# Aatrick/LightDiffusion

Hardware: AMD Instinct MI355X
Metric: UNet denoise steps/sec at 512x512 (higher is better)
Workload: dtype f16 (fp32 accumulate); 1 GPU; SD1.5 512x512 UNet CFG step, euler_ancestral / normal-30, batch 8/GPU (UNet batch 16), latent 64x64; global_batch=8, parallelism=dp1 (replicas, RCCL cond broadcast), hip_graph=True, setup_before_warmup=hipGraph capture + one untimed schedule pass per workload

## Files before the change

### include/ld_mi355x.h

```cpp
#ifndef LD_MI355X_H
#define LD_MI355X_H

#include <stddef.h>
#include <stdint.h>

#ifdef __cplusplus
extern "C" {
#endif

#define LD_OK 0
#define LD_ERR_ARG 1
#define LD_ERR_SHAPE 2
#define LD_ERR_HIP 3
#define LD_ERR_STATE 4

#define LD_F16 0
#define LD_F32 1

const char* ld_version(void);
const char* ld_status_string(int status);

typedef struct {
    int in_channels, out_channels, model_channels;
    int num_levels;
    int channel_mult[8];
    int num_res_blocks[8];
    int transformer_depth[16];
    int transformer_depth_output[24];
    int transformer_depth_middle;
    int context_dim, num_heads;
} ld_unet_config;

typedef struct ld_unet ld_unet;

int ld_unet_create(const ld_unet_config* cfg, ld_unet** out);
void ld_unet_destroy(ld_unet* u);
int ld_unet_param_count(const ld_unet* u);
int ld_unet_param_info(const ld_unet* u, int index, const char** name, int* ndim, int64_t shape[4]);
int ld_unet_load_param(ld_unet* u, const char* name, const void* dev_src, int dtype, void* stream);
int ld_unet_reserve(ld_unet* u, int max_n, int max_h, int max_w, int max_ctx_tokens);
size_t ld_unet_workspace_bytes(const ld_unet* u);
size_t ld_unet_weight_bytes(const ld_unet* u);
int ld_unet_set_context(ld_unet* u, const void* ctx, int dtype, int n, int tokens, void* stream);
int ld_unet_forward(ld_unet* u, const float* x, const float* sigma, float* out, int n, int h, int w, int eps_only, void* stream);
int ld_unet_forward_pair(ld_unet* u, const float* x, const float* sigma, float* out, int nb, int h, int w, void* stream);
int ld_unet_profile(ld_unet* u, const float* x, const float* sigma, float* out, int n, int h, int w, void* stream, double ms[6],
                    double flops[6], int launches[6]);
int ld_unet_profile_pair(ld_unet* u, const float* x, const float* sigma, float* out, int nb, int h, int w, void* stream, double ms[6],
                         double flops[6], int launches[6]);
int ld_unet_profile_kernels(const ld_unet* u, char* buf, size_t buf_bytes);
int ld_unet_profile_launches(const ld_unet* u, char* buf, size_t buf_bytes);
int ld_unet_last_launches(const ld_unet* u);
double ld_unet_last_flops(const ld_unet* u);

typedef struct {
    int z_channels, ch, num_levels;
    int ch_mult[8];
    int num_res_blocks, out_ch;
    int with_encoder;
} ld_vae_config;

typedef struct ld_vae ld_vae;

int ld_vae_create(const ld_vae_config* cfg, ld_vae** out);
void ld_vae_destroy(ld_vae* v);
int ld_vae_param_count(const ld_vae* v);
int ld_vae_param_info(const ld_vae* v, int index, const char** name, int* ndim, int64_t shape[4]);
int ld_vae_load_param(ld_vae* v, const char* name, const void* dev_src, int dtype, void* stream);
int ld_vae_reserve(ld_vae* v, int max_b, int max_h, int max_w);
size_t ld_vae_workspace_bytes(const ld_vae* v);
size_t ld_vae_plan_bytes(ld_vae* v, int b, int h, int w);
int ld_vae_decode(ld_vae* v, const float* z, float* out, int b, int h, int w, void* stream);
int ld_vae_encode(ld_vae* v, const float* pixels_nchw, float* moments, int b, int h, int w, void* stream);
int ld_vae_profile(ld_vae* v, const float* z, float* out, int b, int h, int w, void* stream);
int ld_vae_profile_launches(const ld_vae* v, char* buf, size_t buf_bytes);
int ld_vae_last_launches(const ld_vae* v);
double ld_vae_last_flops(const ld_vae* v);

int ld_op_linear(const void* x, const void* w, const void* bias, const void* residual, void* y, int M, int N, int K,
                 float alpha, int act, void* ws, size_t ws_bytes, void* stream);
int ld_op_conv(const void* x1, int c1, const void* x2, int c2, int n, int h, int w, int hv, int wv, int stride, int ksize,
               const void* wt, const void* bias, const void* rowvec, const void* residual, void* y, int cout,
               void* ws, size_t ws_bytes, void* stream);
size_t ld_op_groupnorm_conv_ws_bytes(int c1, int c2, int n, int h, int w, int cout);
int ld_op_groupnorm_conv(const void* x1, int c1, const void* x2, int c2, int n, int h, int w, const void* gamma, const void* beta, float eps,
                         const void* wt, const void* bias, const void* rowvec, const void* residual, void* y, int cout, void* ws,
                         size_t ws_bytes, void* stream);
int ld_op_repack_conv(const void* src_oihw, int dtype, int cout, int cin, void* dst, void* stream);
size_t ld_op_conv_skip_ws_bytes(int c, int sc1, int sc2, int cout);
int ld_op_conv_skip(const void* x, int c, int n, int h, int w, const void* wt, const void* bias, const void* s1, int sc1, const void* s2, int sc2,
                    const void* wskip, const void* bskip, const void* rowvec, void* y, int cout, void* ws, size_t ws_bytes, void* stream);
size_t ld_op_conv_gn_partials_floats(int n, int hw);
int ld_op_conv_gn_partials(const void* x, int c, int n, int h, int w, int hv, int wv, const void* wt, const void* bias,
                           const void* residual, void* y, int cout, float* part, int* chunks, void* ws, size_t ws_bytes, void* stream);
size_t ld_op_groupnorm_ws_bytes(int n, int hw);
int ld_op_groupnorm(const void* x1, int c1, const void* x2, int c2, int n, int hw, const void* gamma, const void* beta,
                    float eps, int silu, void* y, void* ws, void* stream);
int ld_op_layernorm(const void* x, const void* gamma, const void* beta, void* y, int rows, int c, float eps, void* stream);
int ld_op_attention(const void* q, int ldq, const void* k, int ldk, const void* vt, int ldvt, void* o, int ldo, int b,
                    int heads, int lq, int lk, int d, float scale, int causal, void* stream);
int ld_op_attention_rowv(const void* q, int ldq, const void* k, int ldk, const void* v, int ldv, void* o, int ldo, int b,
                         int heads, int lq, int lk, int d, float scale, int causal, void* stream);
int ld_op_softmax_rows(void* s, int rows, int cols, void* stream);
int ld_op_timestep_embed(const float* sigma, const float* log_sigmas, int n_sigmas, int n, int dim, void* out_f16, float* t_out,
                         void* stream);
int ld_op_cfg_combine(const float* den2, float* out, float cfg, size_t n_half, void* stream);
int ld_op_axpby(float* x, float a, const float* y, float b, const float* z, float c, size_t n, void* stream);
int ld_op_hook_check(const void* a, const void* b, size_t words_ab, const void* x, size_t half_words_x, const void* sigma, int half_sigma,
                     int* flags, int epoch, void* stream);

int ld_op_linear_ln(const void* x, const void* w_prod, const void* b_prod, const void* gamma, const void* beta, const void* w,
                    const void* bias, void* t_out, void* y, int M, int C, int N, float eps, void* ws, size_t ws_bytes, void* stream);
int ld_op_linear_ln_geglu(const void* x, const void* w_prod, const void* b_prod, const void* gamma, const void* beta, const void* w,
                          const void* bias, void* t_out, void* y, int M, int C, int N, float eps, void* ws, size_t ws_bytes, void* stream);
int ld_op_bislerp(const float* x, float* tmp, float* y, int n, int c, int h, int w, int h_new, int w_new, void* stream);
const char* ld_op_last_kernel(void);

#ifdef __cplusplus
}
#endif
#endif
```

### lightdiffusion_amd/_lib.py

```python
from __future__ import annotations

import ctypes as C
import os

_HERE = os.path.dirname(os.path.abspath(__file__))
LIB_PATH = os.environ.get("LD_MI355X_LIB") or os.path.join(_HERE, "libld_mi355x.so")

OK, ERR_ARG, ERR_SHAPE, ERR_HIP, ERR_STATE = 0, 1, 2, 3, 4
F16, F32 = 0, 1


class UNetConfig(C.Structure):
    _fields_ = [("in_channels", C.c_int), ("out_channels", C.c_int), ("model_channels", C.c_int), ("num_levels", C.c_int),
                ("channel_mult", C.c_int * 8), ("num_res_blocks", C.c_int * 8), ("transformer_depth", C.c_int * 16),
                ("transformer_depth_output", C.c_int * 24), ("transformer_depth_middle", C.c_int),
                ("context_dim", C.c_int), ("num_heads", C.c_int)]


class VAEConfig(C.Structure):
    _fields_ = [("z_channels", C.c_int), ("ch", C.c_int), ("num_levels", C.c_int), ("ch_mult", C.c_int * 8),
                ("num_res_blocks", C.c_int), ("out_ch", C.c_int), ("with_encoder", C.c_int)]


class LDError(RuntimeError):
    def __init__(self, status: int, where: str):
        self.status = status
        msg = lib().ld_status_string(status).decode() if _lib is not None else str(status)
        super().__init__(f"{where}: {msg} (status {status})")


_lib = None
_P, _I, _F, _Z = C.c_void_p, C.c_int, C.c_float, C.c_size_t

SIGNATURES = {
    "ld_version": (C.c_char_p, []),
    "ld_status_string": (C.c_char_p, [_I]),
    "ld_unet_create": (_I, [C.POINTER(UNetConfig), C.POINTER(_P)]),
    "ld_unet_destroy": (None, [_P]),
    "ld_unet_param_count": (_I, [_P]),
    "ld_unet_param_info": (_I, [_P, _I, C.POINTER(C.c_char_p), C.POINTER(_I), C.POINTER(C.c_int64)]),
    "ld_unet_load_param": (_I, [_P, C.c_char_p, _P, _I, _P]),
    "ld_unet_reserve": (_I, [_P, _I, _I, _I, _I]),
    "ld_unet_workspace_bytes": (_Z, [_P]),
    "ld_unet_weight_bytes": (_Z, [_P]),
    "ld_unet_set_context": (_I, [_P, _P, _I, _I, _I, _P]),
    "ld_unet_forward": (_I, [_P, _P, _P, _P, _I, _I, _I, _I, _P]),
    "ld_unet_forward_pair": (_I, [_P, _P, _P, _P, _I, _I, _I, _P]),
    "ld_unet_profile_pair": (_I, [_P, _P, _P, _P, _I, _I, _I, _P, C.POINTER(C.c_double), C.POINTER(C.c_double), C.POINTER(_I)]),
    "ld_unet_profile": (_I, [_P, _P, _P, _P, _I, _I, _I, _P, C.POINTER(C.c_double), C.POINTER(C.c_double), C.POINTER(_I)]),
    "ld_unet_profile_kernels": (_I, [_P, C.c_char_p, _Z]),
    "ld_unet_profile_launches": (_I, [_P, C.c_char_p, _Z]),
    "ld_unet_last_launches": (_I, [_P]),
    "ld_unet_last_flops": (C.c_double, [_P]),
    "ld_vae_create": (_I, [C.POINTER(VAEConfig), C.POINTER(_P)]),
    "ld_vae_destroy": (None, [_P]),
    "ld_vae_param_count": (_I, [_P]),
    "ld_vae_param_info": (_I, [_P, _I, C.POINTER(C.c_char_p), C.POINTER(_I), C.POINTER(C.c_int64)]),
    "ld_vae_load_param": (_I, [_P, C.c_char_p, _P, _I, _P]),
    "ld_vae_reserve": (_I, [_P, _I, _I, _I]),
    "ld_vae_workspace_bytes": (_Z, [_P]),
    "ld_vae_plan_bytes": (_Z, [_P, _I, _I, _I]),
    "ld_vae_decode": (_I, [_P, _P, _P, _I, _I, _I, _P]),
    "ld_vae_encode": (_I, [_P, _P, _P, _I, _I, _I, _P]),
    "ld_vae_profile": (_I, [_P, _P, _P, _I, _I, _I, _P]),
    "ld_vae_profile_launches": (_I, [_P, C.c_char_p, _Z]),
    "ld_vae_last_launches": (_I, [_P]),
    "ld_vae_last_flops": (C.c_double, [_P]),
    "ld_op_linear": (_I, [_P, _P, _P, _P, _P, _I, _I, _I, _F, _I, _P, _Z, _P]),
    "ld_op_conv": (_I, [_P, _I, _P, _I, _I, _I, _I, _I, _I, _I, _I, _P, _P, _P, _P, _P, _I, _P, _Z, _P]),
    "ld_op_groupnorm_conv_ws_bytes": (_Z, [_I, _I, _I, _I, _I, _I]),
    "ld_op_groupnorm_conv": (_I, [_P, _I, _P, _I, _I, _I, _I, _P, _P, _F, _P, _P, _P, _P, _P, _I, _P, _Z, _P]),
    "ld_op_repack_conv": (_I, [_P, _I, _I, _I, _P, _P]),
    "ld_op_conv_skip_ws_bytes": (_Z, [_I, _I, _I, _I]),
    "ld_op_conv_skip": (_I, [_P, _I, _I, _I, _I, _P, _P, _P, _I, _P, _I, _P, _P, _P, _P, _I, _P, _Z, _P]),
    "ld_op_groupnorm_ws_bytes": (_Z, [_I, _I]),
    "ld_op_groupnorm": (_I, [_P, _I, _P, _I, _I, _I, _P, _P, _F, _I, _P, _P, _P]),
    "ld_op_layernorm": (_I, [_P, _P, _P, _P, _I, _I, _F, _P]),
    "ld_op_attention": (_I, [_P, _I, _P, _I, _P, _I, _P, _I, _I, _I, _I, _I, _I, _F, _I, _P]),
    "ld_op_conv_gn_partials_floats": (_Z, [_I, _I]),
    "ld_op_conv_gn_partials": (_I, [_P, _I, _I, _I, _I, _I, _I, _P, _P, _P, _P, _I, _P, _P, _P, _Z, _P]),
    "ld_op_attention_rowv": (_I, [_P, _I, _P, _I, _P, _I, _P, _I, _I, _I, _I, _I, _I, _F, _I, _P]),
    "ld_op_softmax_rows": (_I, [_P, _I, _I, _P]),
    "ld_op_timestep_embed": (_I, [_P, _P, _I, _I, _I, _P, _P, _P]),
    "ld_op_cfg_combine": (_I, [_P, _P, _F, _Z, _P]),
    "ld_op_axpby": (_I, [_P, _F, _P, _F, _P, _F, _Z, _P]),
    "ld_op_hook_check": (_I, [_P, _P, _Z, _P, _Z, _P, _I, _P, _I, _P]),
    "ld_op_linear_ln": (_I, [_P, _P, _P, _P, _P, _P, _P, _P, _P, _I, _I, _I, _F, _P, _Z, _P]),
    "ld_op_linear_ln_geglu": (_I, [_P, _P, _P, _P, _P, _P, _P, _P, _P, _I, _I, _I, _F, _P, _Z, _P]),
    "ld_op_bislerp": (_I, [_P, _P, _P, _I, _I, _I, _I, _I, _I, _P]),
    "ld_op_last_kernel": (C.c_char_p, []),
}


def lib() -> C.CDLL:
    global _lib
    if _lib is None:
        if not os.path.exists(LIB_PATH):
            raise ImportError(f"{LIB_PATH} not found — build it with `python -c 'import __graft_entry__ as g; g.build()'` "
                              f"or `make -C lightdiffusion_amd/csrc`.  There is no CPU / PyTorch fallback for the hot path.")
        try:
            import torch
        except ImportError:
            pass
        l = C.CDLL(LIB_PATH)
        missing = []
        for name, (res, args) in SIGNATURES.items():
            if not hasattr(l, name):
                if not os.environ.get("LD_MI355X_LIB"):
                    raise AttributeError(f"{LIB_PATH} does not export {name}: header and library out of sync — rebuild it")
                missing.append(name)
                setattr(l, name, _missing_symbol(name))
                continue
            fn = getattr(l, name)
            fn.restype = res
            fn.argtypes = args
        l._ld_missing = tuple(missing)
        _lib = l
    return _lib


def _missing_symbol(name: str):
    def fail(*_a, **_k):
        raise RuntimeError(f"{LIB_PATH} (LD_MI355X_LIB) does not export {name}: it was built from a commit without this entry point")
    return fail


def check(status: int, where: str) -> None:
    if status != OK:
        raise LDError(status, where)
```

### lightdiffusion_amd/csrc/capi.hip

```cpp
#include <string>

#include "kernels.h"
#include "../../include/ld_mi355x.h"

namespace {
inline size_t align256(size_t v) { return (v + 255) / 256 * 256; }

thread_local std::string t_op_kernels;
inline void op_begin() { t_op_kernels.clear(); }
inline int noted(int st, const char* name) {
    if (name != nullptr && *name != '\0') {
        if (!t_op_kernels.empty()) t_op_kernels += ';';
        t_op_kernels += name;
    }
    return st;
}
inline int gemm_op(const GemmParams& p, hipStream_t s) { return noted(gemm_launch(p, s), gemm_last_kernel_name()); }
inline int gemm_op(const GemmParams& p, const GemmPlan& plan, hipStream_t s) { return noted(gemm_run(p, plan, s), gemm_last_kernel_name()); }

constexpr size_t kSyncBytes = LD_SYNC_INTS * sizeof(int);
inline size_t conv8_scratch_head(int cout, int cin) { return kSyncBytes + (conv8_weight_eligible(cout, cin) ? align256(conv8_weight_bytes(cout, cin)) : 0); }
inline void conv8_scratch(GemmParams& p, void* ws, size_t partial_bytes) {
    const int cin = p.C1 + p.C2;
    p.sync = (int*)ws;
    p.W8 = conv8_weight_eligible(p.N, cin) ? (const half_t*)((char*)ws + kSyncBytes) : nullptr;
    p.partial = (float*)((char*)ws + conv8_scratch_head(p.N, cin));
    p.partial_bytes = partial_bytes;
}
inline int conv8_scratch_op(const GemmParams& p, const GemmPlan& plan, const void* wt, hipStream_t stream) {
    if (plan.route == GR_CONV8) {
        if (hipMemsetAsync(p.sync, 0, kSyncBytes, stream) != hipSuccess) return LD_ERR_HIP;
        const int st = conv8_repack_launch((const half_t*)wt, p.N, p.C1 + p.C2, const_cast<half_t*>(p.W8), stream);
        if (st != LD_OK) return st;
    }
    return gemm_op(p, plan, stream);
}
inline int attn_op(const AttnParams& a, hipStream_t s) { return noted(attention_launch(a, s), attention_last_kernel_name()); }
}

extern "C" {

const char* ld_version(void) { return "ld_mi355x 0.1 (gfx950)"; }

const char* ld_op_last_kernel(void) { return t_op_kernels.c_str(); }

const char* ld_status_string(int s) {
    switch (s) {
        case LD_OK: return "ok";
        case LD_ERR_ARG: return "invalid argument";
        case LD_ERR_SHAPE: return "unsupported shape or alignment";
        case LD_ERR_HIP: return "HIP runtime error";
        case LD_ERR_STATE: return "invalid call order (weights / reserve / context missing)";
        default: return "unknown status";
    }
}

int ld_op_linear(const void* x, const void* w, const void* bias, const void* residual, void* y, int M, int N, int K, float alpha,
                 int act, void* ws, size_t ws_bytes, void* stream_) {
    op_begin();
    hipStream_t stream = (hipStream_t)stream_;
    GemmParams p;
    p.A = (const half_t*)x; p.lda = K;
    p.W = (const half_t*)w; p.ldw = K;
    p.M = M; p.N = N; p.K = K;
    p.alpha = alpha;
    p.bias_n = (const half_t*)bias;
    p.R = (const half_t*)residual;
    p.act = act;
    p.C = (half_t*)y;
    p.ldc = p.ldr = (act == 2 ? N / 2 : N);
    char* wsp = (char*)ws;
    if (act == 2) {
        if (bias == nullptr || (N & 15)) return LD_ERR_ARG;
        const int bn = gemm_pick_bn(N);
        if (N % bn) return LD_ERR_SHAPE;
        const size_t wb = align256((size_t)N * K * sizeof(half_t)), bb = align256((size_t)N * sizeof(half_t));
        if (ws == nullptr || ws_bytes < wb + bb) return LD_ERR_ARG;
        half_t* w2 = (half_t*)wsp;
        half_t* b2 = (half_t*)(wsp + wb);
        int st = repack_rows_launch(w, 0, N, K, w2, bn, stream);
        if (st != LD_OK) return st;
        st = repack_rows_launch(bias, 0, N, 1, b2, bn, stream);
        if (st != LD_OK) return st;
        p.W = w2;
        p.bias_n = b2;
        p.bn = bn;
        wsp += wb + bb;
        ws_bytes -= wb + bb;
    }
    p.partial = (float*)wsp;
    p.partial_bytes = ws ? ws_bytes : 0;
    if (ws == nullptr) p.partial = nullptr;
    return gemm_op(p, stream);
}

static int op_conv(const void* x1, int c1, const void* x2, int c2, int n, int h, int w, int hv, int wv, int stride, int ksize,
                   const void* wt, const void* bias, const void* rowvec, const void* residual, void* y, int cout, void* ws,
                   size_t ws_bytes, void* stream, float* gn_part, int* gn_chunks) {
    if (stride < 1 || (ksize != 1 && ksize != 3)) return LD_ERR_ARG;
    GemmParams p;
    if (gn_part != nullptr) {
        const int HW = (ksize == 3 ? (hv - 1) / stride + 1 : hv) * (ksize == 3 ? (wv - 1) / stride + 1 : wv);
        p.gn_part = gn_part;
        p.gn_P = gn_num_chunks(n, HW);
        p.gn_HW = HW;
        p.gn_ppb = (HW + p.gn_P - 1) / p.gn_P;
        p.gn_part_done = gn_chunks;
    }
    p.conv = 1;
    p.ksize = ksize;
    p.A = (const half_t*)x1; p.A2 = (const half_t*)x2; p.C1 = c1; p.C2 = c2;
    p.Hs = h; p.Ws = w; p.Hv = hv; p.Wv = wv; p.stride = stride;
    p.Ho = ksize == 3 ? (hv - 1) / stride + 1 : hv;
    p.Wo = ksize == 3 ? (wv - 1) / stride + 1 : wv;
    p.K = ksize * ksize * (c1 + c2);
    p.W = (const half_t*)wt; p.ldw = p.K;
    p.M = n * p.Ho * p.Wo; p.N = cout;
    p.bias_n = (const half_t*)bias;
    p.rowvec = (const half_t*)rowvec; p.rows_per_vec = p.Ho * p.Wo; p.ldrv = cout;
    p.R = (const half_t*)residual; p.ldr = cout;
    p.C = (half_t*)y; p.ldc = cout;
    p.partial = (float*)ws;
    p.partial_bytes = ws ? ws_bytes : 0;
    const size_t head = conv8_scratch_head(cout, c1 + c2);
    if (ws != nullptr && ksize == 3 && conv8_weight_eligible(cout, c1 + c2) && ws_bytes > head + ((size_t)8 << 20)) {
        GemmParams c8 = p;
        conv8_scratch(c8, ws, ws_bytes - head);
        if (const GemmPlan plan = gemm_plan(c8); plan.route == GR_CONV8) return conv8_scratch_op(c8, plan, wt, (hipStream_t)stream);
    }
    return gemm_op(p, (hipStream_t)stream);
}

int ld_op_conv(const void* x1, int c1, const void* x2, int c2, int n, int h, int w, int hv, int wv, int stride, int ksize,
               const void* wt, const void* bias, const void* rowvec, const void* residual, void* y, int cout, void* ws,
               size_t ws_bytes, void* stream) {
    op_begin();
    return op_conv(x1, c1, x2, c2, n, h, w, hv, wv, stride, ksize, wt, bias, rowvec, residual, y, cout, ws, ws_bytes, stream, nullptr, nullptr);
}

size_t ld_op_conv_gn_partials_floats(int n, int hw) {
    op_begin();
    return groupnorm_workspace_bytes(n, hw) / sizeof(float);
}

int ld_op_conv_gn_partials(const void* x, int c, int n, int h, int w, int hv, int wv, const void* wt, const void* bias, const void* residual,
                           void* y, int cout, float* part, int* chunks, void* ws, size_t ws_bytes, void* stream) {
    op_begin();
    if (part == nullptr || chunks == nullptr) return LD_ERR_ARG;
    *chunks = 0;
    return op_conv(x, c, nullptr, 0, n, h, w, hv, wv, 1, 3, wt, bias, nullptr, residual, y, cout, ws, ws_bytes, stream, part, chunks);
}

size_t ld_op_groupnorm_conv_ws_bytes(int c1, int c2, int n, int h, int w, int cout) {
    op_begin();
    const size_t C = (size_t)c1 + c2, HW = (size_t)h * w;
    return align256(groupnorm_workspace_bytes(n, (int)HW)) + 2 * align256((size_t)n * C * sizeof(float)) + align256((size_t)n * HW * C * sizeof(half_t)) +
           conv8_scratch_head(cout, c1 + c2) + ((size_t)96 << 20);
}

int ld_op_groupnorm_conv(const void* x1, int c1, const void* x2, int c2, int n, int h, int w, const void* gamma, const void* beta, float eps,
                         const void* wt, const void* bias, const void* rowvec, const void* residual, void* y, int cout, void* ws, size_t ws_bytes,
                         void* stream_) {
    op_begin();
    if (x1 == nullptr || gamma == nullptr || beta == nullptr || wt == nullptr || y == nullptr || ws == nullptr) return LD_ERR_ARG;
    if (ws_bytes < ld_op_groupnorm_conv_ws_bytes(c1, c2, n, h, w, cout)) return LD_ERR_ARG;
    hipStream_t stream = (hipStream_t)stream_;
    const int C = c1 + c2, HW = h * w;
    char* q = (char*)ws;
    float* part = (float*)q; q += align256(groupnorm_workspace_bytes(n, HW));
    float* scale = (float*)q; q += align256((size_t)n * C * sizeof(float));
    float* shift = (float*)q; q += align256((size_t)n * C * sizeof(float));
    half_t* g = (half_t*)q; q += align256((size_t)n * HW * C * sizeof(half_t));
    GemmParams p;
    p.conv = 1; p.ksize = 3;
    p.A = (const half_t*)x1; p.A2 = (const half_t*)x2; p.C1 = c1; p.C2 = c2;
    p.Hs = p.Hv = p.Ho = h; p.Ws = p.Wv = p.Wo = w; p.stride = 1;
    p.K = 9 * C; p.W = (const half_t*)wt; p.ldw = p.K;
    p.M = n * HW; p.N = cout;
    p.bias_n = (const half_t*)bias;
    p.rowvec = (const half_t*)rowvec; p.rows_per_vec = HW; p.ldrv = cout;
    p.R = (const half_t*)residual; p.ldr = cout;
    p.C = (half_t*)y; p.ldc = cout;
    conv8_scratch(p, q, (size_t)96 << 20);
    const GemmPlan fused = gemm_plan(p, true);
    if (fused.can_fuse_groupnorm) {
        int st = groupnorm_scale_shift_launch((const half_t*)x1, c1, (const half_t*)x2, c2, n, HW, (const half_t*)gamma, (const half_t*)beta, eps, part,
                                              scale, shift, stream);
        if (st != LD_OK) return st;
        p.gn_scale = scale; p.gn_shift = shift; p.gn_silu = 1;
        return gemm_op(p, fused, stream);
    }
    int st = groupnorm_launch((const half_t*)x1, c1, (const half_t*)x2, c2, n, HW, (const half_t*)gamma, (const half_t*)beta, eps, 1, g, part, stream);
    if (st != LD_OK) return st;
    p.A = g; p.A2 = nullptr; p.C1 = C; p.C2 = 0;
    return conv8_scratch_op(p, gemm_plan(p), (const half_t*)wt, stream);
}

size_t ld_op_conv_skip_ws_bytes(int c, int sc1, int sc2, int cout) {
    op_begin();
    return align256((size_t)cout * (9 * (size_t)c + sc1 + sc2) * sizeof(half_t)) + align256((size_t)cout * sizeof(half_t)) + ((size_t)96 << 20);
}

int ld_op_conv_skip(const void* x, int c, int n, int h, int w, const void* wt, const void* bias, const void* s1, int sc1, const void* s2, int sc2,
                    const void* wskip, const void* bskip, const void* rowvec, void* y, int cout, void* ws, size_t ws_bytes, void* stream_) {
    op_begin();
    if (x == nullptr || wt == nullptr || bias == nullptr || s1 == nullptr || wskip == nullptr || bskip == nullptr || y == nullptr || ws == nullptr) return LD_ERR_ARG;
    if (c <= 0 || sc1 <= 0 || sc2 < 0 || (sc2 > 0 && s2 == nullptr) || cout <= 0 || n <= 0 || h <= 0 || w <= 0) return LD_ERR_ARG;
    if (ws_bytes < ld_op_conv_skip_ws_bytes(c, sc1, sc2, cout)) return LD_ERR_ARG;
    hipStream_t stream = (hipStream_t)stream_;
    const int K9 = 9 * c, SC = sc1 + sc2;
    char* q = (char*)ws;
    half_t* wf = (half_t*)q; q += align256((size_t)cout * (K9 + SC) * sizeof(half_t));
    half_t* bf = (half_t*)q; q += align256((size_t)cout * sizeof(half_t));
    int st = skip_fold_launch((const half_t*)wt, (const half_t*)wskip, (const half_t*)bias, (const half_t*)bskip, cout, K9, SC, wf, bf, stream);
    if (st != LD_OK) return st;
    GemmParams p;
    p.conv = 1; p.ksize = 3;
    p.A = (const half_t*)x; p.C1 = c;
    p.Hs = p.Hv = p.Ho = h; p.Ws = p.Wv = p.Wo = w; p.stride = 1;
    p.S1 = (const half_t*)s1; p.SC1 = sc1; p.S2 = (const half_t*)s2; p.SC2 = sc2;
    p.K = K9 + SC; p.W = wf; p.ldw = p.K;
    p.M = n * h * w; p.N = cout;
    p.bias_n = bf;
    p.rowvec = (const half_t*)rowvec; p.rows_per_vec = h * w; p.ldrv = cout;
    p.C = (half_t*)y; p.ldc = cout;
    p.partial = (float*)q; p.partial_bytes = (size_t)96 << 20;
    return gemm_op(p, stream);
}

int ld_op_repack_conv(const void* src, int dtype, int cout, int cin, void* dst, void* stream) {
    op_begin();
    return repack_conv3x3_launch(src, dtype == LD_F32, cout, cin, (half_t*)dst, (hipStream_t)stream);
}

size_t ld_op_groupnorm_ws_bytes(int n, int hw) {
    op_begin();
    return groupnorm_workspace_bytes(n, hw);
}

int ld_op_groupnorm(const void* x1, int c1, const void* x2, int c2, int n, int hw, const void* gamma, const void* beta, float eps,
                    int silu, void* y, void* ws, void* stream) {
    op_begin();
    return groupnorm_launch((const half_t*)x1, c1, (const half_t*)x2, c2, n, hw, (const half_t*)gamma, (const half_t*)beta, eps,
                            silu, (half_t*)y, (float*)ws, (hipStream_t)stream);
}

int ld_op_layernorm(const void* x, const void* gamma, const void* beta, void* y, int rows, int c, float eps, void* stream) {
    op_begin();
    return layernorm_launch((const half_t*)x, (const half_t*)gamma, (const half_t*)beta, (half_t*)y, rows, c, eps, (hipStream_t)stream);
}

int ld_op_attention(const void* q, int ldq, const void* k, int ldk, const void* vt, int ldvt, void* o, int ldo, int b, int heads,
                    int lq, int lk, int d, float scale, int causal, void* stream) {
    op_begin();
    AttnParams a;
    a.Q = (const half_t*)q; a.ldq = ldq; a.sQ = (long long)lq * ldq;
    a.K = (const half_t*)k; a.ldk = ldk; a.sK = (long long)lk * ldk;
    a.Vt = (const half_t*)vt; a.ldvt = ldvt; a.sV = (long long)heads * d * ldvt;
    a.O = (half_t*)o; a.ldo = ldo; a.sO = (long long)lq * ldo;
    a.B = b; a.H = heads; a.Lq = lq; a.Lk = lk; a.d = d; a.scale = scale; a.causal = causal;
    return attn_op(a, (hipStream_t)stream);
}

int ld_op_attention_rowv(const void* q, int ldq, const void* k, int ldk, const void* v, int ldv, void* o, int ldo, int b, int heads,
                         int lq, int lk, int d, float scale, int causal, void* stream) {
    op_begin();
    const char *qb = (const char*)q, *kb = (const char*)k, *vb = (const char*)v;
    const long long rowb = (long long)ldq * 2;
    const bool fused = ldq == ldk && ldk == ldv && rowb > 0 && (kb - qb >= 0 ? kb - qb : qb - kb) < rowb && (vb - qb >= 0 ? vb - qb : qb - vb) < rowb;
    if (fused && lq != lk) return LD_ERR_SHAPE;
    AttnParams a;
    a.Q = (const half_t*)q; a.ldq = ldq; a.sQ = (long long)lq * ldq;
    a.K = (const half_t*)k; a.ldk = ldk; a.sK = (long long)lk * ldk;
    a.V = (const half_t*)v; a.ldv = ldv; a.sV = (long long)lk * ldv;
    a.O = (half_t*)o; a.ldo = ldo; a.sO = (long long)lq * ldo;
    a.B = b; a.H = heads; a.Lq = lq; a.Lk = lk; a.d = d; a.scale = scale; a.causal = causal;
    return attn_op(a, (hipStream_t)stream);
}

int ld_op_softmax_rows(void* s, int rows, int cols, void* stream) {
    op_begin();
    return softmax_rows_launch((half_t*)s, rows, cols, cols, (hipStream_t)stream);
}

int ld_op_timestep_embed(const float* sigma, const float* log_sigmas, int n_sigmas, int n, int dim, void* out, float* t_out, void* stream) {
    op_begin();
    return timestep_embed_launch(sigma, log_sigmas, n_sigmas, n, dim, (half_t*)out, t_out, (hipStream_t)stream);
}

int ld_op_cfg_combine(const float* den2, float* out, float cfg, size_t n_half, void* stream) {
// ... 107 lines not shown
```

### lightdiffusion_amd/csrc/gemm.h

```cpp
#pragma once
#include "common.h"

struct GemmParams {
    const half_t* A = nullptr;
    const half_t* A2 = nullptr;
    int lda = 0;
    int conv = 0;
    int ksize = 3;
    int pad = -1;
    int Hs = 0, Ws = 0;
    int Hv = 0, Wv = 0;
    int Ho = 0, Wo = 0, stride = 1;
    int C1 = 0, C2 = 0;
    const half_t* S1 = nullptr;
    const half_t* S2 = nullptr;
    int SC1 = 0, SC2 = 0;
    const half_t* W = nullptr;
    int ldw = 0;
    int M = 0, N = 0, K = 0;
    int n_valid = 0;
    int batch = 1;
    long long sA = 0, sW = 0, sC = 0, sR = 0;
    float alpha = 1.0f;
    const half_t* bias_n = nullptr;
    const half_t* bias_m = nullptr;
    const half_t* rowvec = nullptr;
    int rows_per_vec = 1, ldrv = 0;
    const half_t* R = nullptr;
    int ldr = 0;
    int act = 0;
    half_t* C = nullptr;
    int ldc = 0;
    int bm = 0, bn = 0;
    int splitk = 0;
    int m_fastest = -1;
    int xcd_gm = 0;
    float* partial = nullptr;
    size_t partial_bytes = 0;
    float* stat_out = nullptr;
    int* stat_parts_out = nullptr;
    const float* ln_stat = nullptr;
    int ln_parts = 0;
    int ln_rows = 0;
    int ln_zrows = 0;
    float ln_inv_c = 0.f, ln_eps = 0.f;
    const float* ln_wsum = nullptr;
    int ln_swapped = 0;
    const float* gn_scale = nullptr;
    const float* gn_shift = nullptr;
    int gn_silu = 0;
    float* gn_part = nullptr;
    int gn_P = 0, gn_ppb = 0, gn_HW = 0;
    int* gn_part_done = nullptr;
    const half_t* W8 = nullptr;
    int* sync = nullptr;
    int c8_S = 0;
    int dbg = 0;
};

enum GemmRoute { GR_NONE = 0, GR_CONV8, GR_CONV6, GR_GEMM7, GR_GEMM5, GR_GEMM3, GR_GEMM4 };
enum GemmReduce { GRD_NONE = 0, GRD_PLAIN, GRD_GROUPNORM };
struct GemmPlan {
    int status = LD_OK;
    int route = GR_NONE;
    bool conv = false, geglu = false;
    bool gn = false, up = false;
    bool ln = false;
    bool deep = false, two_wg = false;
    int bm = 0, bn = 0, wc = 0;
    int splitk = 1, c8_S = 0;
    int m_fastest = 0, xcd_gm = 0;
    unsigned grid_x = 0, grid_z = 1;
    int reduce = GRD_NONE;
    int stat_parts = 0;
    int gn_chunks = 0;
    bool halo_tile = false;
    bool can_fuse_groupnorm = false;
    bool takes_skip_segment = false;
    const char* kernel = "";
};
GemmPlan gemm_plan(const GemmParams& p, bool gn_offer = false);
int gemm_run(const GemmParams& p, const GemmPlan& plan, hipStream_t stream);
inline int gemm_launch(const GemmParams& p, hipStream_t stream) { return gemm_run(p, gemm_plan(p), stream); }
const char* gemm_last_kernel_name();

bool conv8_plan(const GemmParams& p, int* S_out);
int conv8_launch(const GemmParams& p, int S, hipStream_t stream);
bool conv8_weight_eligible(int N, int Cin);
size_t conv8_weight_bytes(int N, int Cin);
int conv8_repack_launch(const half_t* w_okki, int N, int Cin, half_t* dst, hipStream_t stream);
#define LD_SYNC_INTS 1024

static inline int gemm_pick_bn(int N) { return (N % 160 == 0) ? 160 : 128; }
```

### lightdiffusion_amd/csrc/gemm.hip

```cpp
#include <cstdlib>
#include <mutex>
#include <set>
#include <string>
#include <type_traits>
#include <vector>

#include "gemm.h"

namespace {

constexpr int BK = 64;
constexpr int NT = 256;

__device__ __forceinline__ void epilogue_store8(const GemmParams& p, int z, int m, int n_out, int n_bias, float (&v)[8]) {
    const bool hb = p.bias_n != nullptr && p.act != 2, hv = p.rowvec != nullptr, hr = p.R != nullptr;
    const uint4 rb = hb ? ld16(p.bias_n + n_bias) : zero16();
    const uint4 rv = hv ? ld16(p.rowvec + (long long)(m / p.rows_per_vec) * p.ldrv + n_out) : zero16();
    const uint4 rr = hr ? ld16(p.R + (long long)z * p.sR + (long long)m * p.ldr + n_out) : zero16();
    const float bm = p.bias_m != nullptr ? (float)p.bias_m[m] : 0.f;
    float b[8], e[8], r[8];
    unpack8(rb, b);
    unpack8(rv, e);
    unpack8(rr, r);
#pragma unroll
// ... 921 lines not shown
            return;
        }
        uint4 rba[3], rbg[3], rres[3];
#pragma unroll
        for (int it = 0; it < 3; ++it) {
            const int q = lane + it * 64;
            const int row = q / 10, cc = q - row * 10;
            const int m = m_base + row, nv = n_base + cc * 8;
            const bool ok = q < 160 && m < p.M;
            rba[it] = (ok && !bias_done) ? ld16(p.bias_n + nv) : zero16();
            rbg[it] = (ok && !bias_done) ? ld16(p.bias_n + nv + 80) : zero16();
            rres[it] = (ok && p.R != nullptr) ? ld16(p.R + (long long)z * p.sR + (long long)m * p.ldr + n_base / 2 + cc * 8) : zero16();
        }
#pragma unroll
        for (int it = 0; it < 3; ++it) {
            const int q = lane + it * 64;
            const int row = q / 10, cc = q - row * 10;
            const int m = m_base + row;
            if (q < 160 && m < p.M) {
                float a[8], g[8], ba[8], bg[8], r[8];
                unpack8(ld16(Cs + row * V5_EPI_LD + cc * 8), a);
                unpack8(ld16(Cs + row * V5_EPI_LD + 80 + cc * 8), g);
                unpack8(rba[it], ba);
                unpack8(rbg[it], bg);
                unpack8(rres[it], r);
#pragma unroll
                for (int j = 0; j < 8; ++j) a[j] = (a[j] + ba[j]) * gelu_f(g[j] + bg[j]) + r[j];
                st16(p.C + (long long)z * p.sC + (long long)m * p.ldc + n_base / 2 + cc * 8, pack8(a));
            }
        }
        return;
    }
    const bool hb = p.bias_n != nullptr && !bias_done, hv = p.rowvec != nullptr, hr = p.R != nullptr;
    if (rows_full && p.bias_m == nullptr && p.act == 0 && bias_done) {
        half_t* Cb = p.C + (long long)z * p.sC + (long long)m_base * p.ldc + n_base;
        const half_t* Rb = hr ? p.R + (long long)z * p.sR + (long long)m_base * p.ldr + n_base : nullptr;
        float s1[5], s2[5];
        uint4 rv[5], rres[5], cv[5];
#pragma unroll
        for (int k = 0; k < 5; ++k) {
            const int q = lane + k * 64;
            const int row = q / 20, cc = q - row * 20;
            rv[k] = hv ? ld16(p.rowvec + (long long)((m_base + row) / p.rows_per_vec) * p.ldrv + n_base + cc * 8) : zero16();
            rres[k] = hr ? ld16(Rb + (long long)row * p.ldr + cc * 8) : zero16();
            cv[k] = ld16(Cs + row * V5_EPI_LD + cc * 8);
        }
#pragma unroll
        for (int k = 0; k < 5; ++k) {
            const int q = lane + k * 64;
            const int row = q / 20, cc = q - row * 20;
            uint4 packed = cv[k];
            if (hv) packed = add8h(packed, rv[k]);
            if (hr) packed = add8h(packed, rres[k]);
            st16(Cb + (long long)row * p.ldc + cc * 8, packed);
            if (EPI == 1 && p.stat_out != nullptr) {
                const half2v one2 = {(half_t)1.f, (half_t)1.f};
                const half2v h0 = __builtin_bit_cast(half2v, packed.x), h1 = __builtin_bit_cast(half2v, packed.y);
                const half2v h2 = __builtin_bit_cast(half2v, packed.z), h3 = __builtin_bit_cast(half2v, packed.w);
                float a1 = __builtin_amdgcn_fdot2(h1, one2, __builtin_amdgcn_fdot2(h0, one2, 0.f, false), false);
                float a2 = __builtin_amdgcn_fdot2(h1, h1, __builtin_amdgcn_fdot2(h0, h0, 0.f, false), false);
                s1[k] = __builtin_amdgcn_fdot2(h3, one2, __builtin_amdgcn_fdot2(h2, one2, a1, false), false);
                s2[k] = __builtin_amdgcn_fdot2(h3, h3, __builtin_amdgcn_fdot2(h2, h2, a2, false), false);
            }
        }
        if (EPI == 1 && p.stat_out != nullptr) {
            float* sc = reinterpret_cast<float*>(Cs);
            asm volatile("s_waitcnt lgkmcnt(0)" ::: "memory");
#pragma unroll
            for (int it = 0; it < 5; ++it) *reinterpret_cast<float2*>(sc + (lane + it * 64) * 2) = make_float2(s1[it], s2[it]);
            asm volatile("s_waitcnt lgkmcnt(0)" ::: "memory");
            if (lane < 16) {
                float a = 0.f, b = 0.f;
#pragma unroll 4
                for (int c = 0; c < 20; ++c) {
                    const float2 t = *reinterpret_cast<const float2*>(sc + (lane * 20 + c) * 2);
                    a += t.x;
                    b += t.y;
                }
                *reinterpret_cast<float2*>(p.stat_out + ((long long)part * p.M + m_base + lane) * 2) = make_float2(a, b);
            }
            asm volatile("s_waitcnt lgkmcnt(0)" ::: "memory");
        }
        return;
    }
    uint4 rb[5], rv[5], rres[5];
#pragma unroll
    for (int it = 0; it < 5; ++it) {
        const int q = lane + it * 64;
        const int row = q / 20, cc = q - row * 20;
        const int m = m_base + row, n = n_base + cc * 8;
        const bool ok = m < p.M;
        rb[it] = (ok && hb) ? ld16(p.bias_n + n) : zero16();
        rv[it] = (ok && hv) ? ld16(p.rowvec + (long long)(m / p.rows_per_vec) * p.ldrv + n) : zero16();
        rres[it] = (ok && hr) ? ld16(p.R + (long long)z * p.sR + (long long)m * p.ldr + n) : zero16();
    }
    float s1[5], s2[5];
#pragma unroll
    for (int it = 0; it < 5; ++it) {
        const int q = lane + it * 64;
        const int row = q / 20, cc = q - row * 20;
        const int m = m_base + row, n = n_base + cc * 8;
        s1[it] = s2[it] = 0.f;
        if (m < p.M) {
            float v[8], b[8], e[8], r[8];
            unpack8(ld16(Cs + row * V5_EPI_LD + cc * 8), v);
            unpack8(rb[it], b);
            unpack8(rv[it], e);
            unpack8(rres[it], r);
            const float bm = p.bias_m != nullptr ? (float)p.bias_m[m] : 0.f;
#pragma unroll
            for (int j = 0; j < 8; ++j) {
                float t = v[j] + b[j] + bm + e[j];
                if (p.act == 1) t = silu_f(t);
                else if (p.act == 3) t = quick_gelu_f(t);
                v[j] = t + r[j];
            }
            const uint4 packed = pack8(v);
            st16(p.C + (long long)z * p.sC + (long long)m * p.ldc + n, packed);
            if (EPI == 1 && p.stat_out != nullptr) {
                float f[8];
                unpack8(packed, f);
#pragma unroll
                for (int j = 0; j < 8; ++j) {
                    s1[it] += f[j];
                    s2[it] += f[j] * f[j];
                }
            }
        }
    }
    if (EPI == 1 && p.stat_out != nullptr) {
        float* sc = reinterpret_cast<float*>(Cs);
        asm volatile("s_waitcnt lgkmcnt(0)" ::: "memory");
#pragma unroll
        for (int it = 0; it < 5; ++it) {
            const int q = lane + it * 64;
            sc[q * 2] = s1[it];
            sc[q * 2 + 1] = s2[it];
        }
        asm volatile("s_waitcnt lgkmcnt(0)" ::: "memory");
        if (lane < 16 && m_base + lane < p.M) {
            float a = 0.f, b = 0.f;
            for (int c = 0; c < 20; ++c) {
                a += sc[(lane * 20 + c) * 2];
                b += sc[(lane * 20 + c) * 2 + 1];
            }
            float* o = p.stat_out + ((long long)part * p.M + m_base + lane) * 2;
            o[0] = a;
            o[1] = b;
        }
        asm volatile("s_waitcnt lgkmcnt(0)" ::: "memory");
    }
}

template <int EPI, bool LNC>
__device__ __forceinline__ void v5_finish(const GemmParams& p, f32x4 (&acc)[4][10], char* smem5, const float* ln_mu, const float* ln_rs, int z, int m0,
                                          int n0, int wm0, int wn0, int wid, int lane, int ks, int splitk, int tn_i) {
    constexpr int TM = 4, TN = 10;
    const int fr = lane & 15, fq = lane >> 4;
    const int m_w = m0 + wm0, n_w = n0 + wn0;
    if (splitk > 1) {
        float* part = p.partial + (long long)ks * p.M * p.N;
#pragma unroll
        for (int i = 0; i < TM; ++i) {
            const int m = m_w + i * 16 + fr;
#pragma unroll
            for (int j = 0; j < TN; ++j) {
                const int n = n_w + j * 16 + fq * 4;
                if (m < p.M) {
                    f32x4 v = acc[i][j];
                    v *= p.alpha;
                    *reinterpret_cast<f32x4*>(part + (long long)m * p.N + n) = v;
                }
            }
        }
        return;
    }
    half_t* Cs = reinterpret_cast<half_t*>(smem5 + wid * 2 * V5_EPI_BYTES);
    const int part = tn_i * 2 + (wid & 1);
    const bool ln = LNC && p.ln_stat != nullptr;
    const bool bias_done = EPI == 2 || p.act == 0;
    const bool add_b = bias_done && p.bias_n != nullptr;
    const half_t* bsrc = (add_b ? p.bias_n + n_w : reinterpret_cast<const half_t*>(g_zero_row)) + fq * 4;
    auto stage = [&](auto I, half_t* dst) {
        constexpr int i = decltype(I)::value;
        const float mu = ln ? ln_mu[wm0 + i * 16 + fr] : 0.f, rs = ln ? ln_rs[wm0 + i * 16 + fr] : 1.f;
#pragma unroll
        for (int j = 0; j < TN; ++j) {
            f32x4 v = acc[i][j];
            if (ln) {
                const f32x4 ws = *reinterpret_cast<const f32x4*>(p.ln_wsum + n_w + j * 16 + fq * 4);
                v = (v - mu * ws) * rs;
            }
            const half4 bh = *reinterpret_cast<const half4*>(bsrc + j * 16);
            f32x4 o;
#pragma unroll
            for (int r = 0; r < 4; ++r) o[r] = v[r] * p.alpha + (float)bh[r];
            *reinterpret_cast<uint2*>(dst + fr * V5_EPI_LD + j * 16 + fq * 4) = make_uint2(pk2h(o[0], o[1]), pk2h(o[2], o[3]));
        }
    };
    half_t* Cs1 = Cs + 16 * V5_EPI_LD;
    stage(std::integral_constant<int, 0>{}, Cs);
    stage(std::integral_constant<int, 1>{}, Cs1);
    asm volatile("s_waitcnt lgkmcnt(0)" ::: "memory");
    __builtin_amdgcn_sched_barrier(0);
    v5_epilogue_strip<EPI>(p, Cs, z, m_w, n_w, lane, part, bias_done);
    v5_epilogue_strip<EPI>(p, Cs1, z, m_w + 16, n_w, lane, part, bias_done);
    asm volatile("s_waitcnt lgkmcnt(0)" ::: "memory");
    __builtin_amdgcn_sched_barrier(0);
    stage(std::integral_constant<int, 2>{}, Cs);
    stage(std::integral_constant<int, 3>{}, Cs1);
    asm volatile("s_waitcnt lgkmcnt(0)" ::: "memory");
    __builtin_amdgcn_sched_barrier(0);
    v5_epilogue_strip<EPI>(p, Cs, z, m_w + 32, n_w, lane, part, bias_done);
    v5_epilogue_strip<EPI>(p, Cs1, z, m_w + 48, n_w, lane, part, bias_done);
}

template <int TM, int TN>
__device__ __forceinline__ void v6_finish(const GemmParams& p, f32x4 (&acc)[TM][TN], char* smem5, int m0, int n0, int wm0, int wn0, int wid, int lane, int ks,
                                          int splitk, int gimg, int gchunk) {
    static_assert(TM == 4 || TM == 8, "wave tile of 64 or 128 rows");
    constexpr int WN = TN * 16, LD = WN + 4, STRIP_BYTES = 16 * LD * 2;
    constexpr int CPR = WN / 8, TOT = 16 * CPR, ITS = (TOT + 63) / 64;
    const int fr = lane & 15, fq = lane >> 4;
    const int m_w = m0 + wm0, n_w = n0 + wn0;
    if (splitk > 1) {
        float* part = p.partial + (long long)ks * p.M * p.N;
#pragma unroll
        for (int i = 0; i < TM; ++i) {
            const int m = m_w + i * 16 + fr;
#pragma unroll
            for (int j = 0; j < TN; ++j) {
                if (m < p.M) {
                    f32x4 v = acc[i][j];
                    v *= p.alpha;
                    *reinterpret_cast<f32x4*>(part + (long long)m * p.N + n_w + j * 16 + fq * 4) = v;
                }
            }
        }
        return;
    }
    half_t* Cs0 = reinterpret_cast<half_t*>(smem5 + wid * 2 * STRIP_BYTES);
    const bool hb = p.bias_n != nullptr, hv = p.rowvec != nullptr, hr = p.R != nullptr;
    const bool gne = p.gn_part != nullptr, g4 = p.N == 128;
    float gs[4] = {0.f, 0.f, 0.f, 0.f};
    const bool packed_ok = p.act == 0 && p.bias_m == nullptr;
    const half_t* bsrc = ((packed_ok && hb) ? p.bias_n + n_w : reinterpret_cast<const half_t*>(g_zero_row)) + fq * 4;
    auto stage = [&](auto I, half_t* dst) {
        constexpr int i = decltype(I)::value;
#pragma unroll
        for (int j = 0; j < TN; ++j) {
            const half4 bh = *reinterpret_cast<const half4*>(bsrc + j * 16);
            f32x4 v = acc[i][j] * p.alpha;
#pragma unroll
            for (int r = 0; r < 4; ++r) v[r] += (float)bh[r];
            *reinterpret_cast<uint2*>(dst + fr * LD + j * 16 + fq * 4) = make_uint2(pk2h(v[0], v[1]), pk2h(v[2], v[3]));
        }
    };
    auto strip = [&](const half_t* Cs, int m_base) {
        if (packed_ok) {
            uint4 rv[ITS], rres[ITS], cv[ITS];
#pragma unroll
            for (int it = 0; it < ITS; ++it) {
                const int q0 = lane + it * 64;
                const int q = (TOT % 64 == 0 || q0 < TOT) ? q0 : 0;
                const int row = q / CPR, cc = q - row * CPR;
                const int m = m_base + row < p.M ? m_base + row : p.M - 1;
                const int n = n_w + cc * 8;
                rv[it] = hv ? ld16(p.rowvec + (long long)(m / p.rows_per_vec) * p.ldrv + n) : zero16();
                rres[it] = hr ? ld16(p.R + (long long)m * p.ldr + n) : zero16();
                cv[it] = ld16(Cs + row * LD + cc * 8);
            }
#pragma unroll
            for (int it = 0; it < ITS; ++it) {
                const int q0 = lane + it * 64;
                const int q = (TOT % 64 == 0 || q0 < TOT) ? q0 : 0;
                const int row = q / CPR, cc = q - row * CPR;
                uint4 packed = cv[it];
                if (hv) packed = add8h(packed, rv[it]);
                if (hr) packed = add8h(packed, rres[it]);
                if ((TOT % 64 == 0 || q0 < TOT) && m_base + row < p.M && n_w + cc * 8 < p.n_valid) {
                    st16(p.C + (long long)(m_base + row) * p.ldc + n_w + cc * 8, packed);
                    if (gne) {
                        const half2v one2 = {(half_t)1.f, (half_t)1.f};
                        const half2v h0 = __builtin_bit_cast(half2v, packed.x), h1 = __builtin_bit_cast(half2v, packed.y);
                        const half2v h2 = __builtin_bit_cast(half2v, packed.z), h3 = __builtin_bit_cast(half2v, packed.w);
                        gs[0] = __builtin_amdgcn_fdot2(h1, one2, __builtin_amdgcn_fdot2(h0, one2, gs[0], false), false);
                        gs[1] = __builtin_amdgcn_fdot2(h1, h1, __builtin_amdgcn_fdot2(h0, h0, gs[1], false), false);
                        gs[2] = __builtin_amdgcn_fdot2(h3, one2, __builtin_amdgcn_fdot2(h2, one2, gs[2], false), false);
                        gs[3] = __builtin_amdgcn_fdot2(h3, h3, __builtin_amdgcn_fdot2(h2, h2, gs[3], false), false);
                    }
                }
            }
            return;
        }
        uint4 rb[ITS], rv[ITS], rres[ITS], cv[ITS];
        half_t rm[ITS];
#pragma unroll
        for (int it = 0; it < ITS; ++it) {
            const int q0 = lane + it * 64;
            const int q = (TOT % 64 == 0 || q0 < TOT) ? q0 : 0;
            const int row = q / CPR, cc = q - row * CPR;
            const int m = m_base + row < p.M ? m_base + row : p.M - 1;
            const int n = n_w + cc * 8;
            rb[it] = hb ? ld16(p.bias_n + n) : zero16();
            rv[it] = hv ? ld16(p.rowvec + (long long)(m / p.rows_per_vec) * p.ldrv + n) : zero16();
            rres[it] = hr ? ld16(p.R + (long long)m * p.ldr + n) : zero16();
            rm[it] = p.bias_m != nullptr ? p.bias_m[m] : (half_t)0.f;
            cv[it] = ld16(Cs + row * LD + cc * 8);
        }
#pragma unroll
        for (int it = 0; it < ITS; ++it) {
            const int q0 = lane + it * 64;
            const int q = (TOT % 64 == 0 || q0 < TOT) ? q0 : 0;
            const int row = q / CPR, cc = q - row * CPR;
            float v[8], b[8], e[8], r[8];
            unpack8(cv[it], v);
            unpack8(rb[it], b);
            unpack8(rv[it], e);
            unpack8(rres[it], r);
            const float bm = (float)rm[it];
#pragma unroll
            for (int j = 0; j < 8; ++j) {
                float t = v[j] + b[j] + bm + e[j];
                if (p.act == 1) t = silu_f(t);
                else if (p.act == 3) t = quick_gelu_f(t);
                v[j] = t + r[j];
            }
            if ((TOT % 64 == 0 || q0 < TOT) && m_base + row < p.M && n_w + cc * 8 < p.n_valid) {
                const uint4 packed = pack8(v);
                st16(p.C + (long long)(m_base + row) * p.ldc + n_w + cc * 8, packed);
                if (gne) {
                    const half2v one2 = {(half_t)1.f, (half_t)1.f};
                    const half2v h0 = __builtin_bit_cast(half2v, packed.x), h1 = __builtin_bit_cast(half2v, packed.y);
                    const half2v h2 = __builtin_bit_cast(half2v, packed.z), h3 = __builtin_bit_cast(half2v, packed.w);
                    gs[0] = __builtin_amdgcn_fdot2(h1, one2, __builtin_amdgcn_fdot2(h0, one2, gs[0], false), false);
                    gs[1] = __builtin_amdgcn_fdot2(h1, h1, __builtin_amdgcn_fdot2(h0, h0, gs[1], false), false);
                    gs[2] = __builtin_amdgcn_fdot2(h3, one2, __builtin_amdgcn_fdot2(h2, one2, gs[2], false), false);
                    gs[3] = __builtin_amdgcn_fdot2(h3, h3, __builtin_amdgcn_fdot2(h2, h2, gs[3], false), false);
                }
            }
        }
    };
    half_t* Cs1 = Cs0 + 16 * LD;
    auto pair = [&](auto P) {
        constexpr int i0 = 2 * decltype(P)::value;
        stage(std::integral_constant<int, i0>{}, Cs0);
        stage(std::integral_constant<int, i0 + 1>{}, Cs1);
        asm volatile("s_waitcnt lgkmcnt(0)" ::: "memory");
        __builtin_amdgcn_sched_barrier(0);
        strip(Cs0, m_w + 16 * i0);
        strip(Cs1, m_w + 16 * i0 + 16);
        asm volatile("s_waitcnt lgkmcnt(0)" ::: "memory");
        __builtin_amdgcn_sched_barrier(0);
    };
    pair(std::integral_constant<int, 0>{});
    pair(std::integral_constant<int, 1>{});
    if constexpr (TM == 8) {
        pair(std::integral_constant<int, 2>{});
        pair(std::integral_constant<int, 3>{});
    }
    if (gne && 64 % CPR == 0) {
        if (!g4) {
            gs[0] += gs[2];
            gs[1] += gs[3];
        }
#pragma unroll
        for (int o = CPR; o < 64; o <<= 1) {
#pragma unroll
            for (int k = 0; k < 4; ++k) gs[k] += __shfl_xor(gs[k], o, 64);
        }
        float* wp = reinterpret_cast<float*>(smem5 + 8 * 2 * STRIP_BYTES);
        if (lane < CPR) *reinterpret_cast<float4*>(wp + (wid * CPR + lane) * 4) = make_float4(gs[0], gs[1], gs[2], gs[3]);
        __syncthreads();
        const int cpg = p.N / 32, tid = wid * 64 + lane;
        if (tid < 2 * WN / cpg) {
            const int col = tid * cpg, wn = col / WN, cf = (col - wn * WN) >> 3;
            const int nch = cpg >= 8 ? cpg >> 3 : 1, part = (cpg == 4 && (col & 4)) ? 2 : 0;
            float s = 0.f, ss = 0.f;
            for (int wmi = 0; wmi < 4; ++wmi)
                for (int c = 0; c < nch; ++c) {
                    const float* e = wp + ((wmi * 2 + wn) * CPR + cf + c) * 4 + part;
                    s += e[0];
                    ss += e[1];
                }
            float* o = p.gn_part + (((long long)gimg * p.gn_P + gchunk) * 32 + (n0 + col) / cpg) * 2;
            o[0] = s;
            o[1] = ss;
        }
    }
}

template <bool CONV, int EPI>
__global__ __launch_bounds__(512, 2) void gemm5_kernel(const GemmParams p) {
    constexpr int TM = 4, TN = 10;
    __shared__ __attribute__((aligned(16))) char smem5[V5_NST * V5_STAGE_BYTES];
    static_assert(8 * 2 * V5_EPI_BYTES <= V5_NST * V5_STAGE_BYTES, "epilogue staging must fit in the ring");
    __shared__ __attribute__((aligned(16))) float ln_mu[V5_BM], ln_rs[V5_BM];

    const int tid = threadIdx.x, lane = tid & 63;
    const int wid = __builtin_amdgcn_readfirstlane(tid >> 6);
    const bool grp1 = wid >= 4;
    const int wm0 = (wid >> 1) * 64, wn0 = (wid & 1) * 160;
    const int z = blockIdx.z;
    const int tiles_m = (p.M + V5_BM - 1) / V5_BM, tiles_n = p.N / V5_BN;
    const int tiles = tiles_m * tiles_n;
    const int splitk = p.splitk > 1 ? p.splitk : 1;
    int bid = xcd_remap(blockIdx.x, tiles * splitk);
    const int ks = bid / tiles;
    bid -= ks * tiles;
    int tn_i = bid % tiles_n, tm_i = bid / tiles_n;
    if (!CONV && p.xcd_gm > 0) {
        const int gn = 8 / p.xcd_gm, per = tiles >> 3, x = bid / per, l = bid - x * per;
        const int bm_t = tiles_m / p.xcd_gm, bn_t = tiles_n / gn;
        tm_i = (x / gn) * bm_t + l % bm_t;
        tn_i = (x % gn) * bn_t + l / bm_t;
    }
    const int m0 = tm_i * V5_BM, n0 = tn_i * V5_BN;
    const int KT = p.K / V5_BK;
    const int kt_begin = (int)((long long)ks * KT / splitk), kt_end = (int)((long long)(ks + 1) * KT / splitk);
    const int nk = kt_end - kt_begin;

    const half_t* Ab = p.A + (long long)z * p.sA;
    const half_t* Wb = p.W + (long long)z * p.sW;
    const half_t* zp = reinterpret_cast<const half_t*>(g_zero_row);
    const int Cin = p.C1 + p.C2;

    const int prow = lane >> 2;
    const int lchunk = (lane & 3) ^ ((V5_SWZ >> (2 * ((prow >> 2) & 3))) & 3);
    const int a_row0 = wid * 32 + prow;
    const half_t* a_ptr[2];
    unsigned a_off[2];
#pragma unroll
    for (int i = 0; i < 2; ++i) {
        const int m = m0 + a_row0 + i * 16;
        a_ptr[i] = zp;
        a_off[i] = CONV ? 0u : (unsigned)(((long long)(m < p.M ? m : p.M - 1) * p.lda + lchunk * 8) * 2);
    }
    const half_t* a_base = Ab + (long long)kt_begin * V5_BK;
    int seg_left = 0;
    int k_issue = kt_begin * V5_BK;
    auto conv_seek = [&](int k0) {
        const int K9 = p.ksize * p.ksize * Cin;
        const bool skp = k0 >= K9 && p.SC1 > 0;
        const int tap = skp ? 0 : k0 / Cin;
        const int c0 = skp ? k0 - K9 : k0 - tap * Cin;
        const int ky = skp ? p.pad : tap / p.ksize, kx = skp ? p.pad : tap - (tap / p.ksize) * p.ksize;
        const int Ca = skp ? p.SC1 : p.C1, Cb = skp ? p.SC2 : p.C2;
        const bool second = c0 >= Ca;
        const half_t* src = skp ? (second ? p.S2 : p.S1) : (second ? p.A2 : Ab);
        const int Cs = second ? Cb : Ca;
        const int cl = second ? c0 - Ca : c0;
        seg_left = ((second ? Ca + Cb : Ca) - c0) / V5_BK;
        const int hw = p.Ho * p.Wo;
#pragma unroll
        for (int i = 0; i < 2; ++i) {
            const int m = m0 + a_row0 + i * 16;
            const int mm = m < p.M ? m : 0;
            const int img = mm / hw, rem = mm - img * hw;
            const int oy = rem / p.Wo, ox = rem - oy * p.Wo;
            const int iy = oy * p.stride - p.pad + ky, ix = ox * p.stride - p.pad + kx;
            const bool ok = m < p.M && (unsigned)iy < (unsigned)p.Hv && (unsigned)ix < (unsigned)p.Wv && tap < p.ksize * p.ksize && c0 < Ca + Cb;
            int sy = iy, sx = ix;
            if (p.Hv == 2 * p.Hs && p.Wv == 2 * p.Ws) {
                sy = iy >> 1;
                sx = ix >> 1;
            } else if (p.Hv != p.Hs || p.Wv != p.Ws) {
                sy = (int)((long long)iy * p.Hs / p.Hv);
                sx = (int)((long long)ix * p.Ws / p.Wv);
            }
            a_ptr[i] = ok ? src + (((long long)img * p.Hs + sy) * p.Ws + sx) * Cs + cl + lchunk * 8 : zp + lchunk * 8;
        }
    };
    unsigned b_off[3];
#pragma unroll
    for (int i = 0; i < 3; ++i) {
        const int piece = i < 2 ? wid * 2 + i : 16 + (wid & 3);
        const int row = piece * 16 + prow;
        const int n = n0 + row < p.n_valid ? n0 + row : p.n_valid - 1;
        b_off[i] = (unsigned)(((long long)n * p.ldw + lchunk * 8) * 2);
    }
    const half_t* b_base = Wb + (long long)kt_begin * V5_BK;

    const unsigned smem_base = __builtin_amdgcn_readfirstlane((unsigned)(unsigned long long)(const __attribute__((address_space(3))) void*)smem5);
    unsigned st_issue = 0;
    auto issue = [&]() {
        const unsigned As = smem_base + st_issue + (unsigned)(wid * 2) * 1024u;
        const unsigned Bs = smem_base + st_issue + (unsigned)V5_A_BYTES;
#pragma unroll
        for (int i = 0; i < 2; ++i) {
            if (CONV) glds16(a_ptr[i], As + (unsigned)i * 1024u);
            else glds16s(a_off[i], a_base, As + (unsigned)i * 1024u);
        }
#pragma unroll
        for (int i = 0; i < 2; ++i) glds16s(b_off[i], b_base, Bs + (unsigned)(wid * 2 + i) * 1024u);
        if (!grp1) glds16s(b_off[2], b_base, Bs + (unsigned)(16 + wid) * 1024u);
        k_issue += V5_BK;
        if (CONV) {
            if (--seg_left <= 0) {
                conv_seek(k_issue);
            } else {
                a_ptr[0] += V5_BK;
                a_ptr[1] += V5_BK;
            }
        } else {
            a_base += V5_BK;
        }
        b_base += V5_BK;
        st_issue = st_issue == (unsigned)((V5_NST - 1) * V5_STAGE_BYTES) ? 0u : st_issue + (unsigned)V5_STAGE_BYTES;
    };
    auto wait_all_but = [&](int n) {
        if (!grp1) {
            if (n >= 2) wait_vmcnt<10>();
            else if (n == 1) wait_vmcnt<5>();
            else wait_vmcnt<0>();
        } else {
            if (n >= 2) wait_vmcnt<8>();
            else if (n == 1) wait_vmcnt<4>();
            else wait_vmcnt<0>();
        }
    };
    if (CONV) conv_seek(k_issue);

    const int fr = lane & 15, fq = lane >> 4;
    const unsigned rchunk = (unsigned)(fq ^ ((V5_SWZ >> (2 * ((fr >> 2) & 3))) & 3)) << 4;
    const char* rdA = smem5 + (wm0 + fr) * 64 + rchunk;
    const char* rdB = smem5 + V5_A_BYTES + (wn0 + fr) * 64 + rchunk;
    int st_read = 0;

    f32x4 acc[TM][TN];
#pragma unroll
    for (int i = 0; i < TM; ++i)
#pragma unroll
        for (int j = 0; j < TN; ++j) acc[i][j] = (f32x4){0.f, 0.f, 0.f, 0.f};
    half8 fa[TM], fb[TN];

    issue();
    issue();
    if (nk > 2) issue();
    if (EPI != 0 && p.ln_stat != nullptr) ln_prepare<V5_BM, V5_BN>(p, ln_mu, ln_rs, z, m0, n0, tid);
    wait_all_but(nk > 2 ? 2 : 1);
    __builtin_amdgcn_s_barrier();
    if (grp1) __builtin_amdgcn_s_barrier();

    for (int k = 0; k < nk; ++k) {
        if (k + 3 < nk) issue();
#pragma unroll
        for (int j = 0; j < TN; ++j) fb[j] = as_half8(ld16(rdB + j * 1024));
#pragma unroll
        for (int i = 0; i < TM; ++i) fa[i] = as_half8(ld16(rdA + i * 1024));
        {
            const int d = st_read == V5_NST - 1 ? -(V5_NST - 1) * V5_STAGE_BYTES : V5_STAGE_BYTES;
            rdA += d;
            rdB += d;
            st_read = st_read == V5_NST - 1 ? 0 : st_read + 1;
        }
        wait_all_but(k + 3 < nk ? 2 : (k + 2 < nk ? 1 : 0));
        asm volatile("s_waitcnt lgkmcnt(0)" ::: "memory");
        __builtin_amdgcn_sched_barrier(0);
        __builtin_amdgcn_s_barrier();
        __builtin_amdgcn_s_setprio(1);
#pragma unroll
        for (int i = 0; i < TM; ++i)
#pragma unroll
            for (int j = 0; j < TN; ++j) acc[i][j] = __builtin_amdgcn_mfma_f32_16x16x32_f16(fb[j], fa[i], acc[i][j], 0, 0, 0);
        __builtin_amdgcn_s_setprio(0);
        __builtin_amdgcn_sched_barrier(0);
        __builtin_amdgcn_s_barrier();
    }
    if (!grp1) __builtin_amdgcn_s_barrier();

    v5_finish<EPI, EPI != 0>(p, acc, smem5, ln_mu, ln_rs, z, m0, n0, wm0, wn0, wid, lane, ks, splitk, tn_i);
}

template <int W, bool GN, int BN = V5_BN, int BM = V5_BM, bool UP = false>
__global__ __launch_bounds__(512, 2) void conv6_kernel(const GemmParams p) {
    constexpr int TM = BM / 64, TN = BN / 32;
    static_assert(BN == 320 || BN == 256 || BN == 160 || BN == 128 || BN == 32, "tile width");
    static_assert(BM == 256 || (BM == 512 && W == 128), "tile height: 256 pixels, or four rows of a 128-pixel band");
    static_assert(!GN || BN == V5_BN || (W == 128 && ((BN == 256 && BM == 256) || (BN == 128 && BM == 512))),
                  "the fused GroupNorm only pays where the output is one tile wide: the UNet's N = 320, the VAE's N = 256 / 128 at >= 256-pixel rows");
    static_assert(!(GN && UP), "no caller");
    constexpr int BPIECES = BN / 16, NB_ALL = BPIECES / 8, NB_EXTRA = BPIECES % 8;
    constexpr int TR = BM / W, HW2 = W + 2, HP = (TR + 2) * HW2;
    constexpr int NH = ((HP + 15) / 16 + 7) / 8;
    constexpr int HBYTES = NH * 8 * 1024;
    constexpr int BSTAGE = BN * 64, NSTB = 4;
    constexpr int RING0 = 2 * HBYTES;
    __shared__ __attribute__((aligned(16))) char smem5[2 * HBYTES + NSTB * BSTAGE];
    static_assert(2 * HBYTES + NSTB * BSTAGE <= 163840, "LDS");
    static_assert(!GN || NH <= 7, "fused GroupNorm: my (<= 7) pieces of the next slab are normalised in one go in the read phase of tap 3 (28 temporaries)");
    constexpr int HPIECES = (HP + 15) / 16;
    constexpr bool TBL_IN_HALO = 2 * HBYTES + NSTB * BSTAGE + 2048 > 163840;
    static_assert(!TBL_IN_HALO || NH * 8 - HPIECES >= 3, "two table slots and a dump slot");
    __shared__ __attribute__((aligned(16))) float gn_lds[(GN && !TBL_IN_HALO) ? 8 * 64 : 4];
    static_assert(8 * 2 * (BN == V5_BN ? V5_EPI_BYTES : 16 * (BN / 2 + 4) * 2) + 8 * (BN / 16) * 16 <= 2 * HBYTES + NSTB * BSTAGE,
                  "epilogue staging (+ the GroupNorm partials of the output) must fit");

    const int tid = threadIdx.x, lane = tid & 63;
    const int wid = __builtin_amdgcn_readfirstlane(tid >> 6);
    const bool grp1 = wid >= 4;
    const int wm = wid >> 1;
    const int wm0 = wm * (BM / 4), wn0 = (wid & 1) * (BN / 2);
    const int tiles_m = p.M / BM, tiles_n = p.N / BN;
    const int tiles = tiles_m * tiles_n;
    const int splitk = p.splitk > 1 ? p.splitk : 1;
    int bid = xcd_remap(blockIdx.x, tiles * splitk);
    const int ks = bid / tiles;
    bid -= ks * tiles;
    const int tn_i = bid % tiles_n, tm_i = bid / tiles_n;
    const int n0 = tn_i * BN;
    const int Cin = p.C1 + p.C2;
    const int NS = Cin / 32;
    const int s_begin = (int)((long long)ks * NS / splitk), s_end = (int)((long long)(ks + 1) * NS / splitk);
    const int nk = (s_end - s_begin) * 9;

    const half_t* zp = reinterpret_cast<const half_t*>(g_zero_row);
    const int Wimg = W == 128 ? p.Wo : W;
    const int HWo = p.Ho * Wimg;
    const int bands = Wimg / W, tiles_img = (p.Ho / TR) * bands;
    const int img = tm_i / tiles_img, t_in = tm_i - img * tiles_img;
    const int row0 = (t_in / bands) * TR, col0 = (t_in - (t_in / bands) * bands) * W;

    int hpix[NH];
#pragma unroll
    for (int j = 0; j < NH; ++j) {
        const int hp = (wid + 8 * j) * 16 + (lane >> 2);
        const int hy = hp / HW2, hx = hp - hy * HW2;
        const int iy = row0 + hy - 1, ix = col0 + hx - 1;
        const bool in = hp < HP && (unsigned)iy < (unsigned)p.Ho && (unsigned)ix < (unsigned)Wimg;
        hpix[j] = !in ? -1 : UP ? (iy >> 1) * (Wimg >> 1) + (ix >> 1) : iy * Wimg + ix;
    }
    const unsigned smem_base = __builtin_amdgcn_readfirstlane((unsigned)(unsigned long long)(const __attribute__((address_space(3))) void*)smem5);
    auto issue_halo = [&](int s, int buf) {
        const int c0 = s * 32;
        const bool second = c0 >= p.C1;
        const half_t* src = (second ? p.A2 : p.A) + (long long)img * p.Hs * p.Ws * (second ? p.C2 : p.C1) + (second ? c0 - p.C1 : c0) + (lane & 3) * 8;
        const int Cs = second ? p.C2 : p.C1;
#pragma unroll
        for (int j = 0; j < NH; ++j) {
            const half_t* g = hpix[j] >= 0 ? src + (long long)hpix[j] * Cs : zp;
            const int slot = (GN && TBL_IN_HALO && wid + 8 * j >= HPIECES) ? NH * 8 - 1 : wid + 8 * j;
            glds16(g, smem_base + (unsigned)(buf * HBYTES) + (unsigned)slot * 1024u);
        }
    };
    float gn_tbl = 0.f;
    auto gn_load = [&](int s) {
        const float* src = ((lane & 32) ? p.gn_shift : p.gn_scale) + (long long)img * Cin + s * 32 + (lane & 31);
        asm volatile("global_load_dword %0, %1, off" : "=&v"(gn_tbl) : "v"(src) : "memory");
    };
    float* const gn_mine = (TBL_IN_HALO ? reinterpret_cast<float*>(smem5 + HPIECES * 1024) : gn_lds) + wid * 64;
    auto gn_apply_slab = [&](int buf) {
        __builtin_amdgcn_sched_barrier(0);
        gn_mine[lane] = gn_tbl;
        const float* tp = gn_mine + (lane & 3) * 8;
        H8 io[NH];
#pragma unroll
        for (int j = 0; j < NH; ++j) io[j].u = ld16(smem5 + buf * HBYTES + (wid + 8 * j) * 1024 + lane * 16);
        const f32x4 sc0 = *reinterpret_cast<const f32x4*>(tp), sc1 = *reinterpret_cast<const f32x4*>(tp + 4);
        const f32x4 sh0 = *reinterpret_cast<const f32x4*>(tp + 32), sh1 = *reinterpret_cast<const f32x4*>(tp + 36);
#pragma unroll
        for (int j = 0; j < NH; ++j) {
#pragma unroll
            for (int e = 0; e < 8; ++e) {
                float v = (float)io[j].e[e] * (e < 4 ? sc0[e & 3] : sc1[e & 3]) + (e < 4 ? sh0[e & 3] : sh1[e & 3]);
                if (p.gn_silu) v *= __builtin_amdgcn_rcpf(1.0f + __expf(-v));
                io[j].e[e] = (half_t)v;
            }
            if (hpix[j] >= 0) st16(smem5 + buf * HBYTES + (wid + 8 * j) * 1024 + lane * 16, io[j].u);
        }
        asm volatile("s_waitcnt lgkmcnt(0)" ::: "memory");
        __builtin_amdgcn_sched_barrier(0);
    };
    const int prow = lane >> 2;
    const int lchunk = (lane & 3) ^ ((V5_SWZ >> (2 * ((prow >> 2) & 3))) & 3);
    const bool b_extra = wid < NB_EXTRA;
    unsigned b_off[NB_ALL + 1];
#pragma unroll
    for (int i = 0; i < NB_ALL + 1; ++i) {
        const int piece = i < NB_ALL ? wid * NB_ALL + i : 8 * NB_ALL + (wid % (NB_EXTRA > 0 ? NB_EXTRA : 1));
        const int n = n0 + piece * 16 + prow;
        b_off[i] = (unsigned)(((long long)n * p.ldw + lchunk * 8) * 2);
    }
    const half_t* b_base = p.W + (long long)s_begin * 32;
    int b_tap = 0;
    unsigned st_issue = 0;
    auto issue_b = [&]() {
        const unsigned Bs = smem_base + (unsigned)RING0 + st_issue;
#pragma unroll
        for (int i = 0; i < NB_ALL; ++i) glds16s(b_off[i], b_base, Bs + (unsigned)(wid * NB_ALL + i) * 1024u);
        if (NB_EXTRA > 0 && b_extra) glds16s(b_off[NB_ALL], b_base, Bs + (unsigned)(8 * NB_ALL + wid) * 1024u);
        if (b_tap == 8) {
            b_tap = 0;
            b_base += 32 - 8 * Cin;
        } else {
            ++b_tap;
            b_base += Cin;
        }
        st_issue = st_issue == (unsigned)((NSTB - 1) * BSTAGE) ? 0u : st_issue + (unsigned)BSTAGE;
    };
    auto wait_keep = [&](int steps, bool halo) {
        constexpr int PX = NB_ALL + 1, PA = NB_ALL;
        if (NB_EXTRA > 0 && b_extra) {
            if (steps >= 2) { if (halo) wait_vmcnt<2 * PX + NH>(); else wait_vmcnt<2 * PX>(); }
            else if (steps == 1) { if (halo) wait_vmcnt<PX + NH>(); else wait_vmcnt<PX>(); }
            else wait_vmcnt<0>();
        } else {
            if (steps >= 2) { if (halo) wait_vmcnt<2 * PA + NH>(); else wait_vmcnt<2 * PA>(); }
            else if (steps == 1) { if (halo) wait_vmcnt<PA + NH>(); else wait_vmcnt<PA>(); }
            else wait_vmcnt<0>();
        }
    };

    const int fr = lane & 15, fq = lane >> 4;
    const int oyw = wm0 / W, oxw = wm0 - oyw * W;
    const int m0 = img * HWo + (row0 + oyw) * Wimg + col0 + oxw - wm0;
    const char* rdA = smem5 + ((oyw * HW2 + oxw + fr) * 64 + fq * 16);
    const unsigned rchunk = (unsigned)(fq ^ ((V5_SWZ >> (2 * ((fr >> 2) & 3))) & 3)) << 4;
    const char* rdB = smem5 + RING0 + (wn0 + fr) * 64 + rchunk;
    int st_read = 0;

    f32x4 acc[TM][TN];
#pragma unroll
    for (int i = 0; i < TM; ++i)
#pragma unroll
// ... 355 lines not shown
        const int m = (int)(q / cpr), cc = (int)(q - (long long)m * cpr);
        float v[8];
        if (p.act == 2) {
            const int half_bn = bn / 2;
            const int no = cc * 8;
            const int tile = no / half_bn, within = no - tile * half_bn;
            const int nv = tile * bn + within, ng = nv + half_bn;
            float a[8] = {0, 0, 0, 0, 0, 0, 0, 0}, g[8] = {0, 0, 0, 0, 0, 0, 0, 0};
            for (int s = 0; s < p.splitk; ++s) {
                const float* base = p.partial + ((long long)s * p.M + m) * p.N;
#pragma unroll
                for (int j = 0; j < 8; ++j) {
                    a[j] += base[nv + j];
                    g[j] += base[ng + j];
                }
            }
            float ba[8], bg[8];
            unpack8(ld16(p.bias_n + nv), ba);
            unpack8(ld16(p.bias_n + ng), bg);
#pragma unroll
            for (int j = 0; j < 8; ++j) v[j] = (a[j] + ba[j]) * gelu_f(g[j] + bg[j]);
            epilogue_store8(p, 0, m, no, 0, v);
        } else {
            const int n = cc * 8;
#pragma unroll
            for (int j = 0; j < 8; ++j) v[j] = 0.f;
            const float* base = p.partial + (long long)m * p.N + n;
            const long long slab = (long long)p.M * p.N;
            int s = 0;
            for (; s + 4 <= p.splitk; s += 4) {
                f32x4 x0[4], x1[4];
#pragma unroll
                for (int u = 0; u < 4; ++u) {
                    x0[u] = *reinterpret_cast<const f32x4*>(base + (s + u) * slab);
                    x1[u] = *reinterpret_cast<const f32x4*>(base + (s + u) * slab + 4);
                }
#pragma unroll
                for (int u = 0; u < 4; ++u)
#pragma unroll
                    for (int j = 0; j < 4; ++j) {
                        v[j] += x0[u][j];
                        v[4 + j] += x1[u][j];
                    }
            }
            for (; s < p.splitk; ++s) {
                const f32x4 x0 = *reinterpret_cast<const f32x4*>(base + s * slab), x1 = *reinterpret_cast<const f32x4*>(base + s * slab + 4);
#pragma unroll
                for (int j = 0; j < 4; ++j) {
                    v[j] += x0[j];
                    v[4 + j] += x1[j];
                }
            }
            epilogue_store8(p, 0, m, n, n, v);
        }
    }
}

__global__ __launch_bounds__(256) void splitk_reduce_gn_kernel(const GemmParams p) {
    __shared__ float csum[2048], csq[2048];
    const int C = p.N, cpg = C / 32;
    const int CS = C / 4, CHS = CS >> 3;
    const int n = blockIdx.y, pc = blockIdx.x, slab = blockIdx.z, tid = threadIdx.x;
    const int rows_par = 256 / CHS;
    const int cc = tid % CHS, prow = tid / CHS;
    const int c0 = slab * CS + cc * 8;
    const int p_begin = pc * p.gn_ppb, p_end = min(p.gn_HW, p_begin + p.gn_ppb);
    const long long slab_stride = (long long)p.M * p.N;
    if (prow < rows_par) {
        float s[8], ss[8];
#pragma unroll
        for (int j = 0; j < 8; ++j) s[j] = ss[j] = 0.f;
        for (int pix = p_begin + prow; pix < p_end; pix += rows_par) {
            const int m = n * p.gn_HW + pix;
            const float* base = p.partial + (long long)m * p.N + c0;
            float v[8];
#pragma unroll
            for (int j = 0; j < 8; ++j) v[j] = 0.f;
            int sp = 0;
            for (; sp + 4 <= p.splitk; sp += 4) {
                f32x4 x0[4], x1[4];
#pragma unroll
                for (int u = 0; u < 4; ++u) {
                    x0[u] = *reinterpret_cast<const f32x4*>(base + (sp + u) * slab_stride);
                    x1[u] = *reinterpret_cast<const f32x4*>(base + (sp + u) * slab_stride + 4);
                }
#pragma unroll
                for (int u = 0; u < 4; ++u)
#pragma unroll
                    for (int j = 0; j < 4; ++j) {
                        v[j] += x0[u][j];
                        v[4 + j] += x1[u][j];
                    }
            }
            for (; sp < p.splitk; ++sp) {
                const f32x4 x0 = *reinterpret_cast<const f32x4*>(base + sp * slab_stride), x1 = *reinterpret_cast<const f32x4*>(base + sp * slab_stride + 4);
#pragma unroll
                for (int j = 0; j < 4; ++j) {
                    v[j] += x0[j];
                    v[4 + j] += x1[j];
                }
            }
            epilogue_store8(p, 0, m, c0, c0, v);
            float f[8];
            unpack8(pack8(v), f);
#pragma unroll
            for (int j = 0; j < 8; ++j) {
                s[j] += f[j];
                ss[j] += f[j] * f[j];
            }
        }
#pragma unroll
        for (int j = 0; j < 8; ++j) {
            csum[prow * CS + cc * 8 + j] = s[j];
            csq[prow * CS + cc * 8 + j] = ss[j];
        }
    }
    __syncthreads();
    {
        const int g = tid >> 5, sub = tid & 31;
        const int cnt = rows_par * cpg;
        float a = 0.f, b = 0.f;
        for (int i = sub; i < cnt; i += 32) {
            const int pr = i / cpg, c = g * cpg + (i - pr * cpg);
            a += csum[pr * CS + c];
            b += csq[pr * CS + c];
        }
#pragma unroll
        for (int o = 1; o < 32; o <<= 1) {
            a += __shfl_xor(a, o, 64);
            b += __shfl_xor(b, o, 64);
        }
        if (sub == 0) {
            float* o = p.gn_part + (((long long)n * p.gn_P + pc) * 32 + slab * 8 + g) * 2;
            o[0] = a;
            o[1] = b;
        }
    }
}

constexpr int V4_MAX_BLOCKS = 256;

thread_local const char* t_last_kernel = "";

const char* plan_kernel_name(const GemmPlan& pl) {
    typedef unsigned long long u64;
    const u64 key = (u64)pl.route | (u64)pl.reduce << 3 | (u64)pl.conv << 5 | (u64)pl.geglu << 6 | (u64)pl.gn << 7 | (u64)pl.up << 8 | (u64)pl.ln << 9 |
                    (u64)pl.deep << 10 | (u64)pl.two_wg << 11 | (u64)pl.bm << 12 | (u64)pl.bn << 24 | (u64)pl.wc << 36;
    thread_local std::vector<std::pair<u64, const char*>> seen;
    for (const auto& e : seen)
        if (e.first == key) return e.second;
    const std::string tile = std::to_string(pl.bm) + "," + std::to_string(pl.bn);
    std::string s;
    switch (pl.route) {
        case GR_CONV8: s = "conv8_kernel<W" + std::to_string(pl.wc) + (pl.up ? ",up>" : ">"); break;
        case GR_CONV6:
            s = "conv6_kernel<W" + std::to_string(pl.wc) + ",halo" + (pl.gn ? "+groupnorm" : "") +
                (pl.bn == V5_BN ? "" : "," + std::to_string(pl.bn) + (pl.bm == V5_BM ? "" : "x" + std::to_string(pl.bm))) + (pl.up ? ",up" : "") + ">";
            break;
        case GR_GEMM7: s = std::string("gemm7_kernel<256,K320,") + (pl.geglu ? "geglu" : "plain") + (pl.ln ? ",ln>" : ">"); break;
        case GR_GEMM5: s = std::string("gemm5_kernel<256,320,") + (pl.conv ? "conv" : pl.geglu ? "geglu" : pl.ln ? "lnfold" : "plain") + ">"; break;
        case GR_GEMM4: s = "gemm4_kernel<" + tile + (pl.conv ? ",conv" : ",plain") + (pl.two_wg ? ",2wg>" : ">"); break;
        default: s = "gemm3_kernel<" + tile + (pl.conv ? ",conv" : ",plain") + (pl.deep ? ",deep>" : ">"); break;
    }
    if (pl.reduce != GRD_NONE) s += pl.reduce == GRD_GROUPNORM ? "+splitk_reduce_gn_kernel" : "+splitk_reduce_kernel";
    static std::mutex mu; static std::set<std::string> pool;
    std::lock_guard<std::mutex> lock(mu);
    const char* name = pool.insert(s).first->c_str();
    seen.push_back({key, name});
    return name;
}

template <int BM, int BN>
void launch_cfg(const GemmParams& p, const GemmPlan& pl, dim3 grid, hipStream_t s) {
    if (pl.route == GR_GEMM4) {
        if constexpr (BM == 64 && BN == 64) {
            if (pl.two_wg) {
                if (!pl.conv) hipLaunchKernelGGL((gemm4_kernel<64, 64, false, 4, 4>), grid, dim3(2 * NT), 0, s, p);
                else hipLaunchKernelGGL((gemm4_kernel<64, 64, true, 4, 4>), grid, dim3(2 * NT), 0, s, p);
                return;
            }
        }
        hipLaunchKernelGGL((gemm4_kernel<BM, BN, false>), grid, dim3(2 * NT), 0, s, p);
    } else if (pl.conv) {
        if constexpr (BM == 64 && BN == 160) {
            if (pl.deep) {
                hipLaunchKernelGGL((gemm3_kernel<BM, BN, true, 4>), grid, dim3(NT), 0, s, p);
                return;
            }
        }
        hipLaunchKernelGGL((gemm3_kernel<BM, BN, true, 2>), grid, dim3(NT), 0, s, p);
    } else {
        hipLaunchKernelGGL((gemm3_kernel<BM, BN, false, 2>), grid, dim3(NT), 0, s, p);
    }
}

template <int W, bool GN, int BN, int BM, bool UP>
void launch_conv6_w(const GemmParams& p, dim3 grid, hipStream_t s) { hipLaunchKernelGGL((conv6_kernel<W, GN, BN, BM, UP>), grid, dim3(512), 0, s, p); }
template <bool GN, int BN = V5_BN, int BM = V5_BM, bool UP = false>
void launch_conv6(int wc, const GemmParams& p, dim3 grid, hipStream_t s) {
    if constexpr (BN == V5_BN) {
        if (wc == 16) return launch_conv6_w<16, GN, BN, BM, UP>(p, grid, s);
        if (wc == 32) return launch_conv6_w<32, GN, BN, BM, UP>(p, grid, s);
    }
    if constexpr (BN == V5_BN || (BN == 256 && !GN)) {
        if (wc == 64) return launch_conv6_w<64, GN, BN, BM, UP>(p, grid, s);
    }
    launch_conv6_w<128, GN, BN, BM, UP>(p, grid, s);
}

}

#ifdef LD_AB_BUILD
static int g_force_bm = 0, g_force_sk = 0;
static int g_shape_ovr[5] = {0, 0, 0, 0, 0};
extern "C" void ld_debug_gemm_shape_override(int M, int N, int K, int bm, int splitk) {
    g_shape_ovr[0] = M; g_shape_ovr[1] = N; g_shape_ovr[2] = K; g_shape_ovr[3] = bm; g_shape_ovr[4] = splitk;
}
extern "C" void ld_debug_gemm_override(int bm, int splitk) {
    g_force_bm = bm;
    g_force_sk = splitk;
}
#endif

const char* gemm_last_kernel_name() { return t_last_kernel; }

static void plan_reduce(const GemmParams& p, GemmPlan* pl) {
    if (pl->splitk <= 1) return;
    const bool gn = p.gn_part != nullptr && p.act != 2 && p.batch == 1 && p.gn_P > 0 && p.gn_HW > 0 && p.M % p.gn_HW == 0 && p.N % 32 == 0 && p.N <= 8192 && p.N >= 256 &&
                    p.ldc == p.N && (p.N / 4) % 8 == 0 && p.N / 32 <= 256;
    pl->reduce = gn ? GRD_GROUPNORM : GRD_PLAIN;
    if (gn) pl->gn_chunks = p.gn_P;
}

static bool v6_plan(const GemmParams& p, bool gn, GemmPlan* out) {
    const bool same = p.Hv == p.Hs && p.Wv == p.Ws;
    const bool up = p.Hv == 2 * p.Hs && p.Wv == 2 * p.Ws;
    if (!(p.conv && p.ksize == 3 && p.stride == 1 && (p.pad < 0 || p.pad == 1) && (same || up) && p.Ho == p.Hv && p.Wo == p.Wv &&
          p.C1 % 32 == 0 && p.C2 % 32 == 0 && p.bm == 0 && p.bn == 0 && p.splitk == 0 && p.batch == 1 && p.act != 2))
        return false;
    if (up && (p.C2 != 0 || gn)) return false;
    if (p.SC1 > 0) return false;
    const int wc = (p.Wo == 16 || p.Wo == 32 || p.Wo == 64 || p.Wo == 128) ? p.Wo : (p.Wo > 128 && p.Wo % 128 == 0) ? 128 : 0;
    if (wc == 0) return false;
    int bn = 0, bm = V5_BM;
    if (p.N % V5_BN == 0) {
        bn = V5_BN;
    } else if (p.N % 256 == 0 && wc >= 64 && (!gn || (p.N == 256 && wc == 128 && !up))) {
        bn = 256;
    } else if (p.N % 128 == 0 && wc == 128 && !up && (!gn || p.N == 128)) {
        bn = 128;
        bm = 512;
    } else if (p.N == 32 && wc == 128 && !gn && !up) {
        bn = 32;
        bm = 512;
    } else {
        return false;
    }
    if (p.Ho % (bm / wc) != 0 || p.M % bm != 0) return false;
    const long long tm = p.M / bm;
    const long long t6 = tm * (p.N / bn);
    const int NS = (p.C1 + p.C2) / 32;
    int sk6 = 1;
    if (t6 < 192 && p.partial != nullptr && p.K >= 8640) {
        sk6 = (int)((256 + t6 - 1) / t6);
        const int cap = p.K / 2560;
        if (sk6 > cap) sk6 = cap;
        if (sk6 > NS) sk6 = NS;
        while (sk6 > 1 && (size_t)sk6 * p.M * p.N * sizeof(float) > p.partial_bytes) --sk6;
    }
#ifdef LD_AB_BUILD
    if (p.partial != nullptr && bn == V5_BN) {
        static const char* names[4] = {"LD_V6_SK_W16", "LD_V6_SK_W32", "LD_V6_SK_W64", "LD_V6_SK_W128"};
        const char* e = getenv(names[wc == 16 ? 0 : wc == 32 ? 1 : wc == 64 ? 2 : 3]);
        if (e != nullptr) {
            int want = atoi(e);
            if (want < 1) want = 1;
            if (want > NS) want = NS;
            while (want > 1 && (size_t)want * p.M * p.N * sizeof(float) > p.partial_bytes) --want;
            sk6 = want;
        }
    }
#endif
    out->splitk = sk6; out->bn = bn; out->bm = bm; out->wc = wc; out->up = up;
    out->grid_x = (unsigned)(t6 * sk6);
    return t6 * sk6 >= 192;
}

GemmPlan gemm_plan(const GemmParams& pin, bool gn_offer) {
    GemmPlan pl;
    GemmParams p = pin;
    const bool gn = gn_offer || p.gn_scale != nullptr;
    const auto fail = [](int st) { GemmPlan f; f.status = st; return f; };
    const auto done = [&pl](int route) { pl.route = route; pl.kernel = plan_kernel_name(pl); return pl; };
#ifdef LD_AB_BUILD
    if (g_force_bm) p.bm = g_force_bm;
    if (g_force_sk) p.splitk = g_force_sk;
    if (g_shape_ovr[0] == p.M && g_shape_ovr[1] == p.N && g_shape_ovr[2] == p.K && p.batch == 1 && !gn) {
        p.bm = g_shape_ovr[3];
        p.splitk = g_shape_ovr[4];
    }
#endif
    if (p.M <= 0 || p.N <= 0 || p.K <= 0 || p.A == nullptr || p.W == nullptr || p.C == nullptr) return fail(LD_ERR_ARG);
    if ((p.N & 7) || (p.K & 7) || (p.ldw & 7) || (p.ldc & 7)) return fail(LD_ERR_SHAPE);
    if (p.conv) {
        const int Cin = p.C1 + p.C2;
        if (p.ksize != 1 && p.ksize != 3) return fail(LD_ERR_ARG);
        if (p.pad < 0) p.pad = p.ksize >> 1;
        if (p.SC1 < 0 || p.SC2 < 0 || (p.SC1 == 0 && p.SC2 != 0)) return fail(LD_ERR_ARG);
        if (Cin <= 0 || (p.C1 % 64) || (p.C2 % 64) || (p.SC1 % 64) || (p.SC2 % 64) || p.K != p.ksize * p.ksize * Cin + p.SC1 + p.SC2) return fail(LD_ERR_SHAPE);
        if (p.SC1 > 0) {
            if (p.S1 == nullptr || (p.SC2 > 0 && p.S2 == nullptr)) return fail(LD_ERR_ARG);
            if (p.stride != 1 || p.Hv != p.Hs || p.Wv != p.Ws || p.Ho != p.Hv || p.Wo != p.Wv || p.pad != p.ksize / 2 || p.SC1 > 32768 || p.SC2 > 32768) return fail(LD_ERR_SHAPE);
        }
        if (p.C1 > 32768 || p.C2 > 32768) return fail(LD_ERR_SHAPE);
        if (p.C2 > 0 && p.A2 == nullptr) return fail(LD_ERR_ARG);
        if (p.M % (p.Ho * p.Wo)) return fail(LD_ERR_SHAPE);
        if (p.batch != 1) return fail(LD_ERR_ARG);
    } else if (p.lda & 7) {
        return fail(LD_ERR_SHAPE);
    }
    if (p.act == 2 && (p.bias_n == nullptr || (p.N & 15))) return fail(LD_ERR_ARG);
    if (p.R != nullptr && (p.ldr & 7)) return fail(LD_ERR_SHAPE);
    if (p.n_valid <= 0 || p.n_valid > p.N) p.n_valid = p.N;
    pl.conv = p.conv != 0; pl.geglu = p.act == 2;

    if (!gn && conv8_plan(p, &pl.c8_S)) {
        pl.wc = p.Wo; pl.up = p.Hv == 2 * p.Hs;
        if (p.gn_part != nullptr) pl.gn_chunks = p.Wo * p.Wo / 16;
        return done(GR_CONV8);
    }
    if (GemmPlan v6 = pl; v6_plan(p, gn, &v6)) {
        pl = v6;
        const int bn6 = pl.bn, wc = pl.wc;
        if (gn) {
            if ((p.gn_scale != nullptr && p.gn_shift == nullptr) || pl.up) return fail(LD_ERR_ARG);
            if (bn6 != V5_BN && (wc != 128 || p.N != bn6 || !((bn6 == 256 && pl.bm == V5_BM) || (bn6 == 128 && pl.bm == 512)))) return fail(LD_ERR_ARG);
            pl.can_fuse_groupnorm = bn6 != V5_BN || p.N == V5_BN;
            if (gn_offer && !pl.can_fuse_groupnorm) return fail(LD_ERR_ARG);
            pl.gn = true;
        }
        if (pl.splitk == 1 && p.gn_part != nullptr) {
            const int cpg = p.N / 32, tiles_img = (p.Ho / (pl.bm / wc)) * (p.Wo / wc);
            const bool ok = (bn6 == 256 || bn6 == 128) && p.N % 32 == 0 && (p.N == 128 || cpg % 8 == 0) && bn6 % cpg == 0 && p.act == 0;
            if (ok) pl.gn_chunks = tiles_img;
        }
        plan_reduce(p, &pl);
        pl.halo_tile = true;
        return done(GR_CONV6);
    }
    if (gn) return fail(LD_ERR_ARG);
    pl.takes_skip_segment = p.conv && p.ksize == 3 && p.stride == 1 && p.Hv == p.Hs && p.Wv == p.Ws && p.SC1 == 0;
    if (!p.conv && p.K == V7_K && p.batch == 1 && !p.ln_swapped && p.bias_m == nullptr && p.rowvec == nullptr && p.bm == 0 && (p.bn == 0 || p.bn == 160) &&
        p.splitk == 0 && (p.n_valid <= 0 || p.n_valid >= p.N) && p.N % (p.act == 2 ? 160 : V7_NB) == 0 && (p.M + V7_BM - 1) / V7_BM >= 192 &&
        (p.act == 0 || (p.act == 2 && p.bias_n != nullptr && p.stat_out == nullptr && p.R == nullptr))) {
        pl.stat_parts = p.N / V7_NB;
        pl.grid_x = (unsigned)((p.M + V7_BM - 1) / V7_BM); pl.ln = p.ln_stat != nullptr;
        return done(GR_GEMM7);
    }
    {
        const bool conv3 = p.conv && p.ksize == 3;
        const bool shape_ok = !p.ln_swapped && p.bm == 0 && (p.bn == 0 || p.bn == 160) && p.N % V5_BN == 0 && p.K % V5_BK == 0 &&
                              p.K >= (p.act == 2 ? 1280 : conv3 ? 640 : 2560) && (p.n_valid == p.N || p.n_valid <= 0 || p.n_valid > p.N) &&
                              p.splitk == 0 && p.M >= 1024;
        const int tm5 = (p.M + V5_BM - 1) / V5_BM, tn5 = p.N / V5_BN;
        if (shape_ok && (long long)tm5 * tn5 * p.batch >= 192 && !(p.act == 2 && p.stat_out != nullptr)) {
            pl.ln = p.ln_stat != nullptr || p.stat_out != nullptr;
            if (p.conv && (pl.ln || p.act == 2)) return fail(LD_ERR_ARG);
            pl.stat_parts = 2 * tn5;
            pl.bm = V5_BM; pl.bn = V5_BN;
            pl.grid_x = (unsigned)(tm5 * tn5); pl.grid_z = (unsigned)p.batch;
            pl.xcd_gm = p.xcd_gm;
            if (!p.conv) {
                pl.xcd_gm = 0;
                if (p.batch == 1 && (tm5 * tn5) % 8 == 0 && p.M % V5_BM == 0) {
                    double best = 0;
                    for (int gm = 1; gm <= 8; gm <<= 1) {
                        const int gn5 = 8 / gm;
                        if (tm5 % gm || tn5 % gn5) continue;
                        const double cost = (double)p.M * gn5 + (double)p.N * gm;
                        if (pl.xcd_gm == 0 || cost < best) {
                            best = cost;
                            pl.xcd_gm = gm;
                        }
                    }
                }
            }
            return done(GR_GEMM5);
        }
    }
    int bn = p.bn ? p.bn : gemm_pick_bn(p.N);
    constexpr int skinny_max = 256;
    const bool skinny_ok = !p.conv && p.act != 2 && p.bn == 0 && p.bm == 0 && (p.N % 64) == 0;
    if (skinny_ok) {
        const long long t160 = (long long)((p.M + 63) / 64) * ((p.N + bn - 1) / bn) * p.batch;
        if (t160 <= skinny_max && (p.N + bn - 1) / bn <= 8) bn = 64;
    }
    bool skinny_conv1 = false;
    if (p.conv && p.ksize == 1 && p.act == 0 && p.bn == 0 && p.bm == 0 && p.splitk == 0 && p.batch == 1 && (p.N % 64) == 0 && p.SC1 == 0) {
        const long long t64 = (long long)((p.M + 63) / 64) * (p.N / 64);
        if (t64 > 128 && t64 <= 512 && p.K >= 1280 && p.K <= 3200) {
            bn = 64;
            skinny_conv1 = true;
        }
    }
    if (bn != 128 && bn != 160 && bn != 64) return fail(LD_ERR_ARG);
    if (p.act == 2 && (p.N % bn)) return fail(LD_ERR_SHAPE);
    const int tiles_n = (p.N + bn - 1) / bn;
    const int KT = (p.K + BK - 1) / BK;
    const int tiles128 = ((p.M + 127) / 128) * tiles_n * p.batch;
    const bool can_split = p.batch == 1 && p.partial != nullptr;
    const int sk_cap = p.K / 640 < 1 ? 1 : (p.K / 640 > 16 ? 16 : p.K / 640);
    int bm = p.bm, sk = p.splitk;
    if (bm == 0) {
        if (tiles128 >= 512) bm = 128;
        else if (p.K >= 4096 && can_split && (tiles128 >= 128 || (p.K >= 8192 && tiles128 >= 64))) bm = 128;
        else if (!p.conv && tiles128 >= 256) bm = 128;
        else bm = 64;
    }
    if (bn == 64) bm = 64;
    if (skinny_conv1) sk = 1;
    if (bm != 64 && bm != 128) return fail(LD_ERR_ARG);
    const int tiles = ((p.M + bm - 1) / bm) * tiles_n;
    const bool deep = p.conv && bm == 64 && bn == 160 && p.batch == 1 && p.splitk == 0 && (tiles <= 32 || (tiles >= 256 && tiles < 512));
    if (sk == 0) {
        sk = 1;
        if (can_split && tiles * p.batch < 512) {
            sk = ((deep ? 256 : 512) + tiles - 1) / tiles;
            if (sk > sk_cap) sk = sk_cap;
        }
    }
    if (sk > 1) {
        if (p.batch != 1 || p.partial == nullptr) return fail(LD_ERR_ARG);
        while (sk > 1 && (size_t)sk * p.M * p.N * sizeof(float) > p.partial_bytes) --sk;
        if (sk > KT) sk = KT;
    }
    if (p.stat_out != nullptr || p.ln_stat != nullptr) {
        if (p.act == 2 && p.stat_out != nullptr) return fail(LD_ERR_ARG);
        sk = 1;
        pl.stat_parts = tiles_n;
    }
    if (sk < 1) sk = 1;
    pl.bm = bm; pl.bn = bn; pl.splitk = sk;
    pl.grid_x = (unsigned)(tiles * sk); pl.grid_z = (unsigned)p.batch;
    pl.m_fastest = p.m_fastest;
    if (p.m_fastest < 0) {
        const int tiles_m = (p.M + bm - 1) / bm;
        pl.m_fastest = (!p.conv && p.batch == 1 && tiles_m >= 2 && tiles_m <= 8 && (long long)p.N * p.K * 2 >= (8ll << 20)) ? 1 : 0;
    }
    plan_reduce(p, &pl);
    const long long blocks = (long long)tiles * sk * p.batch;
    {
        const bool plain_2wg = bn == 64 && !p.conv && blocks > V4_MAX_BLOCKS && blocks <= 512 && p.K >= 640;
        const bool conv1_2wg = bn == 64 && p.conv && p.ksize == 1 && sk <= 1 && (long long)tiles * p.batch <= 512;
        pl.two_wg = plain_2wg || conv1_2wg;
        if (pl.two_wg) return done(GR_GEMM4);
    }
    if (!p.conv && blocks <= V4_MAX_BLOCKS) return done(GR_GEMM4);
    pl.deep = deep;
    return done(GR_GEMM3);
}

int gemm_run(const GemmParams& pin, const GemmPlan& pl, hipStream_t stream) {
    t_last_kernel = "";
    if (pl.status != LD_OK) return pl.status;
    if (pl.gn != (pin.gn_scale != nullptr) || (pl.gn && pin.gn_shift == nullptr)) return LD_ERR_ARG;
    GemmParams p = pin;
    if (p.stat_parts_out != nullptr) *p.stat_parts_out = pl.stat_parts;
    if (p.gn_part_done != nullptr) *p.gn_part_done = pl.gn_chunks;
    if (p.conv && p.pad < 0) p.pad = p.ksize >> 1;
    if (p.n_valid <= 0 || p.n_valid > p.N) p.n_valid = p.N;
    const dim3 grid(pl.grid_x, 1, pl.grid_z);
    t_last_kernel = pl.kernel;
    switch (pl.route) {
        case GR_CONV8:
            if (const int st = conv8_launch(p, pl.c8_S, stream); st != LD_OK) return st;
            break;
        case GR_CONV6:
            p.splitk = pl.splitk;
            if (pl.bn != 32) p.n_valid = p.N;
            if (pl.splitk == 1 && p.gn_part != nullptr) {
                if (pl.gn_chunks > 0) p.gn_P = pl.gn_chunks;
                else p.gn_part = nullptr;
            }
            if (pl.gn) {
                if (pl.bn == 256) launch_conv6<true, 256>(pl.wc, p, grid, stream);
                else if (pl.bn == 128) launch_conv6<true, 128, 512>(pl.wc, p, grid, stream);
                else launch_conv6<true>(pl.wc, p, grid, stream);
            } else if (pl.bn == 128) {
                launch_conv6<false, 128, 512>(pl.wc, p, grid, stream);
            } else if (pl.bn == 32) {
                launch_conv6<false, 32, 512>(pl.wc, p, grid, stream);
            } else if (pl.bn == 256) {
                if (pl.up) launch_conv6<false, 256, V5_BM, true>(pl.wc, p, grid, stream);
                else launch_conv6<false, 256>(pl.wc, p, grid, stream);
            } else {
                if (pl.up) launch_conv6<false, V5_BN, V5_BM, true>(pl.wc, p, grid, stream);
                else launch_conv6<false>(pl.wc, p, grid, stream);
            }
            break;
        case GR_GEMM7:
            if (pl.geglu && pl.ln) hipLaunchKernelGGL((gemm7_kernel<true, true>), grid, dim3(512), 0, stream, p);
            else if (pl.geglu) hipLaunchKernelGGL((gemm7_kernel<true, false>), grid, dim3(512), 0, stream, p);
            else if (pl.ln) hipLaunchKernelGGL((gemm7_kernel<false, true>), grid, dim3(512), 0, stream, p);
            else hipLaunchKernelGGL((gemm7_kernel<false, false>), grid, dim3(512), 0, stream, p);
            break;
        case GR_GEMM5:
            p.splitk = 1; p.bn = 160; p.xcd_gm = pl.xcd_gm;
            if (pl.conv) hipLaunchKernelGGL((gemm5_kernel<true, 0>), grid, dim3(512), 0, stream, p);
            else if (pl.geglu) hipLaunchKernelGGL((gemm5_kernel<false, 2>), grid, dim3(512), 0, stream, p);
            else if (pl.ln) hipLaunchKernelGGL((gemm5_kernel<false, 1>), grid, dim3(512), 0, stream, p);
            else hipLaunchKernelGGL((gemm5_kernel<false, 0>), grid, dim3(512), 0, stream, p);
            break;
        default:
            p.splitk = pl.splitk; p.bn = pl.bn; p.m_fastest = pl.m_fastest;
            if (pl.bn == 64) launch_cfg<64, 64>(p, pl, grid, stream);
            else if (pl.bm == 128 && pl.bn == 160) launch_cfg<128, 160>(p, pl, grid, stream);
            else if (pl.bm == 128 && pl.bn == 128) launch_cfg<128, 128>(p, pl, grid, stream);
            else if (pl.bm == 64 && pl.bn == 160) launch_cfg<64, 160>(p, pl, grid, stream);
            else launch_cfg<64, 128>(p, pl, grid, stream);
            break;
    }
    if (pl.reduce == GRD_GROUPNORM) {
        hipLaunchKernelGGL(splitk_reduce_gn_kernel, dim3(p.gn_P, p.M / p.gn_HW, 4), dim3(256), 0, stream, p);
    } else if (pl.reduce == GRD_PLAIN) {
        const int out_n = p.act == 2 ? p.N / 2 : p.N;
        const long long total = (long long)p.M * (out_n / 8);
        int blocks = (int)((total + 255) / 256);
        if (blocks > 2048) blocks = 2048;
        hipLaunchKernelGGL(splitk_reduce_kernel, dim3(blocks), dim3(256), 0, stream, p, pl.route == GR_CONV6 ? 160 : pl.bn);
    }
    return hipGetLastError() == hipSuccess ? LD_OK : LD_ERR_HIP;
}
```

### lightdiffusion_amd/csrc/kernels.h

```cpp
#pragma once
#include <cstdlib>
#include "common.h"
#include "gemm.h"

static inline int gn_num_chunks(int n_img, int HW) {
    const long long px = (long long)(n_img < 1 ? 1 : n_img) * HW;
    const int target = px <= 8192 ? 512 : (px <= 131072 ? 1024 : 2048);
    int p = target / (4 * (n_img < 1 ? 1 : n_img));
    if (p > HW / 8) p = HW / 8;
    if (p > 256) p = 256;
    return p < 1 ? 1 : p;
}
size_t groupnorm_workspace_bytes(int n_img, int HW);
int groupnorm_launch(const half_t* x1, int C1, const half_t* x2, int C2, int n_img, int HW, const half_t* gamma,
                     const half_t* beta, float eps, int silu, half_t* y, float* partial, hipStream_t stream, int stats_ready = 0);
int groupnorm_stats_launch(const half_t* x1, int C1, const half_t* x2, int C2, int n_img, int HW, float* partial, hipStream_t stream);
int groupnorm_scale_shift_launch(const half_t* x1, int C1, const half_t* x2, int C2, int n_img, int HW, const half_t* gamma, const half_t* beta,
                                 float eps, float* partial, float* scale, float* shift, hipStream_t stream, int stats_ready = 0);
int layernorm_launch(const half_t* x, const half_t* gamma, const half_t* beta, half_t* y, int rows, int C, float eps,
                     hipStream_t stream);
int softmax_rows_launch(half_t* s, int rows, int cols, long long ld, hipStream_t stream, int valid = 0);

struct AttnParams {
    const half_t* Q = nullptr;
    const half_t* K = nullptr;
    const half_t* Vt = nullptr;
    const half_t* V = nullptr;
    int ldv = 0;
    half_t* O = nullptr;
    int ldq = 0, ldk = 0, ldvt = 0, ldo = 0;
    long long sQ = 0, sK = 0, sV = 0, sO = 0;
    int B = 0, H = 0, Lq = 0, Lk = 0, d = 0;
    float scale = 1.0f;
    int causal = 0;
};
int attention_launch(const AttnParams& p, hipStream_t stream);
const char* attention_last_kernel_name();

int ln_fold_launch(const half_t* W, int N, int K, const half_t* gamma, const half_t* beta, const half_t* bias, half_t* Wout, half_t* bout,
                   float* wsum, hipStream_t stream);
int mlp_out_fold_launch(const half_t* Wpo, const half_t* W2, const half_t* b2, const half_t* bpo, int C, half_t* Wout, half_t* bout, hipStream_t stream);
int skip_fold_launch(const half_t* W2, const half_t* Wsk, const half_t* b2, const half_t* bsk, int N, int K9, int SC, half_t* Wout, half_t* bout,
                     hipStream_t stream);
struct SmallConvInArgs {
    const float* x = nullptr;
    const float* scale_sigma = nullptr;
    const half_t* pre_w = nullptr;
    const half_t* pre_b = nullptr;
    const half_t* w = nullptr;
    const half_t* b = nullptr;
    half_t* y = nullptr;
    int N = 0, Cin = 0, H = 0, W = 0, Cout = 0;
    long long dup_off = 0;
};
int small_conv_in_launch(const SmallConvInArgs& a, hipStream_t stream);

struct SmallConvOutArgs {
    const half_t* x = nullptr;
    const half_t* w = nullptr;
    const half_t* b = nullptr;
    int N = 0, H = 0, W = 0, Cin = 0, Cout = 0;
    int mode = 0;
    const float* x_in = nullptr;
    const float* sigma = nullptr;
    float* out = nullptr;
    int in_mod = 0;
};
int small_conv_out_launch(const SmallConvOutArgs& a, hipStream_t stream);

int vae_out_finish_launch(const half_t* t8, float* out, long long npix, int cout, hipStream_t stream);

int small_pointwise_launch(const half_t* x, const half_t* w, const half_t* b, float* out, int N, int HW, int C, hipStream_t stream);

int timestep_embed_launch(const float* sigma, const float* log_sigmas, int n_sig, int N, int dim, half_t* out, float* t_out,
                          hipStream_t stream, int sigma_mod = 0);

struct DupArgs {
    char* base[3] = {nullptr, nullptr, nullptr};
    unsigned long long bytes[3] = {0, 0, 0};
    int count = 0;
};
int dup_halves_launch(const DupArgs& a, hipStream_t stream);

int repack_conv3x3_launch(const void* src, int src_is_f32, int O, int I, half_t* dst, hipStream_t stream);
int repack_rows_launch(const void* src, int src_is_f32, int rows, int cols, half_t* dst, int geglu_bn, hipStream_t stream);
int ctx_pad_launch(const void* src, int src_is_f32, int n, int T, int Tp, int D, half_t* dst, hipStream_t stream);
int fill_half_launch(half_t* dst, size_t n, float v, hipStream_t stream);

int cfg_combine_launch(const float* den2, float* out, float cfg, size_t n_half, hipStream_t stream);
int axpby_launch(float* x, float a, const float* y, float b, const float* z, float c, size_t n, hipStream_t stream);
int hook_check_launch(const void* a, const void* b, size_t words_ab, const void* x, size_t half_words_x, const void* sigma, int half_sigma,
                      int* flags, int epoch, hipStream_t stream);
int bislerp_launch(const float* x, float* tmp, float* y, int n, int c, int h, int w, int h_new, int w_new, hipStream_t stream);
```

### lightdiffusion_amd/csrc/misc.hip

```cpp
#include "kernels.h"

namespace {

template <int CIN>
__global__ __launch_bounds__(256) void small_conv_in_kernel(const SmallConvInArgs a) {
    extern __shared__ __attribute__((aligned(16))) char smem_raw[];
    half_t* wl = reinterpret_cast<half_t*>(smem_raw);
    constexpr int KK = 9 * CIN;
    if ((KK & 3) == 0) {
        for (int i = threadIdx.x; i < a.Cout * KK / 4; i += blockDim.x) {
            const int o = (i * 4) / KK, k = i * 4 - o * KK;
            const half4 v = *reinterpret_cast<const half4*>(a.w + (long long)i * 4);
#pragma unroll
            for (int e = 0; e < 4; ++e) wl[(k + e) * a.Cout + o] = v[e];
        }
    } else {
        for (int i = threadIdx.x; i < a.Cout * KK; i += blockDim.x) {
            const int o = i / KK, k = i - o * KK;
            wl[k * a.Cout + o] = a.w[i];
        }
    }
    float pw[CIN][CIN], pb[CIN];
    if (a.pre_w != nullptr) {
#pragma unroll
// ... 402 lines not shown
    if (den2 == nullptr || out == nullptr) return LD_ERR_ARG;
    hipLaunchKernelGGL(cfg_combine_kernel, dim3(grid_for((long long)n_half, 256)), dim3(256), 0, stream, den2, out, cfg, n_half);
    return hipGetLastError() == hipSuccess ? LD_OK : LD_ERR_HIP;
}

int hook_check_launch(const void* a, const void* b, size_t words_ab, const void* x, size_t half_words_x, const void* sigma, int half_sigma,
                      int* flags, int epoch, hipStream_t stream) {
    if (flags == nullptr || (words_ab && (a == nullptr || b == nullptr)) || (half_words_x && x == nullptr) || (half_sigma && sigma == nullptr))
        return LD_ERR_ARG;
    if (half_sigma < 0 || half_sigma > 256) return LD_ERR_SHAPE;
    const long long total = (long long)(words_ab > half_words_x ? words_ab : half_words_x);
    hipLaunchKernelGGL(hook_check_kernel, dim3(grid_for(total > 0 ? total : 1, 256, 1024)), dim3(256), 0, stream, (const unsigned*)a,
                       (const unsigned*)b, words_ab, (const unsigned*)x, half_words_x, (const unsigned*)sigma, half_sigma, flags, epoch);
    return hipGetLastError() == hipSuccess ? LD_OK : LD_ERR_HIP;
}

int axpby_launch(float* x, float a, const float* y, float b, const float* z, float c, size_t n, hipStream_t stream) {
    if (x == nullptr) return LD_ERR_ARG;
    hipLaunchKernelGGL(axpby_kernel, dim3(grid_for((long long)n, 256)), dim3(256), 0, stream, x, a, y, b, z, c, n);
    return hipGetLastError() == hipSuccess ? LD_OK : LD_ERR_HIP;
}

namespace {
__global__ __launch_bounds__(256) void ln_fold_kernel(const half_t* __restrict__ W, int K, const half_t* __restrict__ gamma,
                                                      const half_t* __restrict__ beta, const half_t* __restrict__ bias, half_t* __restrict__ Wout,
                                                      half_t* __restrict__ bout, float* __restrict__ wsum) {
    __shared__ float red[2][256];
    const int n = blockIdx.x, tid = threadIdx.x;
    float s = 0.f, sb = 0.f;
    for (int k = tid; k < K; k += 256) {
        const float w = (float)W[(long long)n * K + k];
        const half_t wf = (half_t)(w * (float)gamma[k]);
        Wout[(long long)n * K + k] = wf;
        s += (float)wf;
        sb += w * (float)beta[k];
    }
    red[0][tid] = s;
    red[1][tid] = sb;
    __syncthreads();
    for (int o = 128; o > 0; o >>= 1) {
        if (tid < o) {
            red[0][tid] += red[0][tid + o];
            red[1][tid] += red[1][tid + o];
        }
        __syncthreads();
    }
    if (tid == 0) {
        wsum[n] = red[0][0];
        bout[n] = (half_t)((bias != nullptr ? (float)bias[n] : 0.f) + red[1][0]);
    }
}
}

int ln_fold_launch(const half_t* W, int N, int K, const half_t* gamma, const half_t* beta, const half_t* bias, half_t* Wout, half_t* bout,
                   float* wsum, hipStream_t stream) {
    if (W == nullptr || gamma == nullptr || beta == nullptr || Wout == nullptr || bout == nullptr || wsum == nullptr || N <= 0 || K <= 0)
        return LD_ERR_ARG;
    hipLaunchKernelGGL(ln_fold_kernel, dim3(N), dim3(256), 0, stream, W, K, gamma, beta, bias, Wout, bout, wsum);
    return hipGetLastError() == hipSuccess ? LD_OK : LD_ERR_HIP;
}

namespace {
__global__ __launch_bounds__(256) void bislerp_axis_kernel(const float* __restrict__ x, float* __restrict__ y, int n, int c, int h,
                                                           int w, int len_new, int axis_w) {
    const int ho = axis_w ? h : len_new, wo = axis_w ? len_new : w;
    const long long total = (long long)n * ho * wo;
    for (long long idx = (long long)blockIdx.x * blockDim.x + threadIdx.x; idx < total; idx += (long long)gridDim.x * blockDim.x) {
    const int xo = (int)(idx % wo), yo = (int)((idx / wo) % ho), b = (int)(idx / ((long long)wo * ho));
    const int len_old = axis_w ? w : h, o = axis_w ? xo : yo;
    float pos = ((float)o + 0.5f) * ((float)len_old / (float)len_new) - 0.5f;
    pos = fmaxf(pos, 0.f);
    int lo = (int)floorf(pos);
    if (lo > len_old - 1) lo = len_old - 1;
    const int hi = lo + 1 < len_old ? lo + 1 : len_old - 1;
    const float r = lo >= len_old - 1 ? 0.f : pos - (float)lo;
    const long long plane = (long long)h * w;
    const float* pa = x + (long long)b * c * plane + (axis_w ? (long long)yo * w + lo : (long long)lo * w + xo);
    const float* pb = x + (long long)b * c * plane + (axis_w ? (long long)yo * w + hi : (long long)hi * w + xo);
    float na = 0.f, nb = 0.f, dot = 0.f;
    for (int ch = 0; ch < c; ++ch) {
        const float a = pa[ch * plane], bb = pb[ch * plane];
        na += a * a;
        nb += bb * bb;
        dot += a * bb;
    }
    na = sqrtf(na);
    nb = sqrtf(nb);
    const float ia = na > 0.f ? 1.f / na : 0.f, ib = nb > 0.f ? 1.f / nb : 0.f;
    dot *= ia * ib;
    const float om = acosf(dot), so = sinf(om);
    const float wa = sinf((1.f - r) * om) / so * ia, wb = sinf(r * om) / so * ib;
    const float mag = na * (1.f - r) + nb * r;
    const long long oplane = (long long)ho * wo;
    float* py = y + (long long)b * c * oplane + (long long)yo * wo + xo;
    for (int ch = 0; ch < c; ++ch) {
        const float a = pa[ch * plane], bb = pb[ch * plane];
        float v = (wa * a + wb * bb) * mag;
        if (dot > 1.f - 1e-5f) v = a;
        if (dot < 1e-5f - 1.f) v = a * (1.f - r) + bb * r;
        py[ch * oplane] = v;
    }
    }
}
}

int bislerp_launch(const float* x, float* tmp, float* y, int n, int c, int h, int w, int h_new, int w_new, hipStream_t stream) {
    if (x == nullptr || tmp == nullptr || y == nullptr || n <= 0 || c <= 0 || h <= 0 || w <= 0 || h_new <= 0 || w_new <= 0) return LD_ERR_ARG;
    hipLaunchKernelGGL(bislerp_axis_kernel, dim3(grid_for((long long)n * h * w_new, 256)), dim3(256), 0, stream, x, tmp, n, c, h, w, w_new, 1);
    hipLaunchKernelGGL(bislerp_axis_kernel, dim3(grid_for((long long)n * h_new * w_new, 256)), dim3(256), 0, stream, tmp, y, n, c, h, w_new,
                       h_new, 0);
    return hipGetLastError() == hipSuccess ? LD_OK : LD_ERR_HIP;
}

namespace {
__global__ __launch_bounds__(256) void mlp_out_fold_kernel(const half_t* __restrict__ Wpo, const half_t* __restrict__ W2, const half_t* __restrict__ b2,
                                                           const half_t* __restrict__ bpo, int C, half_t* __restrict__ Wout, half_t* __restrict__ bout) {
    extern __shared__ float wrow[];
    const int n = blockIdx.x, tid = threadIdx.x;
    const int H = 4 * C, K = 5 * C;
    for (int c = tid; c < C; c += 256) wrow[c] = (float)Wpo[(long long)n * C + c];
    __syncthreads();
    for (int k = tid; k < H; k += 256) {
        float s = 0.f;
        for (int c = 0; c < C; ++c) s += wrow[c] * (float)W2[(long long)c * H + k];
        Wout[(long long)n * K + k] = (half_t)s;
    }
    for (int c = tid; c < C; c += 256) Wout[(long long)n * K + H + c] = Wpo[(long long)n * C + c];
    if (tid == 0) {
        float s = (float)bpo[n];
        for (int c = 0; c < C; ++c) s += wrow[c] * (float)b2[c];
        bout[n] = (half_t)s;
    }
}
}

int mlp_out_fold_launch(const half_t* Wpo, const half_t* W2, const half_t* b2, const half_t* bpo, int C, half_t* Wout, half_t* bout, hipStream_t stream) {
    if (Wpo == nullptr || W2 == nullptr || b2 == nullptr || bpo == nullptr || Wout == nullptr || bout == nullptr || C <= 0) return LD_ERR_ARG;
    hipLaunchKernelGGL(mlp_out_fold_kernel, dim3(C), dim3(256), (size_t)C * sizeof(float), stream, Wpo, W2, b2, bpo, C, Wout, bout);
    return hipGetLastError() == hipSuccess ? LD_OK : LD_ERR_HIP;
}

namespace {
__global__ __launch_bounds__(256) void skip_fold_kernel(const uint4* __restrict__ W2, const uint4* __restrict__ Wsk, const half_t* __restrict__ b2,
                                                        const half_t* __restrict__ bsk, int N, int K9c, int SCc, uint4* __restrict__ Wout, half_t* __restrict__ bout) {
    const int Kc = K9c + SCc;
    const long long total = (long long)N * Kc;
    for (long long q = (long long)blockIdx.x * blockDim.x + threadIdx.x; q < total; q += (long long)gridDim.x * blockDim.x) {
        const int n = (int)(q / Kc), c = (int)(q - (long long)n * Kc);
        Wout[q] = c < K9c ? W2[(long long)n * K9c + c] : Wsk[(long long)n * SCc + (c - K9c)];
    }
    const int t = blockIdx.x * blockDim.x + threadIdx.x;
    if (t < N) bout[t] = (half_t)((float)b2[t] + (float)bsk[t]);
}
}

int skip_fold_launch(const half_t* W2, const half_t* Wsk, const half_t* b2, const half_t* bsk, int N, int K9, int SC, half_t* Wout, half_t* bout,
                     hipStream_t stream) {
    if (W2 == nullptr || Wsk == nullptr || b2 == nullptr || bsk == nullptr || Wout == nullptr || bout == nullptr || N <= 0 || K9 <= 0 || SC <= 0 ||
        (K9 & 7) || (SC & 7))
        return LD_ERR_ARG;
    const long long total = (long long)N * ((K9 + SC) / 8);
    int blocks = (int)((total + 255) / 256);
    if (blocks > 4096) blocks = 4096;
    if (blocks * 256 < N) blocks = (N + 255) / 256;
    hipLaunchKernelGGL(skip_fold_kernel, dim3(blocks), dim3(256), 0, stream, reinterpret_cast<const uint4*>(W2), reinterpret_cast<const uint4*>(Wsk), b2, bsk, N,
                       K9 / 8, SC / 8, reinterpret_cast<uint4*>(Wout), bout);
    return hipGetLastError() == hipSuccess ? LD_OK : LD_ERR_HIP;
}
```

### lightdiffusion_amd/csrc/unet.hip

```cpp
#include <cstring>

#include "runtime.h"
#include "../../include/ld_mi355x.h"

namespace {

struct ResW {
    std::string prefix;
    int cin = 0, cout = 0, emb_off = 0;
    int gn1_g, gn1_b, c1_w, c1_b, emb_w, emb_b, gn2_g, gn2_b, c2_w, c2_b, sk_w = -1, sk_b = -1;
    size_t f_c2_w = 0, f_c2_b = 0;
};
struct StW {
    int c = 0, bn = 0, ctx_slot = 0;
    size_t f_qk_w = 0, f_q2_w = 0, f_ff1_w = 0, f_qk_b = 0, f_q2_b = 0, f_ff1_b = 0, f_qk_s = 0, f_q2_s = 0,
           f_ff1_s = 0;
    size_t f_mo_w = 0, f_mo_b = 0;
    int gn_g, gn_b, pin_w, pin_b, ln1_g, ln1_b, q1_w, k1_w, v1_w, o1_w, o1_b, ln2_g, ln2_b, q2_w, k2_w, v2_w, o2_w, o2_b, ln3_g,
        ln3_b, ff1_w, ff1_b, ff2_w, ff2_b, pout_w, pout_b;
};
struct ConvW {
    int cin = 0, cout = 0, w = -1, b = -1;
};
enum LayerKind { L_CONV_IN, L_RES, L_ST, L_DOWN, L_UP };
struct Layer {
    int kind, idx;
};
struct Feat {
    half_t* p;
    int C, H, W;
    float* gn = nullptr;
    int gnP = 0;
};

}

struct ld_unet {
    ld_unet_config cfg;
    ParamTable pt;
    std::vector<ResW> res;
    std::vector<StW> st;
    std::vector<ConvW> convs;
    std::vector<std::vector<Layer>> in_blocks, out_blocks;
    std::vector<Layer> mid_block;
    int te0_w, te0_b, te2_w, te2_b, outn_g, outn_b, outc_w, outc_b;
    int emb_total = 0, ted = 0;
    Arena arena;
    char* ws_base = nullptr;
    size_t ws_bytes = 0;
    float* splitk_ws = nullptr;
    size_t splitk_bytes = 0;
    float* log_sigmas = nullptr;
    int max_n = 0, max_h = 0, max_w = 0, max_tok = 0;
    half_t* ctx16 = nullptr;
    std::vector<half_t*> ctx_k, ctx_vt;
    int ctx_n = 0, ctx_tok = 0, ctx_tpad = 0;
    int plan_n = 0, plan_h = 0, plan_w = 0, plan_pair = 0;
    int last_launches = 0;
    double last_flops = 0.0;
    int* sync_ws = nullptr;
    struct W8 { int slot, N, Cin; size_t off; };
    std::vector<W8> w8_list;
    std::vector<long long> w8_of_slot;
    char* w8_base = nullptr;
    size_t w8_bytes = 0;
    const half_t* w8(int slot) const {
        return (w8_base != nullptr && slot >= 0 && slot < (int)w8_of_slot.size() && w8_of_slot[slot] >= 0) ? reinterpret_cast<const half_t*>(w8_base + w8_of_slot[slot]) : nullptr;
    }
    void want_w8(int slot, int N, int Cin) {
        if (!conv8_weight_eligible(N, Cin)) return;
        w8_list.push_back({slot, N, Cin, w8_bytes});
        w8_bytes += (conv8_weight_bytes(N, Cin) + 255) / 256 * 256;
    }
    Timing timing;
    bool want_timing = false;
    char* fold_base = nullptr;
    size_t fold_bytes = 0;
    bool fold_dirty = true;
};

namespace {

std::string S(const char* fmt, int a = 0, int b = 0) {
    char buf[160];
    snprintf(buf, sizeof buf, fmt, a, b);
    return buf;
}

int add_res(ld_unet* u, const std::string& p, int cin, int cout) {
    ParamTable& t = u->pt;
    ResW r;
    r.prefix = p;
    r.cin = cin;
    r.cout = cout;
    r.gn1_g = t.add(p + ".in_layers.0.weight", PK_VEC, {cin});
    r.gn1_b = t.add(p + ".in_layers.0.bias", PK_VEC, {cin});
    r.c1_w = t.add(p + ".in_layers.2.weight", PK_CONV3, {cout, cin, 3, 3});
    r.c1_b = t.add(p + ".in_layers.2.bias", PK_VEC, {cout});
    u->want_w8(r.c1_w, cout, cin);
    r.gn2_g = t.add(p + ".out_layers.0.weight", PK_VEC, {cout});
    r.gn2_b = t.add(p + ".out_layers.0.bias", PK_VEC, {cout});
    r.c2_w = t.add(p + ".out_layers.3.weight", PK_CONV3, {cout, cout, 3, 3});
    r.c2_b = t.add(p + ".out_layers.3.bias", PK_VEC, {cout});
    u->want_w8(r.c2_w, cout, cout);
    if (cin != cout) {
        r.sk_w = t.add(p + ".skip_connection.weight", PK_MAT, {cout, cin, 1, 1});
        r.sk_b = t.add(p + ".skip_connection.bias", PK_VEC, {cout});
        size_t& fb = u->fold_bytes;
        r.f_c2_w = fb;
        fb += ((size_t)cout * (9 * cout + cin) * sizeof(half_t) + 255) / 256 * 256;
        r.f_c2_b = fb;
        fb += ((size_t)cout * sizeof(half_t) + 255) / 256 * 256;
    }
    r.emb_off = u->emb_total;
    u->emb_total += cout;
    u->res.push_back(r);
    return (int)u->res.size() - 1;
}

int add_st(ld_unet* u, const std::string& p, int c) {
    ParamTable& t = u->pt;
    const int ctx = u->cfg.context_dim;
    StW s;
    s.c = c;
    s.bn = gemm_pick_bn(8 * c);
    s.ctx_slot = (int)u->st.size();
    s.gn_g = t.add(p + ".norm.weight", PK_VEC, {c});
    s.gn_b = t.add(p + ".norm.bias", PK_VEC, {c});
    s.pin_w = t.add(p + ".proj_in.weight", PK_MAT, {c, c, 1, 1});
    s.pin_b = t.add(p + ".proj_in.bias", PK_VEC, {c});
    const std::string b = p + ".transformer_blocks.0";
    s.ln1_g = t.add(b + ".norm1.weight", PK_VEC, {c});
    s.ln1_b = t.add(b + ".norm1.bias", PK_VEC, {c});
    s.q1_w = t.add(b + ".attn1.to_q.weight", PK_MAT, {c, c});
    s.k1_w = t.add(b + ".attn1.to_k.weight", PK_MAT, {c, c}, 16);
    s.v1_w = t.add(b + ".attn1.to_v.weight", PK_MAT, {c, c}, 16);
    s.o1_w = t.add(b + ".attn1.to_out.0.weight", PK_MAT, {c, c});
    s.o1_b = t.add(b + ".attn1.to_out.0.bias", PK_VEC, {c});
    s.ln2_g = t.add(b + ".norm2.weight", PK_VEC, {c});
    s.ln2_b = t.add(b + ".norm2.bias", PK_VEC, {c});
    s.q2_w = t.add(b + ".attn2.to_q.weight", PK_MAT, {c, c});
    s.k2_w = t.add(b + ".attn2.to_k.weight", PK_MAT, {c, ctx});
    s.v2_w = t.add(b + ".attn2.to_v.weight", PK_MAT, {c, ctx});
    s.o2_w = t.add(b + ".attn2.to_out.0.weight", PK_MAT, {c, c});
    s.o2_b = t.add(b + ".attn2.to_out.0.bias", PK_VEC, {c});
    s.ln3_g = t.add(b + ".norm3.weight", PK_VEC, {c});
    s.ln3_b = t.add(b + ".norm3.bias", PK_VEC, {c});
    s.ff1_w = t.add(b + ".ff.net.0.proj.weight", PK_GEGLU_W, {8 * c, c}, 256, s.bn);
    s.ff1_b = t.add(b + ".ff.net.0.proj.bias", PK_GEGLU_B, {8 * c}, 256, s.bn);
    s.ff2_w = t.add(b + ".ff.net.2.weight", PK_MAT, {c, 4 * c});
    s.ff2_b = t.add(b + ".ff.net.2.bias", PK_VEC, {c});
    s.pout_w = t.add(p + ".proj_out.weight", PK_MAT, {c, c, 1, 1});
    s.pout_b = t.add(p + ".proj_out.bias", PK_VEC, {c});
    {
        size_t& fb = u->fold_bytes;
        auto take = [&](size_t bytes) {
            const size_t o = fb;
            fb += (bytes + 255) / 256 * 256;
            return o;
        };
        const size_t C = (size_t)c;
        s.f_qk_w = take(3 * C * C * sizeof(half_t));
        s.f_q2_w = take(C * C * sizeof(half_t));
        s.f_ff1_w = take(8 * C * C * sizeof(half_t));
        s.f_qk_b = take(3 * C * sizeof(half_t));
        s.f_q2_b = take(C * sizeof(half_t));
        s.f_ff1_b = take(8 * C * sizeof(half_t));
        s.f_qk_s = take(3 * C * sizeof(float));
        s.f_q2_s = take(C * sizeof(float));
        s.f_ff1_s = take(8 * C * sizeof(float));
        s.f_mo_w = take(5 * C * C * sizeof(half_t));
        s.f_mo_b = take(C * sizeof(half_t));
    }
    u->st.push_back(s);
    return (int)u->st.size() - 1;
}

int add_conv(ld_unet* u, const std::string& p, int cin, int cout) {
    ConvW c;
    c.cin = cin;
    c.cout = cout;
    c.w = u->pt.add(p + ".weight", PK_CONV3, {cout, cin, 3, 3});
    c.b = u->pt.add(p + ".bias", PK_VEC, {cout});
    u->convs.push_back(c);
    return (int)u->convs.size() - 1;
}

int build(ld_unet* u) {
    const ld_unet_config& c = u->cfg;
    if (c.num_levels < 1 || c.num_levels > 8 || c.model_channels % 32 || c.num_heads < 1) return LD_ERR_ARG;
    const int mc = c.model_channels;
    u->ted = mc * 4;
    ParamTable& t = u->pt;
    u->te0_w = t.add("time_embed.0.weight", PK_MAT, {u->ted, mc});
    u->te0_b = t.add("time_embed.0.bias", PK_VEC, {u->ted});
    u->te2_w = t.add("time_embed.2.weight", PK_MAT, {u->ted, u->ted});
    u->te2_b = t.add("time_embed.2.bias", PK_VEC, {u->ted});
    u->in_blocks.push_back({{L_CONV_IN, add_conv(u, "input_blocks.0.0", c.in_channels, mc)}});
    int ch = mc, idx = 1, td = 0;
    std::vector<int> chans{mc};
    for (int lvl = 0; lvl < c.num_levels; ++lvl) {
        for (int r = 0; r < c.num_res_blocks[lvl]; ++r) {
            std::vector<Layer> L;
            L.push_back({L_RES, add_res(u, S("input_blocks.%d.0", idx), ch, c.channel_mult[lvl] * mc)});
            ch = c.channel_mult[lvl] * mc;
            if (c.transformer_depth[td++] > 0) L.push_back({L_ST, add_st(u, S("input_blocks.%d.1", idx), ch)});
            u->in_blocks.push_back(L);
            chans.push_back(ch);
            ++idx;
        }
        if (lvl != c.num_levels - 1) {
            u->in_blocks.push_back({{L_DOWN, add_conv(u, S("input_blocks.%d.0.op", idx), ch, ch)}});
            chans.push_back(ch);
            ++idx;
        }
    }
    u->mid_block.push_back({L_RES, add_res(u, "middle_block.0", ch, ch)});
    if (c.transformer_depth_middle > 0) u->mid_block.push_back({L_ST, add_st(u, "middle_block.1", ch)});
    u->mid_block.push_back({L_RES, add_res(u, "middle_block.2", ch, ch)});
    int n_out = 0;
    for (int lvl = 0; lvl < c.num_levels; ++lvl) n_out += c.num_res_blocks[lvl] + 1;
    int tdo = n_out;
    idx = 0;
    for (int lvl = c.num_levels - 1; lvl >= 0; --lvl) {
        for (int i = 0; i <= c.num_res_blocks[lvl]; ++i) {
            const int ich = chans.back();
            chans.pop_back();
            std::vector<Layer> L;
            L.push_back({L_RES, add_res(u, S("output_blocks.%d.0", idx), ch + ich, mc * c.channel_mult[lvl])});
            ch = mc * c.channel_mult[lvl];
            int j = 1;
            if (c.transformer_depth_output[--tdo] > 0) {
                L.push_back({L_ST, add_st(u, S("output_blocks.%d.%d", idx, j), ch)});
                ++j;
            }
            if (lvl && i == c.num_res_blocks[lvl]) {
                L.push_back({L_UP, add_conv(u, S("output_blocks.%d.%d.conv", idx, j), ch, ch)});
                u->want_w8(u->convs.back().w, ch, ch);
            }
            u->out_blocks.push_back(L);
            ++idx;
        }
    }
    u->outn_g = t.add("out.0.weight", PK_VEC, {ch});
    u->outn_b = t.add("out.0.bias", PK_VEC, {ch});
    u->outc_w = t.add("out.2.weight", PK_CONV3, {c.out_channels, mc, 3, 3});
    u->outc_b = t.add("out.2.bias", PK_VEC, {c.out_channels});
    for (size_t i = 0; i < u->res.size(); ++i)
        u->res[i].emb_w = t.add(u->res[i].prefix + ".emb_layers.1.weight", PK_MAT, {u->res[i].cout, u->ted}, i == 0 ? 256 : 16);
    for (size_t i = 0; i < u->res.size(); ++i)
        u->res[i].emb_b = t.add(u->res[i].prefix + ".emb_layers.1.bias", PK_VEC, {u->res[i].cout}, i == 0 ? 256 : 16);
    return t.finalize();
}

struct Run {
    ld_unet* u;
    Exec ex;
    int n;
    int n_alloc = 0;
    bool pair_pending = false;
    const half_t* emb_all;
    half_t* P(int slot) const { return u->pt.ptr(slot); }
    int na() const { return n_alloc > 0 ? n_alloc : n; }
    void dup(void* base, size_t half_bytes) {
        ex.launches += 1;
        ex.t_begin(KC_MISC, 0.0, 1, "dup", (long long)half_bytes, 0, 0, 1);
        if (!ex.dry && ex.status == LD_OK &&
            hipMemcpyAsync(static_cast<char*>(base) + half_bytes, base, half_bytes, hipMemcpyDeviceToDevice, ex.stream) != hipSuccess)
            ex.note(LD_ERR_HIP);
        ex.t_end("hipMemcpyAsync(pair)");
    }

    void want_stats(GemmParams& p, float* buf, int HW, int* done) {
        p.gn_part = buf;
        p.gn_P = gn_num_chunks(n, HW);
        p.gn_HW = HW;
        p.gn_ppb = (HW + p.gn_P - 1) / p.gn_P;
        p.gn_part_done = done;
    }

    half_t* conv3(const half_t* x1, int C1, const half_t* x2, int C2, int Hs, int Ws, int Hv, int Wv, int stride, int wslot, int bslot,
                  int cout, const half_t* rowvec, int ldrv, const half_t* R, half_t* out, int* Ho_, int* Wo_, int ksize = 3, float* stats = nullptr,
                  int* stats_done = nullptr) {
        const int Ho = ksize == 3 ? (Hv - 1) / stride + 1 : Hv, Wo = ksize == 3 ? (Wv - 1) / stride + 1 : Wv;
        GemmParams p;
        p.conv = 1;
        p.ksize = ksize;
        p.A = x1; p.A2 = x2; p.C1 = C1; p.C2 = C2;
        p.Hs = Hs; p.Ws = Ws; p.Hv = Hv; p.Wv = Wv; p.Ho = Ho; p.Wo = Wo; p.stride = stride;
        p.W = P(wslot); p.ldw = ksize * ksize * (C1 + C2);
        p.W8 = ksize == 3 ? u->w8(wslot) : nullptr;
        p.M = n * Ho * Wo; p.N = cout; p.K = ksize * ksize * (C1 + C2);
        p.bias_n = P(bslot);
        p.rowvec = rowvec; p.rows_per_vec = Ho * Wo; p.ldrv = ldrv;
        p.R = R; p.ldr = cout;
        p.C = out; p.ldc = cout;
        if (stats != nullptr) want_stats(p, stats, Ho * Wo, stats_done);
        ex.gemm(p);
        if (Ho_) *Ho_ = Ho;
        if (Wo_) *Wo_ = Wo;
        return out;
    }

    void linear(const half_t* x, int lda, int wslot, int bslot, const half_t* R, half_t* y, int M, int N, int K, int act = 0, int bn = 0) {
        GemmParams p;
        p.A = x; p.lda = lda;
        p.W = P(wslot); p.ldw = K;
        p.M = M; p.N = N; p.K = K;
        p.bias_n = bslot >= 0 ? P(bslot) : nullptr;
        p.R = R; p.ldr = (act == 2 ? N / 2 : N);
        p.act = act; p.bn = bn;
        p.C = y; p.ldc = (act == 2 ? N / 2 : N);
        ex.gemm(p);
    }

    Feat resblock(const ResW& r, const half_t* x1, int C1, const half_t* x2, int C2, int H, int W, float* in_stats = nullptr, int in_P = 0) {
        Arena& ar = *ex.arena;
        const size_t M = (size_t)na() * H * W;
        half_t* out = ar.halfs(M * r.cout);
        float* gno = reinterpret_cast<float*>(ar.alloc(groupnorm_workspace_bytes(na(), H * W)));
        int gno_done = 0;
        if (C2 != 0) in_stats = nullptr;
        const size_t mk = ar.mark();
        auto conv_params = [&](const half_t* a1, int c1, const half_t* a2, int c2, int wslot, int bslot, const half_t* rowvec, int ldrv, const half_t* R,
                               half_t* dst) {
            GemmParams p;
            p.conv = 1; p.ksize = 3;
            p.A = a1; p.A2 = a2; p.C1 = c1; p.C2 = c2;
            p.Hs = H; p.Ws = W; p.Hv = H; p.Wv = W; p.Ho = H; p.Wo = W; p.stride = 1;
            p.W = P(wslot); p.ldw = 9 * (c1 + c2);
            p.W8 = u->w8(wslot);
            p.M = n * H * W; p.N = r.cout; p.K = 9 * (c1 + c2);
            p.bias_n = P(bslot);
            p.rowvec = rowvec; p.rows_per_vec = H * W; p.ldrv = ldrv;
            p.R = R; p.ldr = r.cout;
            p.C = dst; p.ldc = r.cout;
            return p;
        };
        half_t* g1 = ar.halfs(M * r.cin);
        half_t* h1 = ar.halfs(M * r.cout);
        const half_t* skip = x1;
        bool fold_skip = false;
        if (r.sk_w >= 0) {
            fold_skip = u->fold_base != nullptr && ex.conv_takes_skip_segment(conv_params(h1, r.cout, nullptr, 0, r.c2_w, r.c2_b, nullptr, 0, nullptr, out));
            half_t* sk = (!fold_skip || ex.dry) ? ar.halfs(M * r.cout) : nullptr;
            if (!fold_skip) {
                conv3(x1, C1, x2, C2, H, W, H, W, 1, r.sk_w, r.sk_b, r.cout, nullptr, 0, nullptr, sk, nullptr, nullptr, 1);
                skip = sk;
            }
        }
        float* gnp = reinterpret_cast<float*>(ar.alloc(groupnorm_workspace_bytes(na(), H * W)));
        int gnp_done = 0;
        {
            GemmParams c1 = conv_params(x1, C1, x2, C2, r.c1_w, r.c1_b, emb_all + r.emb_off, u->emb_total, nullptr, h1);
            want_stats(c1, gnp, H * W, &gnp_done);
            ex.gn_silu_conv(c1, n, H * W, P(r.gn1_g), P(r.gn1_b), 1e-5f, g1, in_stats, in_P);
        }
        half_t* g2 = g1;
        if (r.cout > r.cin) g2 = ar.halfs(M * r.cout);
        {
            GemmParams c2 = conv_params(h1, r.cout, nullptr, 0, r.c2_w, r.c2_b, nullptr, 0, skip, out);
            if (fold_skip) {
                c2.S1 = x1; c2.SC1 = C1; c2.S2 = x2; c2.SC2 = C2;
                c2.W = reinterpret_cast<const half_t*>(u->fold_base + r.f_c2_w);
                c2.K = 9 * r.cout + r.cin; c2.ldw = c2.K;
                c2.bias_n = reinterpret_cast<const half_t*>(u->fold_base + r.f_c2_b);
                c2.R = nullptr;
                c2.W8 = nullptr;
            }
            want_stats(c2, gno, H * W, &gno_done);
            ex.gn_silu_conv(c2, n, H * W, P(r.gn2_g), P(r.gn2_b), 1e-5f, g2, gnp_done ? gnp : nullptr, gnp_done);
        }
        ar.release(mk);
        return {out, r.cout, H, W, gno_done ? gno : nullptr, gno_done};
    }

    Feat transformer(const StW& s, const half_t* x, int H, int W, float* in_stats = nullptr, int in_P = 0) {
        Arena& ar = *ex.arena;
        const int C = s.c, L = H * W, heads = u->cfg.num_heads, d = C / heads;
        int M = n * L;
        const size_t Ma = (size_t)na() * L;
        half_t* out = ar.halfs(Ma * C);
        float* gno = reinterpret_cast<float*>(ar.alloc(groupnorm_workspace_bytes(na(), L)));
        int gno_done = 0;
        const size_t mk = ar.mark();
        half_t* g = ar.halfs(Ma * C);
        ex.groupnorm(x, C, nullptr, 0, n, L, P(s.gn_g), P(s.gn_b), 1e-6f, 0, g, in_stats, in_P);
        half_t* t = ar.halfs(Ma * C);
        half_t* qkv = ar.halfs(Ma * 3 * C);
        half_t* ao = ar.halfs(Ma * C);
        half_t* ff = nullptr;
        float* stat = reinterpret_cast<float*>(ar.alloc((size_t)((C + 63) / 64) * Ma * 2 * sizeof(float)));
        int parts = 0;
        char* fb = u->fold_base;
        auto producer = [&](const half_t* x_, int lda, int wslot, int bslot, const half_t* R, int K) {
            GemmParams p;
            p.A = x_; p.lda = lda;
            p.W = P(wslot); p.ldw = K;
            p.M = M; p.N = C; p.K = K;
            p.bias_n = P(bslot);
            p.R = R; p.ldr = C;
            p.C = t; p.ldc = C;
            p.stat_out = stat;
            p.stat_parts_out = &parts;
            ex.gemm(p);
        };
        auto ln_args = [&](GemmParams& p, size_t wsum_off) {
            p.ln_stat = stat; p.ln_parts = parts; p.ln_rows = M;
            p.ln_inv_c = 1.0f / (float)C; p.ln_eps = 1e-5f;
            p.ln_wsum = reinterpret_cast<const float*>(fb + wsum_off);
        };
        producer(g, C, s.pin_w, s.pin_b, nullptr, C);
        {
            GemmParams p;
            p.A = t; p.lda = C;
            p.W = reinterpret_cast<const half_t*>(fb + s.f_qk_w); p.ldw = C;
            p.M = M; p.N = 3 * C; p.K = C;
            p.C = qkv; p.ldc = 3 * C;
            p.bias_n = reinterpret_cast<const half_t*>(fb + s.f_qk_b);
            ln_args(p, s.f_qk_s);
            ex.gemm(p);
        }
        {
            AttnParams a;
            a.Q = qkv; a.ldq = 3 * C; a.sQ = (long long)L * 3 * C;
            a.K = qkv + C; a.ldk = 3 * C; a.sK = (long long)L * 3 * C;
            a.V = qkv + 2 * C; a.ldv = 3 * C; a.sV = (long long)L * 3 * C;
            a.O = ao; a.ldo = C; a.sO = (long long)L * C;
            a.B = n; a.H = heads; a.Lq = L; a.Lk = L; a.d = d;
            a.scale = 1.0f / sqrtf((float)d);
            ex.attention(a);
        }
        const bool split_here = pair_pending;
        producer(ao, C, s.o1_w, s.o1_b, t, C);
        half_t* q2 = qkv;
        {
            GemmParams p;
            p.A = t; p.lda = C;
            p.W = reinterpret_cast<const half_t*>(fb + s.f_q2_w); p.ldw = C;
            p.M = M; p.N = C; p.K = C;
            p.C = q2; p.ldc = C;
            p.bias_n = reinterpret_cast<const half_t*>(fb + s.f_q2_b);
            ln_args(p, s.f_q2_s);
            ex.gemm(p);
        }
        if (split_here) {
            const size_t hb = (size_t)M * C * sizeof(half_t);
            DupArgs da;
            da.count = 3;
            da.base[0] = reinterpret_cast<char*>(t); da.base[1] = reinterpret_cast<char*>(q2); da.base[2] = reinterpret_cast<char*>(const_cast<half_t*>(x));
            da.bytes[0] = da.bytes[1] = da.bytes[2] = hb;
            ex.launches += 1;
            ex.t_begin(KC_MISC, 0.0, 1, "dup3", (long long)hb, 0, 0, 1);
            if (!ex.dry && ex.status == LD_OK) ex.note(dup_halves_launch(da, ex.stream));
            ex.t_end("dup_halves_kernel");
            pair_pending = false;
            n = n_alloc;
            M = n * L;
        }
        {
            const int Tp = u->ctx_tpad;
            AttnParams a;
            a.Q = q2; a.ldq = C; a.sQ = (long long)L * C;
            a.K = u->ctx_k[s.ctx_slot]; a.ldk = C; a.sK = (long long)Tp * C;
            a.Vt = u->ctx_vt[s.ctx_slot]; a.ldvt = Tp; a.sV = (long long)C * Tp;
            a.O = ao; a.ldo = C; a.sO = (long long)L * C;
            a.B = n; a.H = heads; a.Lq = L; a.Lk = u->ctx_tok; a.d = d;
            a.scale = 1.0f / sqrtf((float)d);
            ex.attention(a);
        }
        producer(ao, C, s.o2_w, s.o2_b, t, C);
        ff = ar.halfs(Ma * 4 * C);
        {
            GemmParams p;
            p.A = t; p.lda = C;
            p.W = reinterpret_cast<const half_t*>(fb + s.f_ff1_w); p.ldw = C;
            p.M = M; p.N = 8 * C; p.K = C;
            p.bias_n = reinterpret_cast<const half_t*>(fb + s.f_ff1_b);
            p.act = 2; p.bn = s.bn;
            p.C = ff; p.ldc = 4 * C; p.ldr = 4 * C;
            ln_args(p, s.f_ff1_s);
            ex.gemm(p);
        }
        {
            GemmParams p;
            p.conv = 1; p.ksize = 1;
            p.A = ff; p.A2 = t; p.C1 = 4 * C; p.C2 = C;
            p.Hs = p.Hv = p.Ho = H; p.Ws = p.Wv = p.Wo = W; p.stride = 1;
            p.W = reinterpret_cast<const half_t*>(fb + s.f_mo_w); p.ldw = 5 * C;
            p.M = M; p.N = C; p.K = 5 * C;
            p.bias_n = reinterpret_cast<const half_t*>(fb + s.f_mo_b);
            p.R = x; p.ldr = C;
            p.C = out; p.ldc = C;
            want_stats(p, gno, L, &gno_done);
            ex.gemm(p);
        }
        ar.release(mk);
        return {out, C, H, W, gno_done ? gno : nullptr, gno_done};
    }
};

int fold_layernorms(ld_unet* u, hipStream_t stream) {
    for (const StW& s : u->st) {
        const int C = s.c;
        char* fb = u->fold_base;
        auto H = [&](size_t off) { return reinterpret_cast<half_t*>(fb + off); };
        auto F = [&](size_t off) { return reinterpret_cast<float*>(fb + off); };
        const half_t* P_q1 = u->pt.ptr(s.q1_w);
        int st = ln_fold_launch(P_q1, 3 * C, C, u->pt.ptr(s.ln1_g), u->pt.ptr(s.ln1_b), nullptr, H(s.f_qk_w), H(s.f_qk_b), F(s.f_qk_s), stream);
        if (st == LD_OK) st = ln_fold_launch(u->pt.ptr(s.q2_w), C, C, u->pt.ptr(s.ln2_g), u->pt.ptr(s.ln2_b), nullptr, H(s.f_q2_w), H(s.f_q2_b), F(s.f_q2_s), stream);
        if (st == LD_OK) st = ln_fold_launch(u->pt.ptr(s.ff1_w), 8 * C, C, u->pt.ptr(s.ln3_g), u->pt.ptr(s.ln3_b), u->pt.ptr(s.ff1_b), H(s.f_ff1_w), H(s.f_ff1_b), F(s.f_ff1_s), stream);
        if (st == LD_OK) st = mlp_out_fold_launch(u->pt.ptr(s.pout_w), u->pt.ptr(s.ff2_w), u->pt.ptr(s.ff2_b), u->pt.ptr(s.pout_b), C, H(s.f_mo_w), H(s.f_mo_b), stream);
        if (st != LD_OK) return st;
    }
    for (const ResW& r : u->res) {
        if (r.sk_w < 0) continue;
        const int st = skip_fold_launch(u->pt.ptr(r.c2_w), u->pt.ptr(r.sk_w), u->pt.ptr(r.c2_b), u->pt.ptr(r.sk_b), r.cout, 9 * r.cout, r.cin,
                                        reinterpret_cast<half_t*>(u->fold_base + r.f_c2_w), reinterpret_cast<half_t*>(u->fold_base + r.f_c2_b), stream);
        if (st != LD_OK) return st;
    }
    u->fold_dirty = false;
    return LD_OK;
}

int derive_conv8_weights(ld_unet* u, hipStream_t stream) {
    for (const ld_unet::W8& w : u->w8_list) {
        const int st = conv8_repack_launch(u->pt.ptr(w.slot), w.N, w.Cin, reinterpret_cast<half_t*>(u->w8_base + w.off), stream);
        if (st != LD_OK) return st;
    }
    return LD_OK;
}

int run_forward(ld_unet* u, bool dry, const float* x, const float* sigma, float* out, int n, int h, int w, int eps_only, hipStream_t stream,
                size_t* dry_peak = nullptr, bool pair = false) {
    if (!dry && u->fold_dirty) {
        if (u->w8_base != nullptr) {
            const int st = derive_conv8_weights(u, stream);
            if (st != LD_OK) return st;
        }
        {
            const int st = fold_layernorms(u, stream);
            if (st != LD_OK) return st;
        }
        u->fold_dirty = false;
    }
    if (pair && (n & 1)) return LD_ERR_SHAPE;
    Run R;
    R.u = u;
    R.n = n;
    R.n_alloc = n;
    Exec& ex = R.ex;
    ex.stream = stream;
    ex.dry = dry;
    Arena plan;
    ex.arena = dry ? &plan : &u->arena;
    ex.splitk_ws = u->splitk_ws;
    ex.splitk_bytes = u->splitk_bytes;
    ex.sync_ws = u->sync_ws;
    if (u->want_timing && !dry) {
        u->timing.reset();
        ex.timing = &u->timing;
    }
    Arena& ar = *ex.arena;
    ar.release(0);
    const ld_unet_config& c = u->cfg;
    const int mc = c.model_channels, ted = u->ted;
    const int in_mod = pair ? n / 2 : 0;
    if (pair) R.pair_pending = true;

    half_t* temb = ar.halfs((size_t)n * mc);
    ex.launches += 1;
    ex.t_begin(KC_MISC, 0.0, 1);
    if (!dry) ex.note(timestep_embed_launch(sigma, u->log_sigmas, 1000, n, mc, temb, nullptr, stream, in_mod));
    ex.t_end("timestep_embed_kernel");
    half_t* e1 = ar.halfs((size_t)n * ted);
    R.linear(temb, mc, u->te0_w, u->te0_b, nullptr, e1, n, ted, mc, 1);
    half_t* semb = ar.halfs((size_t)n * ted);
    R.linear(e1, ted, u->te2_w, u->te2_b, nullptr, semb, n, ted, ted, 1);
    half_t* emb_all = ar.halfs((size_t)n * u->emb_total);
    R.linear(semb, ted, u->res[0].emb_w, u->res[0].emb_b, nullptr, emb_all, n, u->emb_total, ted);
    R.emb_all = emb_all;

    auto run_layers = [&](const std::vector<Layer>& layers, Feat f, const half_t* x2, int C2, int outH, int outW) -> Feat {
        for (const Layer& L : layers) {
            switch (L.kind) {
                case L_RES: {
                    f = R.resblock(u->res[L.idx], f.p, f.C, x2, C2, f.H, f.W, f.gn, f.gnP);
                    x2 = nullptr;
                    C2 = 0;
                    break;
                }
                case L_ST: f = R.transformer(u->st[L.idx], f.p, f.H, f.W, f.gn, f.gnP); break;
                case L_DOWN: {
                    const ConvW& cw = u->convs[L.idx];
                    const int Ho = (f.H - 1) / 2 + 1, Wo = (f.W - 1) / 2 + 1;
                    if (R.pair_pending) {
                        R.dup(const_cast<half_t*>(f.p), (size_t)R.n * f.H * f.W * f.C * sizeof(half_t));
                        R.pair_pending = false;
                        R.n = n;
                    }
                    half_t* o = ar.halfs((size_t)n * Ho * Wo * cw.cout);
                    float* gno = reinterpret_cast<float*>(ar.alloc(groupnorm_workspace_bytes(n, Ho * Wo)));
                    int gno_done = 0;
                    R.conv3(f.p, f.C, nullptr, 0, f.H, f.W, f.H, f.W, 2, cw.w, cw.b, cw.cout, nullptr, 0, nullptr, o, nullptr, nullptr, 3, gno, &gno_done);
                    f = {o, cw.cout, Ho, Wo, gno_done ? gno : nullptr, gno_done};
                    break;
                }
                case L_UP: {
                    const ConvW& cw = u->convs[L.idx];
                    const int Hv = outH > 0 ? outH : f.H * 2, Wv = outW > 0 ? outW : f.W * 2;
                    half_t* o = ar.halfs((size_t)n * Hv * Wv * cw.cout);
                    R.conv3(f.p, f.C, nullptr, 0, f.H, f.W, Hv, Wv, 1, cw.w, cw.b, cw.cout, nullptr, 0, nullptr, o, nullptr, nullptr);
                    f = {o, cw.cout, Hv, Wv};
                    break;
                }
                default: break;
            }
        }
        return f;
    };

    std::vector<Feat> hs;
    Feat f{nullptr, 0, h, w};
    {
        const ConvW& cw = u->convs[u->in_blocks[0][0].idx];
        half_t* o = ar.halfs((size_t)n * h * w * mc);
        if (R.pair_pending) R.n = n / 2;
        SmallConvInArgs a;
        a.x = x; a.scale_sigma = sigma; a.w = u->pt.ptr(cw.w); a.b = u->pt.ptr(cw.b); a.y = o;
        a.N = R.n; a.Cin = c.in_channels; a.H = h; a.W = w; a.Cout = mc;
        if (R.pair_pending) a.dup_off = (long long)R.n * h * w * mc;
        ex.launches += 1;
        ex.flops += 2.0 * R.n * h * w * mc * 9.0 * c.in_channels;
        ex.t_begin(KC_MISC, 2.0 * R.n * h * w * mc * 9.0 * c.in_channels, 1);
        if (!dry) ex.note(small_conv_in_launch(a, stream));
        ex.t_end("small_conv_in_kernel");
        f = {o, mc, h, w};
        hs.push_back(f);
    }
    for (size_t b = 1; b < u->in_blocks.size(); ++b) {
        f = run_layers(u->in_blocks[b], f, nullptr, 0, 0, 0);
        if (R.pair_pending && b == 1) {
            R.dup(const_cast<half_t*>(f.p), (size_t)R.n * f.H * f.W * f.C * sizeof(half_t));
            R.pair_pending = false;
            R.n = n;
            f.gn = nullptr;
            f.gnP = 0;
        }
        hs.push_back(f);
    }
    if (R.pair_pending) {
        R.pair_pending = false;
        R.n = n;
    }
    f = run_layers(u->mid_block, f, nullptr, 0, 0, 0);
    for (size_t b = 0; b < u->out_blocks.size(); ++b) {
        const Feat skip = hs.back();
        hs.pop_back();
        if (skip.H != f.H || skip.W != f.W) ex.note(LD_ERR_SHAPE);
        const int oh = hs.empty() ? 0 : hs.back().H, ow = hs.empty() ? 0 : hs.back().W;
        f = run_layers(u->out_blocks[b], f, skip.p, skip.C, oh, ow);
    }
    {
        half_t* g = ar.halfs((size_t)n * f.H * f.W * f.C);
        ex.groupnorm(f.p, f.C, nullptr, 0, n, f.H * f.W, u->pt.ptr(u->outn_g), u->pt.ptr(u->outn_b), 1e-5f, 1, g, f.gn, f.gnP);
        SmallConvOutArgs a;
        a.x = g; a.w = u->pt.ptr(u->outc_w); a.b = u->pt.ptr(u->outc_b);
        a.N = n; a.H = f.H; a.W = f.W; a.Cin = f.C; a.Cout = c.out_channels;
        a.mode = eps_only ? 2 : 0;
        a.x_in = x; a.sigma = sigma; a.out = out; a.in_mod = in_mod;
        ex.launches += 1;
        ex.flops += 2.0 * n * f.H * f.W * f.C * 9.0 * c.out_channels;
        ex.t_begin(KC_MISC, 2.0 * n * f.H * f.W * f.C * 9.0 * c.out_channels, 1);
        if (!dry) ex.note(small_conv_out_launch(a, stream));
        ex.t_end("small_conv_out_kernel");
    }
    u->last_launches = ex.launches;
    u->last_flops = ex.flops;
    if (dry_peak) *dry_peak = ar.peak;
    return ex.status;
}

}

extern "C" {

int ld_unet_create(const ld_unet_config* cfg, ld_unet** out) {
    if (cfg == nullptr || out == nullptr) return LD_ERR_ARG;
    ld_unet* u = new ld_unet();
    u->cfg = *cfg;
    const int st = build(u);
    if (st != LD_OK) {
        u->pt.destroy();
        delete u;
        return st;
    }
    std::vector<float> ls(1000);
    {
        const double b0 = sqrt(0.00085), b1 = sqrt(0.012);
        double ac = 1.0;
        for (int i = 0; i < 1000; ++i) {
            const double sb = b0 + (b1 - b0) * (double)i / 999.0;
            ac *= 1.0 - sb * sb;
            ls[i] = (float)log(sqrt((1.0 - ac) / ac));
        }
    }
    u->w8_of_slot.assign(u->pt.slots.size(), -1);
    for (const ld_unet::W8& w : u->w8_list) u->w8_of_slot[w.slot] = (long long)w.off;
    if (u->w8_bytes > 0 && hipMalloc((void**)&u->w8_base, u->w8_bytes) != hipSuccess) u->w8_base = nullptr;
    if (u->fold_bytes > 0 && hipMalloc((void**)&u->fold_base, u->fold_bytes) != hipSuccess) {
        u->pt.destroy();
        delete u;
        return LD_ERR_HIP;
    }
    if (hipMalloc((void**)&u->sync_ws, LD_SYNC_INTS * sizeof(int)) != hipSuccess || hipMemset(u->sync_ws, 0, LD_SYNC_INTS * sizeof(int)) != hipSuccess ||
        hipMalloc((void**)&u->log_sigmas, 1000 * sizeof(float)) != hipSuccess ||
        hipMemcpy(u->log_sigmas, ls.data(), 1000 * sizeof(float), hipMemcpyHostToDevice) != hipSuccess) {
        u->pt.destroy();
        delete u;
        return LD_ERR_HIP;
    }
    *out = u;
    return LD_OK;
}

void ld_unet_destroy(ld_unet* u) {
    if (u == nullptr) return;
    u->pt.destroy();
    u->timing.destroy();
    if (u->ws_base) (void)hipFree(u->ws_base);
    if (u->log_sigmas) (void)hipFree(u->log_sigmas);
    if (u->sync_ws) (void)hipFree(u->sync_ws);
    if (u->w8_base) (void)hipFree(u->w8_base);
    if (u->fold_base) (void)hipFree(u->fold_base);
    delete u;
}

int ld_unet_param_count(const ld_unet* u) { return u ? (int)u->pt.slots.size() : 0; }

int ld_unet_param_info(const ld_unet* u, int i, const char** name, int* ndim, int64_t shape[4]) {
    if (u == nullptr || i < 0 || i >= (int)u->pt.slots.size()) return LD_ERR_ARG;
    const ParamSlot& s = u->pt.slots[i];
    if (name) *name = s.name.c_str();
    if (ndim) *ndim = s.ndim;
    if (shape)
        for (int k = 0; k < 4; ++k) shape[k] = s.shape[k];
    return LD_OK;
}

int ld_unet_load_param(ld_unet* u, const char* name, const void* src, int dtype, void* stream) {
    if (u == nullptr || name == nullptr) return LD_ERR_ARG;
    u->fold_dirty = true;
    return u->pt.load(name, src, dtype, (hipStream_t)stream);
}

size_t ld_unet_workspace_bytes(const ld_unet* u) { return u ? u->ws_bytes : 0; }
size_t ld_unet_weight_bytes(const ld_unet* u) { return u ? u->pt.bytes + (u->fold_base ? u->fold_bytes : 0) + (u->w8_base ? u->w8_bytes : 0) : 0; }

int ld_unet_reserve(ld_unet* u, int max_n, int max_h, int max_w, int max_tok) {
    if (u == nullptr || max_n < 1 || max_h < 1 || max_w < 1 || max_tok < 1) return LD_ERR_ARG;
    if (u->ws_base) {
        (void)hipFree(u->ws_base);
        u->ws_base = nullptr;
    }
    u->arena = Arena();
// ... 162 lines not shown
```

### lightdiffusion_amd/ops.py

```python
from __future__ import annotations

import math
from typing import Optional

import torch

from ._lib import F16, F32, check, lib


def _stream() -> int:
    return torch.cuda.current_stream().cuda_stream


def _p(t: Optional[torch.Tensor]) -> Optional[int]:
    if t is None:
        return None
    assert t.is_cuda and t.is_contiguous(), "device-resident contiguous tensors only"
    return t.data_ptr()


def last_kernel() -> str:
    return lib().ld_op_last_kernel().decode()


_WS = {}


def _ws(nbytes: int, device) -> torch.Tensor:
    d = torch.device(device)
    idx = d.index if d.index is not None else torch.cuda.current_device()
    n = max(nbytes, 256)
    if torch.cuda.is_current_stream_capturing():
        return torch.empty(n, dtype=torch.uint8, device=device)
    key = (idx, torch.cuda.current_stream(idx).cuda_stream)
    buf = _WS.get(key)
    if buf is None or buf.numel() < n:
        buf = torch.empty(n, dtype=torch.uint8, device=device)
        _WS[key] = buf
    return buf[:n]


def linear(x: torch.Tensor, weight: torch.Tensor, bias: Optional[torch.Tensor] = None, residual: Optional[torch.Tensor] = None,
           act: str = "none", alpha: float = 1.0) -> torch.Tensor:
    code = {"none": 0, "silu": 1, "geglu": 2, "quick_gelu": 3}[act]
    K = x.shape[-1]
    N = weight.shape[0]
    M = x.numel() // K
    y = torch.empty(*x.shape[:-1], N // 2 if code == 2 else N, dtype=torch.float16, device=x.device)
    ws = _ws(64 << 20, x.device)
    check(lib().ld_op_linear(_p(x), _p(weight), _p(bias), _p(residual), _p(y), M, N, K, alpha, code, _p(ws), ws.numel(), _stream()),
          "ld_op_linear")
    return y


def linear_ln(x: torch.Tensor, w_prod: torch.Tensor, b_prod: Optional[torch.Tensor], gamma: torch.Tensor, beta: torch.Tensor,
              weight: torch.Tensor, bias: Optional[torch.Tensor], eps: float = 1e-5):
    M, C = x.shape
    N = weight.shape[0]
    t = torch.empty(M, C, dtype=torch.float16, device=x.device)
    y = torch.empty(M, N, dtype=torch.float16, device=x.device)
    ws = _ws(2 * N * C + 8 * N + 8 * ((C + 63) // 64) * M + 4096, x.device)
    check(lib().ld_op_linear_ln(_p(x), _p(w_prod), _p(b_prod), _p(gamma), _p(beta), _p(weight), _p(bias), _p(t), _p(y), M, C, N, eps,
                                _p(ws), ws.numel(), _stream()), "ld_op_linear_ln")
    return t, y


def linear_ln_geglu(x: torch.Tensor, w_prod: torch.Tensor, b_prod: Optional[torch.Tensor], gamma: torch.Tensor, beta: torch.Tensor,
                    weight: torch.Tensor, bias: torch.Tensor, eps: float = 1e-5):
    M, C = x.shape
    N = weight.shape[0]
    t = torch.empty(M, C, dtype=torch.float16, device=x.device)
    y = torch.empty(M, N // 2, dtype=torch.float16, device=x.device)
    ws = _ws(4 * N * C + 12 * N + 8 * ((C + 63) // 64) * M + 4096, x.device)
    check(lib().ld_op_linear_ln_geglu(_p(x), _p(w_prod), _p(b_prod), _p(gamma), _p(beta), _p(weight), _p(bias), _p(t), _p(y), M, C, N, eps,
                                      _p(ws), ws.numel(), _stream()), "ld_op_linear_ln_geglu")
    return t, y


def repack_conv_weight(w_oihw: torch.Tensor) -> torch.Tensor:
    O, I, kh, kw = w_oihw.shape
    w_oihw = w_oihw.contiguous()
    out = torch.empty(O, kh * kw * I, dtype=torch.float16, device=w_oihw.device)
    if kh == 3:
        check(lib().ld_op_repack_conv(_p(w_oihw), F32 if w_oihw.dtype == torch.float32 else F16, O, I, _p(out), _stream()),
              "ld_op_repack_conv")
    else:
        out.copy_(w_oihw.reshape(O, I))
    return out


def conv2d(x: torch.Tensor, w_packed: torch.Tensor, bias: Optional[torch.Tensor], ksize: int = 3, stride: int = 1,
           x2: Optional[torch.Tensor] = None, out_hw: Optional[tuple] = None, rowvec: Optional[torch.Tensor] = None,
           residual: Optional[torch.Tensor] = None) -> torch.Tensor:
    n, h, w, c1 = x.shape
    c2 = 0 if x2 is None else x2.shape[-1]
    hv, wv = (h, w) if out_hw is None else out_hw
    cout = w_packed.shape[0]
    ho = (hv - 1) // stride + 1 if ksize == 3 else hv
    wo = (wv - 1) // stride + 1 if ksize == 3 else wv
    y = torch.empty(n, ho, wo, cout, dtype=torch.float16, device=x.device)
    ws = _ws(192 << 20, x.device)
    check(lib().ld_op_conv(_p(x), c1, _p(x2), c2, n, h, w, hv, wv, stride, ksize, _p(w_packed), _p(bias), _p(rowvec), _p(residual),
                           _p(y), cout, _p(ws), ws.numel(), _stream()), "ld_op_conv")
    return y


def conv2d_skip(x: torch.Tensor, w_packed: torch.Tensor, bias: torch.Tensor, s1: torch.Tensor, s2: Optional[torch.Tensor], w_skip: torch.Tensor,
                b_skip: torch.Tensor, rowvec: Optional[torch.Tensor] = None) -> torch.Tensor:
    n, h, w, c = x.shape
    sc1 = s1.shape[-1]
    sc2 = 0 if s2 is None else s2.shape[-1]
    cout = w_packed.shape[0]
    y = torch.empty(n, h, w, cout, dtype=torch.float16, device=x.device)
    ws = _ws(lib().ld_op_conv_skip_ws_bytes(c, sc1, sc2, cout), x.device)
    check(lib().ld_op_conv_skip(_p(x), c, n, h, w, _p(w_packed), _p(bias), _p(s1), sc1, _p(s2), sc2, _p(w_skip), _p(b_skip), _p(rowvec), _p(y), cout,
                                _p(ws), ws.numel(), _stream()), "ld_op_conv_skip")
    return y


def conv2d_gn_partials(x: torch.Tensor, w_packed: torch.Tensor, bias: Optional[torch.Tensor], out_hw: Optional[tuple] = None,
                       residual: Optional[torch.Tensor] = None):
    import ctypes
    n, h, w, c = x.shape
    hv, wv = (h, w) if out_hw is None else out_hw
    cout = w_packed.shape[0]
    y = torch.empty(n, hv, wv, cout, dtype=torch.float16, device=x.device)
    part = torch.zeros(lib().ld_op_conv_gn_partials_floats(n, hv * wv), dtype=torch.float32, device=x.device)
    chunks = ctypes.c_int(0)
    ws = _ws(192 << 20, x.device)
    check(lib().ld_op_conv_gn_partials(_p(x), c, n, h, w, hv, wv, _p(w_packed), _p(bias), _p(residual), _p(y), cout, _p(part), ctypes.byref(chunks),
                                       _p(ws), ws.numel(), _stream()), "ld_op_conv_gn_partials")
    if chunks.value == 0:
        return y, None
    return y, part[: n * chunks.value * 64].view(n, chunks.value, 32, 2)


def group_norm_silu_conv2d(x: torch.Tensor, gamma: torch.Tensor, beta: torch.Tensor, eps: float, w_packed: torch.Tensor,
                           bias: Optional[torch.Tensor], x2: Optional[torch.Tensor] = None, rowvec: Optional[torch.Tensor] = None,
                           residual: Optional[torch.Tensor] = None) -> torch.Tensor:
    n, h, w, c1 = x.shape
    c2 = 0 if x2 is None else x2.shape[-1]
    cout = w_packed.shape[0]
    y = torch.empty(n, h, w, cout, dtype=torch.float16, device=x.device)
    ws = _ws(lib().ld_op_groupnorm_conv_ws_bytes(c1, c2, n, h, w, cout), x.device)
    check(lib().ld_op_groupnorm_conv(_p(x), c1, _p(x2), c2, n, h, w, _p(gamma), _p(beta), eps, _p(w_packed), _p(bias), _p(rowvec), _p(residual),
                                     _p(y), cout, _p(ws), ws.numel(), _stream()), "ld_op_groupnorm_conv")
    return y


def group_norm(x: torch.Tensor, gamma: torch.Tensor, beta: torch.Tensor, eps: float, silu: bool = False,
               x2: Optional[torch.Tensor] = None) -> torch.Tensor:
    n, c1 = x.shape[0], x.shape[-1]
    hw = x.numel() // (n * c1)
    c2 = 0 if x2 is None else x2.shape[-1]
    y = torch.empty(*x.shape[:-1], c1 + c2, dtype=torch.float16, device=x.device)
    ws = _ws(lib().ld_op_groupnorm_ws_bytes(n, hw), x.device)
    check(lib().ld_op_groupnorm(_p(x), c1, _p(x2), c2, n, hw, _p(gamma), _p(beta), eps, int(silu), _p(y), _p(ws), _stream()),
          "ld_op_groupnorm")
    return y


def layer_norm(x: torch.Tensor, gamma: torch.Tensor, beta: torch.Tensor, eps: float = 1e-5) -> torch.Tensor:
    c = x.shape[-1]
    y = torch.empty_like(x)
    check(lib().ld_op_layernorm(_p(x), _p(gamma), _p(beta), _p(y), x.numel() // c, c, eps, _stream()), "ld_op_layernorm")
    return y


def attention(q: torch.Tensor, k: torch.Tensor, v: torch.Tensor, heads: int, causal: bool = False) -> torch.Tensor:
    b, lq, c = q.shape
    lk = k.shape[1]
    d = c // heads
    lkp = (lk + 7) // 8 * 8
    vt = torch.zeros(b, c, lkp, dtype=torch.float16, device=q.device)
    vt[:, :, :lk] = v.transpose(1, 2)
    o = torch.empty_like(q)
    check(lib().ld_op_attention(_p(q), c, _p(k.contiguous()), c, _p(vt), lkp, _p(o), c, b, heads, lq, lk, d, 1.0 / math.sqrt(d), int(causal), _stream()),
          "ld_op_attention")
    return o


def attention_qkv(qkv: torch.Tensor, heads: int, causal: bool = False) -> torch.Tensor:
    b, l, c3 = qkv.shape
    c = c3 // 3
    d = c // heads
    o = torch.empty(b, l, c, dtype=torch.float16, device=qkv.device)
    base = qkv.data_ptr()
    check(lib().ld_op_attention_rowv(base, c3, base + 2 * c, c3, base + 4 * c, c3, _p(o), c, b, heads, l, l, d, 1.0 / math.sqrt(d), int(causal),
                                     _stream()), "ld_op_attention_rowv")
    return o


def attention_rowv(q: torch.Tensor, k: torch.Tensor, v: torch.Tensor, heads: int, causal: bool = False) -> torch.Tensor:
    b, lq, c = q.shape
    lk = k.shape[1]
    d = c // heads
    o = torch.empty_like(q)
    check(lib().ld_op_attention_rowv(_p(q), c, _p(k.contiguous()), c, _p(v.contiguous()), c, _p(o), c, b, heads, lq, lk, d, 1.0 / math.sqrt(d), int(causal),
                                     _stream()), "ld_op_attention_rowv")
    return o


def softmax_rows_(s: torch.Tensor) -> torch.Tensor:
    cols = s.shape[-1]
    check(lib().ld_op_softmax_rows(_p(s), s.numel() // cols, cols, _stream()), "ld_op_softmax_rows")
    return s


def timestep_embed(sigma: torch.Tensor, log_sigmas: torch.Tensor, dim: int):
    n = sigma.numel()
    out = torch.empty(n, dim, dtype=torch.float16, device=sigma.device)
    t = torch.empty(n, dtype=torch.float32, device=sigma.device)
    check(lib().ld_op_timestep_embed(_p(sigma), _p(log_sigmas), log_sigmas.numel(), n, dim, _p(out), _p(t), _stream()),
          "ld_op_timestep_embed")
    return out, t


def cfg_combine(den2: torch.Tensor, cfg: float) -> torch.Tensor:
    half = den2.shape[0] // 2
    out = torch.empty_like(den2[:half])
    check(lib().ld_op_cfg_combine(_p(den2), _p(out), float(cfg), out.numel(), _stream()), "ld_op_cfg_combine")
    return out


def axpby_(x: torch.Tensor, a: float, y: Optional[torch.Tensor] = None, b: float = 0.0, z: Optional[torch.Tensor] = None,
           c: float = 0.0) -> torch.Tensor:
    check(lib().ld_op_axpby(_p(x), float(a), _p(y), float(b), _p(z), float(c), x.numel(), _stream()), "ld_op_axpby")
    return x


def bislerp(samples: torch.Tensor, width: int, height: int) -> torch.Tensor:
    x = samples.float().contiguous()
    n, c, h, w = x.shape
    tmp = torch.empty(n, c, h, width, dtype=torch.float32, device=x.device)
    y = torch.empty(n, c, height, width, dtype=torch.float32, device=x.device)
    check(lib().ld_op_bislerp(_p(x), _p(tmp), _p(y), n, c, h, w, height, width, _stream()), "ld_op_bislerp")
    return y.to(samples.dtype)


import torch.nn as nn


def _to_f16_cl(x: torch.Tensor) -> torch.Tensor:
    return x.to(torch.float16).contiguous(memory_format=torch.channels_last)


class _NoInit:
    def reset_parameters(self):
        return None


class Linear(_NoInit, nn.Module):
    def __init__(self, in_features, out_features, bias=True, device=None, dtype=None):
        super().__init__()
        self.in_features, self.out_features = in_features, out_features
        self.weight = nn.Parameter(torch.empty(out_features, in_features, device=device, dtype=dtype), requires_grad=False)
# ... 84 lines not shown
```

Measured before the change: 60.21 steps/s.

## Fold nearest-upsample into 3x3 conv as four-phase 2x2 convs

Adds a folded weight set that rewrites nearest-2x upsample followed by a 3x3 conv as four 2x2 convolutions, one per output phase, over the low-resolution input. The upsample conv in the UNet decoder routes to a gemm5 variant whose epilogue scatters phase outputs into the interleaved high-res layout. An optional split-K reduce kernel does the same scatter. This cuts the reduction work from 9 taps to 4 per output and avoids reading the upsampled activation. In exchange it needs extra folded-weight memory and an untimed fold pass, and the new route bypasses the existing conv8 path.

Measured after the change: 61.50 steps/s (median of 6 runs). 1.02x the previous value.

```diff
diff --git a/include/ld_mi355x.h b/include/ld_mi355x.h
--- a/include/ld_mi355x.h
+++ b/include/ld_mi355x.h
@@ -90,6 +90,9 @@
 size_t ld_op_conv_skip_ws_bytes(int c, int sc1, int sc2, int cout);
 int ld_op_conv_skip(const void* x, int c, int n, int h, int w, const void* wt, const void* bias, const void* s1, int sc1, const void* s2, int sc2,
                     const void* wskip, const void* bskip, const void* rowvec, void* y, int cout, void* ws, size_t ws_bytes, void* stream);
+int ld_op_upconv2x_fold(const void* wt, int cout, int cin, void* wfold, void* stream);
+int ld_op_upconv2x(const void* x, int c, int n, int h, int w, int hv, int wv, const void* wt, const void* wfold, const void* bias, void* y, int cout,
+                   void* ws, size_t ws_bytes, void* stream);
 size_t ld_op_conv_gn_partials_floats(int n, int hw);
 int ld_op_conv_gn_partials(const void* x, int c, int n, int h, int w, int hv, int wv, const void* wt, const void* bias,
                            const void* residual, void* y, int cout, float* part, int* chunks, void* ws, size_t ws_bytes, void* stream);
diff --git a/lightdiffusion_amd/_lib.py b/lightdiffusion_amd/_lib.py
--- a/lightdiffusion_amd/_lib.py
+++ b/lightdiffusion_amd/_lib.py
@@ -71,6 +71,8 @@
     "ld_op_groupnorm_conv_ws_bytes": (_Z, [_I, _I, _I, _I, _I, _I]),
     "ld_op_groupnorm_conv": (_I, [_P, _I, _P, _I, _I, _I, _I, _P, _P, _F, _P, _P, _P, _P, _P, _I, _P, _Z, _P]),
     "ld_op_repack_conv": (_I, [_P, _I, _I, _I, _P, _P]),
+    "ld_op_upconv2x_fold": (_I, [_P, _I, _I, _P, _P]),
+    "ld_op_upconv2x": (_I, [_P, _I, _I, _I, _I, _I, _I, _P, _P, _P, _P, _I, _P, _Z, _P]),
     "ld_op_conv_skip_ws_bytes": (_Z, [_I, _I, _I, _I]),
     "ld_op_conv_skip": (_I, [_P, _I, _I, _I, _I, _P, _P, _P, _I, _P, _I, _P, _P, _P, _P, _I, _P, _Z, _P]),
     "ld_op_groupnorm_ws_bytes": (_Z, [_I, _I]),
diff --git a/lightdiffusion_amd/csrc/capi.hip b/lightdiffusion_amd/csrc/capi.hip
--- a/lightdiffusion_amd/csrc/capi.hip
+++ b/lightdiffusion_amd/csrc/capi.hip
@@ -96,7 +96,7 @@
 
 static int op_conv(const void* x1, int c1, const void* x2, int c2, int n, int h, int w, int hv, int wv, int stride, int ksize,
                    const void* wt, const void* bias, const void* rowvec, const void* residual, void* y, int cout, void* ws,
-                   size_t ws_bytes, void* stream, float* gn_part, int* gn_chunks) {
+                   size_t ws_bytes, void* stream, float* gn_part, int* gn_chunks, const void* wup = nullptr) {
     if (stride < 1 || (ksize != 1 && ksize != 3)) return LD_ERR_ARG;
     GemmParams p;
     if (gn_part != nullptr) {
@@ -115,6 +115,7 @@
     p.Wo = ksize == 3 ? (wv - 1) / stride + 1 : wv;
     p.K = ksize * ksize * (c1 + c2);
     p.W = (const half_t*)wt; p.ldw = p.K;
+    p.Wup = (const half_t*)wup;
     p.M = n * p.Ho * p.Wo; p.N = cout;
     p.bias_n = (const half_t*)bias;
     p.rowvec = (const half_t*)rowvec; p.rows_per_vec = p.Ho * p.Wo; p.ldrv = cout;
@@ -136,6 +137,18 @@
                size_t ws_bytes, void* stream) {
     op_begin();
     return op_conv(x1, c1, x2, c2, n, h, w, hv, wv, stride, ksize, wt, bias, rowvec, residual, y, cout, ws, ws_bytes, stream, nullptr, nullptr);
+}
+
+int ld_op_upconv2x_fold(const void* wt, int cout, int cin, void* wfold, void* stream) {
+    op_begin();
+    return upconv_fold_launch((const half_t*)wt, cout, cin, (half_t*)wfold, (hipStream_t)stream);
+}
+
+int ld_op_upconv2x(const void* x, int c, int n, int h, int w, int hv, int wv, const void* wt, const void* wfold, const void* bias, void* y, int cout,
+                   void* ws, size_t ws_bytes, void* stream) {
+    op_begin();
+    if (wfold == nullptr) return LD_ERR_ARG;
+    return op_conv(x, c, nullptr, 0, n, h, w, hv, wv, 1, 3, wt, bias, nullptr, nullptr, y, cout, ws, ws_bytes, stream, nullptr, nullptr, wfold);
 }
 
 size_t ld_op_conv_gn_partials_floats(int n, int hw) {
diff --git a/lightdiffusion_amd/csrc/gemm.h b/lightdiffusion_amd/csrc/gemm.h
--- a/lightdiffusion_amd/csrc/gemm.h
+++ b/lightdiffusion_amd/csrc/gemm.h
@@ -55,11 +55,12 @@
     const half_t* W8 = nullptr;
     int* sync = nullptr;
     int c8_S = 0;
+    const half_t* Wup = nullptr;
     int dbg = 0;
 };
 
-enum GemmRoute { GR_NONE = 0, GR_CONV8, GR_CONV6, GR_GEMM7, GR_GEMM5, GR_GEMM3, GR_GEMM4 };
-enum GemmReduce { GRD_NONE = 0, GRD_PLAIN, GRD_GROUPNORM };
+enum GemmRoute { GR_NONE = 0, GR_CONV8, GR_CONV6, GR_GEMM7, GR_GEMM5, GR_GEMM3, GR_GEMM4, GR_UPCONV };
+enum GemmReduce { GRD_NONE = 0, GRD_PLAIN, GRD_GROUPNORM, GRD_UPCONV };
 struct GemmPlan {
     int status = LD_OK;
     int route = GR_NONE;
@@ -89,6 +90,7 @@
 bool conv8_weight_eligible(int N, int Cin);
 size_t conv8_weight_bytes(int N, int Cin);
 int conv8_repack_launch(const half_t* w_okki, int N, int Cin, half_t* dst, hipStream_t stream);
+int upconv_reduce_launch(const GemmParams& p, hipStream_t stream);
 #define LD_SYNC_INTS 1024
 
 static inline int gemm_pick_bn(int N) { return (N % 160 == 0) ? 160 : 128; }
diff --git a/lightdiffusion_amd/csrc/gemm.hip b/lightdiffusion_amd/csrc/gemm.hip
--- a/lightdiffusion_amd/csrc/gemm.hip
+++ b/lightdiffusion_amd/csrc/gemm.hip
@@ -1097,7 +1097,28 @@
     }
 }
 
-template <int EPI, bool LNC>
+__device__ __forceinline__ void v5_upconv_strip(const GemmParams& p, const half_t* Cs, int m_base, int col, int py, int px, int lane) {
+    const int m = m_base + (lane & 15);
+    const int mm = m < p.M ? m : p.M - 1;
+    const int hw = p.Hs * p.Ws, img = mm / hw, rem = mm - img * hw, y = rem / p.Ws, x = rem - y * p.Ws;
+    const int orow = (img * 2 * p.Hs + 2 * y + py) * (2 * p.Ws) + 2 * x + px;
+    uint4 cv[5];
+#pragma unroll
+    for (int k = 0; k < 5; ++k) {
+        const int q = lane + k * 64;
+        const int row = q / 20, cc = q - row * 20;
+        cv[k] = ld16(Cs + row * V5_EPI_LD + cc * 8);
+    }
+#pragma unroll
+    for (int k = 0; k < 5; ++k) {
+        const int q = lane + k * 64;
+        const int row = q / 20, cc = q - row * 20;
+        const int o = __shfl(orow, row, 64);
+        if (m_base + row < p.M) st16(p.C + (long long)o * p.ldc + col + cc * 8, cv[k]);
+    }
+}
+
+template <int EPI, bool LNC, bool UPF = false>
 __device__ __forceinline__ void v5_finish(const GemmParams& p, f32x4 (&acc)[4][10], char* smem5, const float* ln_mu, const float* ln_rs, int z, int m0,
                                           int n0, int wm0, int wn0, int wid, int lane, int ks, int splitk, int tn_i) {
     constexpr int TM = 4, TN = 10;
@@ -1125,7 +1146,8 @@
     const bool ln = LNC && p.ln_stat != nullptr;
     const bool bias_done = EPI == 2 || p.act == 0;
     const bool add_b = bias_done && p.bias_n != nullptr;
-    const half_t* bsrc = (add_b ? p.bias_n + n_w : reinterpret_cast<const half_t*>(g_zero_row)) + fq * 4;
+    const int up_cout = UPF ? p.N >> 2 : 1, up_ph = UPF ? n0 / up_cout : 0, up_col = n_w - up_ph * up_cout;
+    const half_t* bsrc = (add_b ? p.bias_n + (UPF ? up_col : n_w) : reinterpret_cast<const half_t*>(g_zero_row)) + fq * 4;
     auto stage = [&](auto I, half_t* dst) {
         constexpr int i = decltype(I)::value;
         const float mu = ln ? ln_mu[wm0 + i * 16 + fr] : 0.f, rs = ln ? ln_rs[wm0 + i * 16 + fr] : 1.f;
@@ -1148,16 +1170,26 @@
     stage(std::integral_constant<int, 1>{}, Cs1);
     asm volatile("s_waitcnt lgkmcnt(0)" ::: "memory");
     __builtin_amdgcn_sched_barrier(0);
-    v5_epilogue_strip<EPI>(p, Cs, z, m_w, n_w, lane, part, bias_done);
-    v5_epilogue_strip<EPI>(p, Cs1, z, m_w + 16, n_w, lane, part, bias_done);
+    if constexpr (UPF) {
+        v5_upconv_strip(p, Cs, m_w, up_col, up_ph >> 1, up_ph & 1, lane);
+        v5_upconv_strip(p, Cs1, m_w + 16, up_col, up_ph >> 1, up_ph & 1, lane);
+    } else {
+        v5_epilogue_strip<EPI>(p, Cs, z, m_w, n_w, lane, part, bias_done);
+        v5_epilogue_strip<EPI>(p, Cs1, z, m_w + 16, n_w, lane, part, bias_done);
+    }
     asm volatile("s_waitcnt lgkmcnt(0)" ::: "memory");
     __builtin_amdgcn_sched_barrier(0);
     stage(std::integral_constant<int, 2>{}, Cs);
     stage(std::integral_constant<int, 3>{}, Cs1);
     asm volatile("s_waitcnt lgkmcnt(0)" ::: "memory");
     __builtin_amdgcn_sched_barrier(0);
-    v5_epilogue_strip<EPI>(p, Cs, z, m_w + 32, n_w, lane, part, bias_done);
-    v5_epilogue_strip<EPI>(p, Cs1, z, m_w + 48, n_w, lane, part, bias_done);
+    if constexpr (UPF) {
+        v5_upconv_strip(p, Cs, m_w + 32, up_col, up_ph >> 1, up_ph & 1, lane);
+        v5_upconv_strip(p, Cs1, m_w + 48, up_col, up_ph >> 1, up_ph & 1, lane);
+    } else {
+        v5_epilogue_strip<EPI>(p, Cs, z, m_w + 32, n_w, lane, part, bias_done);
+        v5_epilogue_strip<EPI>(p, Cs1, z, m_w + 48, n_w, lane, part, bias_done);
+    }
 }
 
 template <int TM, int TN>
@@ -1335,7 +1367,7 @@
     }
 }
 
-template <bool CONV, int EPI>
+template <bool CONV, int EPI, bool UPF = false>
 __global__ __launch_bounds__(512, 2) void gemm5_kernel(const GemmParams p) {
     constexpr int TM = 4, TN = 10;
     __shared__ __attribute__((aligned(16))) char smem5[V5_NST * V5_STAGE_BYTES];
@@ -1385,6 +1417,24 @@
     int seg_left = 0;
     int k_issue = kt_begin * V5_BK;
     auto conv_seek = [&](int k0) {
+        if constexpr (UPF) {
+            const int tap = k0 / Cin, c0 = k0 - tap * Cin;
+            const int ph = n0 / (p.N >> 2);
+            const int dy = (ph >> 1) - 1 + (tap >> 1), dx = (ph & 1) - 1 + (tap & 1);
+            const int hw = p.Hs * p.Ws;
+            seg_left = (Cin - c0) / V5_BK;
+#pragma unroll
+            for (int i = 0; i < 2; ++i) {
+                const int m = m0 + a_row0 + i * 16;
+                const int mm = m < p.M ? m : 0;
+                const int img = mm / hw, rem = mm - img * hw;
+                const int y = rem / p.Ws, x = rem - y * p.Ws;
+                const int iy = y + dy, ix = x + dx;
+                const bool ok = m < p.M && (unsigned)iy < (unsigned)p.Hs && (unsigned)ix < (unsigned)p.Ws && tap < 4;
+                a_ptr[i] = ok ? Ab + (((long long)img * p.Hs + iy) * p.Ws + ix) * Cin + c0 + lchunk * 8 : zp + lchunk * 8;
+            }
+            return;
+        }
         const int K9 = p.ksize * p.ksize * Cin;
         const bool skp = k0 >= K9 && p.SC1 > 0;
         const int tap = skp ? 0 : k0 / Cin;
@@ -1514,7 +1564,7 @@
     }
     if (!grp1) __builtin_amdgcn_s_barrier();
 
-    v5_finish<EPI, EPI != 0>(p, acc, smem5, ln_mu, ln_rs, z, m0, n0, wm0, wn0, wid, lane, ks, splitk, tn_i);
+    v5_finish<EPI, EPI != 0, UPF>(p, acc, smem5, ln_mu, ln_rs, z, m0, n0, wm0, wn0, wid, lane, ks, splitk, tn_i);
 }
 
 template <int W, bool GN, int BN = V5_BN, int BM = V5_BM, bool UP = false>
@@ -2176,6 +2226,7 @@
     const std::string tile = std::to_string(pl.bm) + "," + std::to_string(pl.bn);
     std::string s;
     switch (pl.route) {
+        case GR_UPCONV: s = "upconv_kernel<256,320>"; break;
         case GR_CONV8: s = "conv8_kernel<W" + std::to_string(pl.wc) + (pl.up ? ",up>" : ">"); break;
         case GR_CONV6:
             s = "conv6_kernel<W" + std::to_string(pl.wc) + ",halo" + (pl.gn ? "+groupnorm" : "") +
@@ -2186,7 +2237,7 @@
         case GR_GEMM4: s = "gemm4_kernel<" + tile + (pl.conv ? ",conv" : ",plain") + (pl.two_wg ? ",2wg>" : ">"); break;
         default: s = "gemm3_kernel<" + tile + (pl.conv ? ",conv" : ",plain") + (pl.deep ? ",deep>" : ">"); break;
     }
-    if (pl.reduce != GRD_NONE) s += pl.reduce == GRD_GROUPNORM ? "+splitk_reduce_gn_kernel" : "+splitk_reduce_kernel";
+    if (pl.reduce != GRD_NONE) s += pl.reduce == GRD_GROUPNORM ? "+splitk_reduce_gn_kernel" : pl.reduce == GRD_UPCONV ? "+upconv_reduce_kernel" : "+splitk_reduce_kernel";
     static std::mutex mu; static std::set<std::string> pool;
     std::lock_guard<std::mutex> lock(mu);
     const char* name = pool.insert(s).first->c_str();
@@ -2254,6 +2305,28 @@
                     p.ldc == p.N && (p.N / 4) % 8 == 0 && p.N / 32 <= 256;
     pl->reduce = gn ? GRD_GROUPNORM : GRD_PLAIN;
     if (gn) pl->gn_chunks = p.gn_P;
+}
+
+static bool upconv_plan(const GemmParams& p, GemmPlan* out) {
+    if (!(p.conv && p.ksize == 3 && p.stride == 1 && p.pad == 1 && p.Hv == 2 * p.Hs && p.Wv == 2 * p.Ws && p.Ho == p.Hv && p.Wo == p.Wv && p.C2 == 0 &&
+          p.SC1 == 0 && p.C1 % V5_BK == 0 && p.N % V5_BN == 0 && p.n_valid == p.N && p.bm == 0 && p.bn == 0 && p.splitk == 0 && p.batch == 1 && p.act == 0 &&
+          p.alpha == 1.0f && p.rowvec == nullptr && p.R == nullptr && p.bias_m == nullptr && p.stat_out == nullptr && p.ln_stat == nullptr && p.ldc == p.N))
+        return false;
+    if ((long long)p.M * 4 > 0x7fffffffll) return false;
+    if (p.M / (p.Ho * p.Wo) <= 2) return false;
+    const int Ms = p.M / 4, K = 4 * p.C1;
+    const long long tiles = (long long)((Ms + V5_BM - 1) / V5_BM) * (4 * p.N / V5_BN);
+    int sk = 1;
+    if (tiles < 192 && p.partial != nullptr) {
+        sk = (int)((256 + tiles - 1) / tiles);
+        const int cap = K / 640 < 1 ? 1 : K / 640;
+        if (sk > cap) sk = cap;
+        while (sk > 1 && (size_t)sk * Ms * 4 * p.N * sizeof(float) > p.partial_bytes) --sk;
+    }
+    out->bm = V5_BM; out->bn = V5_BN; out->splitk = sk; out->up = true;
+    out->grid_x = (unsigned)(tiles * sk); out->grid_z = 1;
+    out->reduce = sk > 1 ? GRD_UPCONV : GRD_NONE;
+    return true;
 }
 
 static bool v6_plan(const GemmParams& p, bool gn, GemmPlan* out) {
@@ -2353,6 +2426,7 @@
         if (p.gn_part != nullptr) pl.gn_chunks = p.Wo * p.Wo / 16;
         return done(GR_CONV8);
     }
+    if (p.Wup != nullptr && !gn && upconv_plan(p, &pl)) return done(GR_UPCONV);
     if (GemmPlan v6 = pl; v6_plan(p, gn, &v6)) {
         pl = v6;
         const int bn6 = pl.bn, wc = pl.wc;
@@ -2522,6 +2596,15 @@
                 else launch_conv6<false>(pl.wc, p, grid, stream);
             }
             break;
+        case GR_UPCONV: {
+            p.W = p.Wup; p.K = 4 * p.C1; p.ldw = p.K; p.M = pin.M / 4; p.N = 4 * pin.N; p.n_valid = p.N;
+            p.splitk = pl.splitk; p.bn = 160; p.xcd_gm = 0;
+            hipLaunchKernelGGL((gemm5_kernel<true, 0, true>), grid, dim3(512), 0, stream, p);
+            if (pl.reduce == GRD_UPCONV) {
+                if (const int st = upconv_reduce_launch(p, stream); st != LD_OK) return st;
+            }
+            return hipGetLastError() == hipSuccess ? LD_OK : LD_ERR_HIP;
+        }
         case GR_GEMM7:
             if (pl.geglu && pl.ln) hipLaunchKernelGGL((gemm7_kernel<true, true>), grid, dim3(512), 0, stream, p);
             else if (pl.geglu) hipLaunchKernelGGL((gemm7_kernel<true, false>), grid, dim3(512), 0, stream, p);
diff --git a/lightdiffusion_amd/csrc/kernels.h b/lightdiffusion_amd/csrc/kernels.h
--- a/lightdiffusion_amd/csrc/kernels.h
+++ b/lightdiffusion_amd/csrc/kernels.h
@@ -42,6 +42,7 @@
 int mlp_out_fold_launch(const half_t* Wpo, const half_t* W2, const half_t* b2, const half_t* bpo, int C, half_t* Wout, half_t* bout, hipStream_t stream);
 int skip_fold_launch(const half_t* W2, const half_t* Wsk, const half_t* b2, const half_t* bsk, int N, int K9, int SC, half_t* Wout, half_t* bout,
                      hipStream_t stream);
+int upconv_fold_launch(const half_t* W, int O, int I, half_t* Wout, hipStream_t stream);
 struct SmallConvInArgs {
     const float* x = nullptr;
     const float* scale_sigma = nullptr;
diff --git a/lightdiffusion_amd/csrc/misc.hip b/lightdiffusion_amd/csrc/misc.hip
--- a/lightdiffusion_amd/csrc/misc.hip
+++ b/lightdiffusion_amd/csrc/misc.hip
@@ -578,6 +578,54 @@
     const int t = blockIdx.x * blockDim.x + threadIdx.x;
     if (t < N) bout[t] = (half_t)((float)b2[t] + (float)bsk[t]);
 }
+__global__ __launch_bounds__(256) void upconv_fold_kernel(const uint4* __restrict__ W, int O, int Ic, uint4* __restrict__ Wout) {
+    const long long total = 16ll * O * Ic;
+    for (long long q = (long long)blockIdx.x * blockDim.x + threadIdx.x; q < total; q += (long long)gridDim.x * blockDim.x) {
+        const int c = (int)(q % Ic);
+        const int t = (int)((q / Ic) & 3);
+        const int o = (int)((q / (4ll * Ic)) % O);
+        const int ph = (int)(q / (4ll * Ic * O));
+        const int py = ph >> 1, px = ph & 1, a = t >> 1, b = t & 1;
+        const int ky0 = py + a == 0 ? 0 : (py + a == 2 ? 2 : (py == 0 ? 1 : 0)), ky1 = py + a == 1 ? ky0 + 1 : ky0;
+        const int kx0 = px + b == 0 ? 0 : (px + b == 2 ? 2 : (px == 0 ? 1 : 0)), kx1 = px + b == 1 ? kx0 + 1 : kx0;
+        float acc[8] = {0.f, 0.f, 0.f, 0.f, 0.f, 0.f, 0.f, 0.f};
+        for (int ky = ky0; ky <= ky1; ++ky)
+            for (int kx = kx0; kx <= kx1; ++kx) {
+                float v[8];
+                unpack8(W[((long long)o * 9 + ky * 3 + kx) * Ic + c], v);
+#pragma unroll
+                for (int j = 0; j < 8; ++j) acc[j] += v[j];
+            }
+        Wout[q] = pack8(acc);
+    }
+}
+__global__ __launch_bounds__(256) void upconv_reduce_kernel(const GemmParams p) {
+    const int cpr = p.N / 8, cout = p.N >> 2, hw = p.Hs * p.Ws;
+    const long long total = (long long)p.M * cpr;
+    const long long slab = (long long)p.M * p.N;
+    for (long long q = (long long)blockIdx.x * blockDim.x + threadIdx.x; q < total; q += (long long)gridDim.x * blockDim.x) {
+        const int m = (int)(q / cpr), n = (int)(q - (long long)m * cpr) * 8;
+        const int ph = n / cout, col = n - ph * cout;
+        const float* base = p.partial + (long long)m * p.N + n;
+        float v[8];
+        unpack8(p.bias_n != nullptr ? ld16(p.bias_n + col) : zero16(), v);
+        float a[8] = {0.f, 0.f, 0.f, 0.f, 0.f, 0.f, 0.f, 0.f};
+        for (int s = 0; s < p.splitk; ++s) {
+            const f32x4 x0 = *reinterpret_cast<const f32x4*>(base + s * slab), x1 = *reinterpret_cast<const f32x4*>(base + s * slab + 4);
+#pragma unroll
+            for (int j = 0; j < 4; ++j) {
+                a[j] += x0[j];
+                a[4 + j] += x1[j];
+            }
+        }
+#pragma unroll
+        for (int j = 0; j < 8; ++j) v[j] += a[j];
+        const int img = m / hw, rem = m - img * hw, y = rem / p.Ws, x = rem - y * p.Ws;
+        const long long orow = (long long)(img * 2 * p.Hs + 2 * y + (ph >> 1)) * (2 * p.Ws) + 2 * x + (ph & 1);
+        st16(p.C + orow * p.ldc + col, pack8(v));
+    }
+}
+
 }
 
 int skip_fold_launch(const half_t* W2, const half_t* Wsk, const half_t* b2, const half_t* bsk, int N, int K9, int SC, half_t* Wout, half_t* bout,
@@ -593,3 +641,21 @@
                        K9 / 8, SC / 8, reinterpret_cast<uint4*>(Wout), bout);
     return hipGetLastError() == hipSuccess ? LD_OK : LD_ERR_HIP;
 }
+
+int upconv_fold_launch(const half_t* W, int O, int I, half_t* Wout, hipStream_t stream) {
+    if (W == nullptr || Wout == nullptr || O <= 0 || I <= 0 || (I & 7)) return LD_ERR_ARG;
+    const long long total = 16ll * O * (I / 8);
+    int blocks = (int)((total + 255) / 256);
+    if (blocks > 4096) blocks = 4096;
+    hipLaunchKernelGGL(upconv_fold_kernel, dim3(blocks), dim3(256), 0, stream, reinterpret_cast<const uint4*>(W), O, I / 8, reinterpret_cast<uint4*>(Wout));
+    return hipGetLastError() == hipSuccess ? LD_OK : LD_ERR_HIP;
+}
+
+int upconv_reduce_launch(const GemmParams& p, hipStream_t stream) {
+    if (p.partial == nullptr || p.C == nullptr || p.splitk < 2 || p.M <= 0 || (p.N % 32) || p.Hs <= 0 || p.Ws <= 0 || p.M % (p.Hs * p.Ws)) return LD_ERR_ARG;
+    const long long total = (long long)p.M * (p.N / 8);
+    int blocks = (int)((total + 255) / 256);
+    if (blocks > 2048) blocks = 2048;
+    hipLaunchKernelGGL(upconv_reduce_kernel, dim3(blocks), dim3(256), 0, stream, p);
+    return hipGetLastError() == hipSuccess ? LD_OK : LD_ERR_HIP;
+}
diff --git a/lightdiffusion_amd/csrc/unet.hip b/lightdiffusion_amd/csrc/unet.hip
--- a/lightdiffusion_amd/csrc/unet.hip
+++ b/lightdiffusion_amd/csrc/unet.hip
@@ -21,6 +21,7 @@
 };
 struct ConvW {
     int cin = 0, cout = 0, w = -1, b = -1;
+    long long f_up = -1;
 };
 enum LayerKind { L_CONV_IN, L_RES, L_ST, L_DOWN, L_UP };
 struct Layer {
@@ -237,6 +238,8 @@
             if (lvl && i == c.num_res_blocks[lvl]) {
                 L.push_back({L_UP, add_conv(u, S("output_blocks.%d.%d.conv", idx, j), ch, ch)});
                 u->want_w8(u->convs.back().w, ch, ch);
+                u->convs.back().f_up = (long long)u->fold_bytes;
+                u->fold_bytes += (16 * (size_t)ch * ch * sizeof(half_t) + 255) / 256 * 256;
             }
             u->out_blocks.push_back(L);
             ++idx;
@@ -281,7 +284,7 @@
 
     half_t* conv3(const half_t* x1, int C1, const half_t* x2, int C2, int Hs, int Ws, int Hv, int Wv, int stride, int wslot, int bslot,
                   int cout, const half_t* rowvec, int ldrv, const half_t* R, half_t* out, int* Ho_, int* Wo_, int ksize = 3, float* stats = nullptr,
-                  int* stats_done = nullptr) {
+                  int* stats_done = nullptr, const half_t* wup = nullptr) {
         const int Ho = ksize == 3 ? (Hv - 1) / stride + 1 : Hv, Wo = ksize == 3 ? (Wv - 1) / stride + 1 : Wv;
         GemmParams p;
         p.conv = 1;
@@ -290,6 +293,7 @@
         p.Hs = Hs; p.Ws = Ws; p.Hv = Hv; p.Wv = Wv; p.Ho = Ho; p.Wo = Wo; p.stride = stride;
         p.W = P(wslot); p.ldw = ksize * ksize * (C1 + C2);
         p.W8 = ksize == 3 ? u->w8(wslot) : nullptr;
+        p.Wup = wup;
         p.M = n * Ho * Wo; p.N = cout; p.K = ksize * ksize * (C1 + C2);
         p.bias_n = P(bslot);
         p.rowvec = rowvec; p.rows_per_vec = Ho * Wo; p.ldrv = ldrv;
@@ -519,6 +523,11 @@
                                         reinterpret_cast<half_t*>(u->fold_base + r.f_c2_w), reinterpret_cast<half_t*>(u->fold_base + r.f_c2_b), stream);
         if (st != LD_OK) return st;
     }
+    for (const ConvW& c : u->convs) {
+        if (c.f_up < 0) continue;
+        const int st = upconv_fold_launch(u->pt.ptr(c.w), c.cout, c.cin, reinterpret_cast<half_t*>(u->fold_base + c.f_up), stream);
+        if (st != LD_OK) return st;
+    }
     u->fold_dirty = false;
     return LD_OK;
 }
@@ -610,7 +619,8 @@
                     const ConvW& cw = u->convs[L.idx];
                     const int Hv = outH > 0 ? outH : f.H * 2, Wv = outW > 0 ? outW : f.W * 2;
                     half_t* o = ar.halfs((size_t)n * Hv * Wv * cw.cout);
-                    R.conv3(f.p, f.C, nullptr, 0, f.H, f.W, Hv, Wv, 1, cw.w, cw.b, cw.cout, nullptr, 0, nullptr, o, nullptr, nullptr);
+                    const half_t* wup = (u->fold_base != nullptr && cw.f_up >= 0) ? reinterpret_cast<const half_t*>(u->fold_base + cw.f_up) : nullptr;
+                    R.conv3(f.p, f.C, nullptr, 0, f.H, f.W, Hv, Wv, 1, cw.w, cw.b, cw.cout, nullptr, 0, nullptr, o, nullptr, nullptr, 3, nullptr, nullptr, wup);
                     f = {o, cw.cout, Hv, Wv};
                     break;
                 }
diff --git a/lightdiffusion_amd/ops.py b/lightdiffusion_amd/ops.py
--- a/lightdiffusion_amd/ops.py
+++ b/lightdiffusion_amd/ops.py
@@ -102,6 +102,25 @@
     ws = _ws(192 << 20, x.device)
     check(lib().ld_op_conv(_p(x), c1, _p(x2), c2, n, h, w, hv, wv, stride, ksize, _p(w_packed), _p(bias), _p(rowvec), _p(residual),
                            _p(y), cout, _p(ws), ws.numel(), _stream()), "ld_op_conv")
+    return y
+
+
+def upconv2x_fold(w_packed: torch.Tensor) -> torch.Tensor:
+    O = w_packed.shape[0]
+    I = w_packed.shape[1] // 9
+    out = torch.empty(4, O, 4 * I, dtype=torch.float16, device=w_packed.device)
+    check(lib().ld_op_upconv2x_fold(_p(w_packed), O, I, _p(out), _stream()), "ld_op_upconv2x_fold")
+    return out
+
+
+def upconv2x(x: torch.Tensor, w_packed: torch.Tensor, w_fold: torch.Tensor, bias: Optional[torch.Tensor], out_hw: Optional[tuple] = None) -> torch.Tensor:
+    n, h, w, c = x.shape
+    hv, wv = (2 * h, 2 * w) if out_hw is None else out_hw
+    cout = w_packed.shape[0]
+    y = torch.empty(n, hv, wv, cout, dtype=torch.float16, device=x.device)
+    ws = _ws(192 << 20, x.device)
+    check(lib().ld_op_upconv2x(_p(x), c, n, h, w, hv, wv, _p(w_packed), _p(w_fold), _p(bias), _p(y), cout, _p(ws), ws.numel(), _stream()),
+          "ld_op_upconv2x")
     return y
 
 
```
